# AberHu/TF-NAS

Measured on AMD Instinct MI355X. Metric: supernet search images/sec (w-step + alpha-step), higher is better.
Workload: dtype fp32

## Files before the change

### include/tfnas_hip.h

```cpp
#ifndef TFNAS_HIP_H
#define TFNAS_HIP_H

#include <stddef.h>
#include <stdint.h>

#ifdef __cplusplus
extern "C" {
#endif

#define TFNAS_ABI_VERSION 4
#define TFNAS_MAX_GROUPS 8
#define TFNAS_MAX_SINK 4
#define TFNAS_MAX_CELLS 32

#define TFNAS_MODE_CELL 0
#define TFNAS_MODE_STEM 1
#define TFNAS_MODE_HEAD 2

#define TFNAS_ACT_RELU 0
#define TFNAS_ACT_SWISH 1
#define TFNAS_ACT_RELU6 2
#define TFNAS_ACT_HSWISH 3

#define TFNAS_EINVAL (-1)
#define TFNAS_ENULL (-2)
#define TFNAS_ERANGE (-3)

typedef struct TfnasGroup {
    int32_t mc;
    int32_t k;
    int32_t se;
    int32_t mcp;
    int32_t off;
    int32_t se_off;
    int32_t pad0, pad1;
    const float *w_expand, *w_dw, *w_proj, *w_se_r, *b_se_r, *w_se_e, *b_se_e;
    float *g_expand, *g_dw, *g_proj, *g_se_r, *gb_se_r, *g_se_e, *gb_se_e;
} TfnasGroup;

typedef struct TfnasCellDesc {
    int32_t N, H, W;
    int32_t ic, oc;
    int32_t stride;
    int32_t act;
    int32_t has_res;
    int32_t G;
    int32_t need_wgrad;
    int32_t Ho, Wo;
    int32_t M;
    int32_t SE;
    float eps;
    int32_t mode;
    int32_t Hi, Wi;
    int32_t stor;
    int32_t gemm_mode;
    int32_t flags;
    TfnasGroup g[TFNAS_MAX_GROUPS];
    int (*sync_fn)(void *user, double *table, uint64_t ndoubles, void *stream);
    void *sync_user;
    int32_t sync_world;
    int32_t route;
    int32_t fwd_route;
    int32_t pad_route;
    void *wgrad_stream[3];
} TfnasCellDesc;
#define TFNAS_GEMM_EXPLICIT 0x1000
#define TFNAS_CELL_LAZY_JOIN 1
#define TFNAS_CELL_ACCUM_WGRAD 0x20
#define TFNAS_CELL_K7 0x80
#define TFNAS_CELL_ACTS 0x100
#define TFNAS_CELL_NOEXPAND 0x200
#define TFNAS_CELL_FUSED 0x400
#define TFNAS_ROUTE_FX_OFF 0x1
#define TFNAS_ROUTE_FOLD_OFF 0x2
#define TFNAS_ROUTE_DWWG_OFF 0x4
#define TFNAS_ROUTE_DWWG2_OFF 0x8
#define TFNAS_ROUTE_XG_OFF 0x10
#define TFNAS_ROUTE_XG_ALL 0x20
#define TFNAS_ROUTE_DW_SHIFT 6
#define TFNAS_ROUTE_DW_MASK 0xc0
#define TFNAS_ROUTE_SE_SHIFT 8
#define TFNAS_ROUTE_SE_MASK 0x300
#define TFNAS_ROUTE_WGRAD_INLINE 0x400
#define TFNAS_ROUTE_GRAM2 0x800
#define TFNAS_ROUTE_ALL 0xfff
#define TFNAS_ROUTE_TAKEN_VALID 0x1
#define TFNAS_ROUTE_TAKEN_FX 0x2

typedef struct TfnasCellWs {
    uint64_t E;
    uint64_t D;
    uint64_t Pr;
    uint64_t fsmall;
    uint64_t off_pooled, off_gate, off_hpre;
    uint64_t stats;
    uint64_t off_stats1, off_stats2, off_stats3;
    uint64_t out;
    uint64_t dZ;
    uint64_t dEh;
    uint64_t bsmall;
    uint64_t off_dgate, off_dpooled, off_dgl, off_dhpre, off_cb1;
    uint64_t red;
    uint64_t off_red3, off_red2, off_red1, off_resdot;
    uint64_t part;
    uint64_t dx;
    uint64_t dxp;
} TfnasCellWs;

int tfnas_abi_version(void);

typedef int (*tfnas_stats_sync_fn)(void *user, double *table, uint64_t ndoubles, void *stream);
int tfnas_set_stats_sync(tfnas_stats_sync_fn fn, void *user, int world);

int tfnas_shutdown(void);

uint64_t tfnas_sizeof(int which);

int tfnas_cell_plan(TfnasCellDesc *d);

int tfnas_cell_ws(const TfnasCellDesc *d, TfnasCellWs *ws);

int tfnas_efree_supported(const TfnasCellDesc *d);
int tfnas_cell_route(const TfnasCellDesc *d);
int tfnas_fx_supported(const TfnasCellDesc *d);

int tfnas_mixedop_fwd(const TfnasCellDesc *d, const float *x, const float *wmix,
                      float *E, float *D, float *Pr, float *fsmall, double *stats, float *part,
                      float *out, void *stream);

int tfnas_mixedop_bwd(const TfnasCellDesc *d, const float *x, const float *wmix,
                      const float *E, const float *D, const float *Pr, const float *fsmall,
                      const double *stats, const float *dout,
                      float *dZ, float *dEh, float *bsmall, double *red, float *part,
                      float *dx, float *dxp, float *dwmix, void *stream);

typedef struct TfnasBnAffine {
    const float *weight[3], *bias[3];
    float *g_weight[3], *g_bias[3];
    float *running_mean[3], *running_var[3];
    float momentum;
    int32_t eval;
} TfnasBnAffine;

int tfnas_mbconv_fwd(const TfnasCellDesc *d, const TfnasBnAffine *bn, const float *drop_scale, const float *x,
                     float *E, float *D, float *Pr, float *fsmall, double *stats, float *part, float *out, void *stream);

int tfnas_mbconv_bwd(const TfnasCellDesc *d, const TfnasBnAffine *bn, const float *drop_scale, const float *x,
                     const float *E, const float *D, const float *Pr, const float *fsmall, const double *stats,
                     const float *dout, float *dout_s, float *dZ, float *dEh, float *bsmall, double *red, float *part,
                     float *dx, float *dxp, void *stream);

int tfnas_head_affine_fwd(const TfnasCellDesc *d, const TfnasBnAffine *bn, const float *x, float *E, double *stats,
                          float *part, float *pooled, void *stream);
int tfnas_head_affine_bwd(const TfnasCellDesc *d, const TfnasBnAffine *bn, const float *x, const float *E,
                          const double *stats, const float *dpooled, float *dEh, float *cb1, double *red, float *part,
                          float *dx, float *dxp, void *stream);

int tfnas_head_fwd(const TfnasCellDesc *d, const float *x, float *E, double *stats, float *part, float *pooled,
                   void *stream);
int tfnas_head_bwd(const TfnasCellDesc *d, const float *x, const float *E, const double *stats, const float *dpooled,
                   float *dEh, float *cb1, double *red, float *part, float *dx, float *dxp, void *stream);

int tfnas_head_wgrad(const TfnasCellDesc *d, const float *x, const float *E, const float *dEh, const float *cb1, float *part,
                     void *stream);

int tfnas_cls_ce(int N, int C, int K, const float *pooled, const float *W, const float *bias, const int64_t *target, float scale,
                 float *logits, float *loss_n, float *dlogits, float *dpooled, void *stream);
int tfnas_cls_ce_ex(int N, int C, int K, const float *pooled, const float *W, const float *bias, const int64_t *target, float scale,
                    float eps, float *logits, float *loss_n, int32_t *rank, float *dlogits, float *dpooled, void *stream);
int tfnas_cls_wgrad(int npath, int N, int C, int K, const float *const *pooled, const float *const *dlogits,
                    const float *const *loss_n, float loss_scale, float *dW, float *db, float *loss, void *stream);
int tfnas_cls_wgrad_ex(int npath, int N, int C, int K, const float *const *pooled, const float *const *dlogits,
                       const float *const *loss_n, const int32_t *rank0, float loss_scale, float *dW, float *db, float *loss,
                       double *meter, void *stream);
int tfnas_cls_reduce(int N, int C, int K, const float *pooled, const float *dlogits, const float *loss_n, const int32_t *rank,
                     const float *gscale, int accumulate, float *dW, float *db, float *out, double *meter, void *stream);
int tfnas_add_into(float *dst, const float *src, uint64_t count, void *stream);

int tfnas_arch_fwd(int ncell, const float *const *log_alpha, const float *e, const float *lat, float T,
                   float *w, float *cell_lat, void *stream);

int tfnas_arch_bwd(int ncell, const float *w, const float *lat, const float *dw, const float *dcell_lat,
                   float T, float *const *dlog_alpha, void *stream);

int tfnas_arch_sample(int ncell, const float *const *log_alpha, const uint8_t *mask, const float *e, float T,
                      int mode, int32_t *pos_out, void *stream);

int tfnas_arch_project(int n, float *const *p, const int32_t *len, void *stream);

int tfnas_sink_fwd(int K, const float *betas, const float *const *res, const float *cell_lat,
                   uint64_t count, float *out, float *out_lat, float *bw_out, void *stream);

int tfnas_sink_bwd(int K, const float *bw, const float *const *res, const float *cell_lat, const float *dout,
                   const float *dlat, uint64_t count, float *const *dres, float *dbetas, float *dcell_lat,
                   double *dot_scratch, void *stream);

#define TFNAS_MAX_STAGES 8

typedef struct TfnasStage {
    int32_t ncell;
    int32_t start_res;
    int32_t first_cell;
    int32_t nres;
    const float *betas;
    float *dbetas;
} TfnasStage;

typedef struct TfnasPathDesc {
    int32_t ncell, nstage;
    int32_t soft;
    int32_t need_dx0;
    int32_t efree_mask_lo;
    int32_t reserved0;
    TfnasStage stage[TFNAS_MAX_STAGES];
    TfnasCellDesc cell[TFNAS_MAX_CELLS];
} TfnasPathDesc;

typedef struct TfnasPathWs {
    uint64_t saved;
    uint64_t scratch;
    uint64_t total;
    uint64_t out_count;
    int32_t out_h, out_w, out_c, pad;
} TfnasPathWs;

int tfnas_path_create(void **ctx);
int tfnas_path_destroy(void *ctx);
int tfnas_path_set_side_stream(void *ctx, void *stream);
int tfnas_path_plan(void *ctx, const TfnasPathDesc *pd, TfnasPathWs *ws);
int tfnas_path_set_wgrad_accum(void *ctx, uint32_t cell_mask);

int tfnas_paths_fwd(int npath, void *const *ctx, const float *const *x0, const float *const *wmix,
                    const float *const *cell_lat, float *const *arena, float *const *out, float *const *out_lat,
                    void *const *streams);

int tfnas_paths_bwd(int npath, void *const *ctx, const float *const *x0, const float *const *wmix,
                    const float *const *cell_lat, float *const *arena, const float *const *dout,
                    const float *const *dout_lat, float *const *dx0, float *const *dwmix, float *const *dcell_lat,
                    void *const *streams, int stage_begin, int stage_end);

int tfnas_sgd_clip_step(float *w, float *g, float *m, int nranges, const uint64_t *off, const uint64_t *goff, const uint64_t *len,
                        float max_norm, float lr, float momentum, float wd, float grad_scale, double *scratch,
                        uint64_t scratch_doubles, float *norm_out, void *stream);

int tfnas_pack_ranges(const float *src, float *dst, int nranges, const uint64_t *off, const uint64_t *doff,
                      const uint64_t *len, void *stream);

int tfnas_arch_adam_project(int n, float *const *p, const float *const *g, const int32_t *len, float *m, float *v,
                            float max_norm, float lr, float beta1, float beta2, float eps, float wd, int step,
                            float grad_scale, float *norm_out, void *stream);

int tfnas_set_lazy_join(int on);
int tfnas_side_stream(void *stream, void **side);
int tfnas_side_join(void *stream);

#define TFNAS_GEMM_F32 0
#define TFNAS_GEMM_BF16 1
#define TFNAS_GEMM_X2 3
#define TFNAS_GEMM_X3 6
#define TFNAS_GEMM_EVERYWHERE 0x100
int tfnas_set_gemm_mode(int mode);
int tfnas_gemm_mode(void);

int tfnas_prof_enable(unsigned mask);
int tfnas_prof_count(void);
const char *tfnas_prof_name(int id);
int tfnas_prof_collect(int id, uint64_t *launches, double *total_ms);
int tfnas_prof_last_split(int id, uint64_t *soft_launches, double *soft_ms);

#ifdef __cplusplus
}
#endif
#endif
```

### tf-nas_amd/csrc/capi.hip

```cpp
#include <string.h>
#include "tfnas_dev.h"
#include "kernels.h"
#include "cell_impl.h"

#include <stdlib.h>
#include <mutex>
#include <vector>

struct SideCtx {
    int device;
    hipStream_t main, side;
    hipEvent_t fork[4], join;
};
static std::mutex g_side_mu;
static std::vector<SideCtx*> g_side;

static SideCtx* side_for(hipStream_t s) {
    int dev = 0;
    if (hipGetDevice(&dev) != hipSuccess) return nullptr;
    std::lock_guard<std::mutex> lk(g_side_mu);
    for (SideCtx* c : g_side)
        if (c->main == s && c->device == dev) return c;
    SideCtx* c = new SideCtx();
    c->device = dev;
// ... 51 lines not shown
static int g_lazy_join = 0;
extern "C" int tfnas_set_lazy_join(int on) {
    g_lazy_join = on ? 1 : 0;
    return 0;
}
extern "C" int tfnas_side_stream(void* stream, void** side) {
    if (!side) return TFNAS_ENULL;
    *side = nullptr;
    SideCtx* c = side_for(S(stream));
    if (c) *side = (void*)c->side;
    return 0;
}
extern "C" int tfnas_side_join(void* stream) {
    return side_join(side_for(S(stream)), S(stream));
}

extern "C" int tfnas_shutdown(void) {
    std::lock_guard<std::mutex> lk(g_side_mu);
    for (SideCtx* c : g_side) {
        (void)hipStreamSynchronize(c->side);
        for (int i = 0; i < 4; ++i) (void)hipEventDestroy(c->fork[i]);
        (void)hipEventDestroy(c->join);
        (void)hipStreamDestroy(c->side);
        delete c;
    }
    g_side.clear();
    return 0;
}

StatsSync g_stats_sync = {nullptr, nullptr, 1};

extern "C" int tfnas_set_stats_sync(tfnas_stats_sync_fn fn, void* user, int world) {
    if (fn && world < 1) return TFNAS_ERANGE;
    g_stats_sync.fn = fn;
    g_stats_sync.user = user;
    g_stats_sync.world = fn ? world : 1;
    return 0;
}

extern "C" int tfnas_abi_version(void) { return TFNAS_ABI_VERSION; }
extern "C" int tfnas_set_gemm_mode(int mode) { return set_gemm_mode(mode); }
extern "C" int tfnas_gemm_mode(void) { return gemm_mode(); }

extern "C" uint64_t tfnas_sizeof(int which) {
    switch (which) {
        case 0: return sizeof(TfnasGroup);
        case 1: return sizeof(TfnasCellDesc);
        case 2: return sizeof(TfnasCellWs);
        case 3: return sizeof(TfnasStage);
        case 4: return sizeof(TfnasPathDesc);
        case 5: return sizeof(TfnasPathWs);
        case 6: return sizeof(TfnasBnAffine);
        case 7: return TFNAS_PART_ALLOC;
        case 8: return TFNAS_TAIL_SLOTS;
        default: return 0;
    }
}

static int check_act(const TfnasCellDesc* d) {
    if (d->act == TFNAS_ACT_RELU || d->act == TFNAS_ACT_SWISH) return 0;
    if (d->act != TFNAS_ACT_RELU6 && d->act != TFNAS_ACT_HSWISH) return TFNAS_EINVAL;
    if (!(d->flags & TFNAS_CELL_ACTS) || d->mode == TFNAS_MODE_STEM) return TFNAS_EINVAL;
    return 0;
}

static int check_kind(const TfnasCellDesc* d) {
    const CellKind kind = cell_kind(*d);
    if (kind == TFNAS_KIND_MBCONV) return 0;
    if (cell_noexpand(*d) && cell_fused(*d)) return TFNAS_EINVAL;
    if (d->mode != TFNAS_MODE_CELL || d->G != 1) return TFNAS_EINVAL;
    const TfnasGroup& g = d->g[0];
    if (kind == TFNAS_KIND_NOEXPAND && (g.mc != d->ic || g.w_expand || g.g_expand)) return TFNAS_EINVAL;
    if (kind == TFNAS_KIND_FUSED && (g.k != 3 || g.w_dw || g.g_dw)) return TFNAS_EINVAL;
    return 0;
}

static int check_modes(const TfnasCellDesc* d) {
    TRY(check_act(d));
    if (d->gemm_mode != 0) {
        const int gm = d->gemm_mode & ~(TFNAS_GEMM_EXPLICIT | TFNAS_GEMM_EVERYWHERE);
        if (!(d->gemm_mode & TFNAS_GEMM_EXPLICIT) || (gm != 0 && gm != 1 && gm != 3 && gm != 6)) return TFNAS_EINVAL;
    }
    if (d->flags & ~(TFNAS_CELL_LAZY_JOIN | TFNAS_CELL_ACCUM_WGRAD | TFNAS_CELL_K7 | TFNAS_CELL_ACTS | TFNAS_CELL_NOEXPAND |
                     TFNAS_CELL_FUSED))
        return TFNAS_EINVAL;
    TRY(check_kind(d));
    if (!(d->flags & TFNAS_CELL_K7)) {
        for (int g = 0; g < d->G && g < TFNAS_MAX_GROUPS; ++g)
            if (d->g[g].k == 7) return TFNAS_EINVAL;
    }
    if (d->route & ~TFNAS_ROUTE_ALL) return TFNAS_EINVAL;
    if ((d->route & TFNAS_ROUTE_XG_OFF) && (d->route & TFNAS_ROUTE_XG_ALL)) return TFNAS_EINVAL;
    if ((d->route & TFNAS_ROUTE_SE_MASK) == TFNAS_ROUTE_SE_MASK) return TFNAS_EINVAL;
    if (d->fwd_route & ~(TFNAS_ROUTE_TAKEN_VALID | TFNAS_ROUTE_TAKEN_FX)) return TFNAS_EINVAL;
    if (d->sync_fn && d->sync_world < 1) return TFNAS_ERANGE;
    return 0;
}

static bool wgrad_row_fits(const TfnasCellDesc& d) { return cell_fused(d) ? conv_wgrad_row_fits(d) : dw_wgrad_row_fits(d); }

extern "C" int tfnas_cell_plan(TfnasCellDesc* d) {
    if (!d) return TFNAS_ENULL;
    if (d->G < 1 || d->G > TFNAS_MAX_GROUPS) return TFNAS_ERANGE;
    if (d->mode < TFNAS_MODE_CELL || d->mode > TFNAS_MODE_HEAD) return TFNAS_EINVAL;
    if (d->mode == TFNAS_MODE_STEM) {
        if (d->ic != 27 || d->G != 1 || d->Hi < 1 || d->Wi < 1 || d->has_res) return TFNAS_EINVAL;
        d->H = (d->Hi - 1) / 2 + 1;
        d->W = (d->Wi - 1) / 2 + 1;
    } else if (d->ic < 4 || (d->ic & 3)) {
        return TFNAS_EINVAL;
    }
    if (d->mode == TFNAS_MODE_HEAD && d->G != 1) return TFNAS_EINVAL;
    if (d->stor != 0) return TFNAS_EINVAL;
    if (d->N < 1 || d->H < 1 || d->W < 1 || d->oc < 4 || (d->oc & 3)) return TFNAS_EINVAL;
    if (d->oc > 1024) return TFNAS_EINVAL;
    if (d->stride != 1 && d->stride != 2) return TFNAS_EINVAL;
    TRY(check_act(d));
    if (d->has_res && (d->ic != d->oc || d->stride != 1)) return TFNAS_EINVAL;
    TRY(check_modes(d));
    d->Ho = (d->H - 1) / d->stride + 1;
    d->Wo = (d->W - 1) / d->stride + 1;
    int off = 0, se_off = 0;
    for (int g = 0; g < d->G; ++g) {
        TfnasGroup& gr = d->g[g];
        if (gr.mc < 1 || (gr.k != 3 && gr.k != 5 && gr.k != 7) ||
            gr.se < 0) return TFNAS_EINVAL;
        if (gr.se & 3) return TFNAS_EINVAL;
        gr.mcp = (gr.mc + 3) & ~3;
        off = (off + 31) & ~31;
        gr.off = off;
        gr.se_off = se_off;
        off += gr.mcp;
        se_off += gr.se;
    }
    off = (off + 31) & ~31;
    if ((off & 511) == 0) off += 32;
    d->M = off;
    d->SE = se_off;
    if ((double)d->N * d->H * d->W >= 2147483647.0) return TFNAS_ERANGE;
    if (!wgrad_row_fits(*d)) return TFNAS_ERANGE;
    return 0;
}

extern "C" int tfnas_cell_ws(const TfnasCellDesc* d, TfnasCellWs* ws) {
    if (!d || !ws) return TFNAS_ENULL;
    memset(ws, 0, sizeof(*ws));
    if (!wgrad_row_fits(*d)) return TFNAS_ERANGE;
    const uint64_t P = (uint64_t)d->N * d->H * d->W, Po = (uint64_t)d->N * d->Ho * d->Wo;
    const uint64_t M = d->M, N = d->N, SE = d->SE, G = d->G, oc = d->oc;
    ws->E = cell_has_E(*d) ? P * M : 0;
    ws->D = Po * M;
    ws->Pr = G * Po * oc;
    ws->off_pooled = 0;
    ws->off_gate = N * M;
    ws->off_hpre = 2 * N * M;
    ws->fsmall = 2 * N * M + N * SE + 4;
    ws->off_stats1 = 0;
    ws->off_stats2 = 2 * M;
    ws->off_stats3 = 4 * M;
    ws->stats = 4 * M + 2 * G * oc;
    ws->out = Po * oc;
    ws->dZ = Po * M;
    ws->dEh = P * M;
    ws->off_dgate = 0;
    ws->off_dpooled = N * M;
    ws->off_dgl = 2 * N * M;
    ws->off_dhpre = 3 * N * M;
    ws->off_cb1 = 3 * N * M + ((N * SE + 3) & ~(uint64_t)3);
    ws->bsmall = ws->off_cb1 + 4 * M;
    ws->off_red3 = 0;
    ws->off_resdot = 2 * G * oc;
    ws->off_red2 = 2 * G * oc + oc;
    ws->off_red1 = ws->off_red2 + 2 * M;
    ws->red = ws->off_red1 + 2 * M;
    ws->part = (d->need_wgrad ? 2 : 1) * (uint64_t)TFNAS_PART_ALLOC;
    ws->dx = P * d->ic;
    {
        const int ns = (d->mode == TFNAS_MODE_STEM || !cell_has_E(*d)) ? 1 : gemm_plan_expand_dgrad(*d, true).splits;
        ws->dxp = ns > 1 ? (uint64_t)ns * P * d->ic : 4;
    }
    return 0;
}

extern "C" int tfnas_efree_supported(const TfnasCellDesc* dp) { return (dp && efree_supported(*dp)) ? 1 : 0; }
extern "C" int tfnas_fx_supported(const TfnasCellDesc* dp) { return (dp && fx_supported(*dp)) ? 1 : 0; }
static int route_taken(const TfnasCellDesc& d, bool affine) {
    return TFNAS_ROUTE_TAKEN_VALID | ((!affine && fx_supported(d)) ? TFNAS_ROUTE_TAKEN_FX : 0);
}
extern "C" int tfnas_cell_route(const TfnasCellDesc* dp) { return dp ? route_taken(*dp, false) : 0; }

static void bn_site(const TfnasCellDesc& d, int site, int& nch, uint64_t& cnt) {
    const uint64_t P = (uint64_t)d.N * d.H * d.W, Po = (uint64_t)d.N * d.Ho * d.Wo;
    nch = site == 2 ? d.oc : d.g[0].mc;
    cnt = site == 0 ? P : Po;
}
static int check_bn_sites(const TfnasCellDesc& d, const TfnasBnAffine* bn) {
    if (cell_has_bn0(d)) return 0;
    if (bn->weight[0] || bn->bias[0] || bn->g_weight[0] || bn->g_bias[0] || bn->running_mean[0] || bn->running_var[0])
        return TFNAS_EINVAL;
    return 0;
}
static int bn_fwd_fix(const TfnasCellDesc& d, const TfnasBnAffine* bn, int site, double* stats, hipStream_t s) {
    int nch;
    uint64_t cnt;
    bn_site(d, site, nch, cnt);
    return launch_bn_fwd_fix(stats, nch, cnt, d.eps, bn->weight[site], bn->bias[site], bn->running_mean[site],
                             bn->running_var[site], bn->momentum, bn->eval, s, stats_world(d));
}

static int fwd_front_mbconv(const TfnasCellDesc& d, const TfnasCellDesc& d0, const CellFwdBufs& b, bool fx, bool sync,
                            double* stats1, double* stats2, hipStream_t s) {
    const TfnasBnAffine* bn = b.bn;
    if (fx) TRY(launch_fx_stats(d, b.x, stats1, b.part, s));
    else if (b.E) TRY(launch_expand_fwd(d, b.x, b.E, stats1, b.part, s));
    else TRY(launch_expand_stats_gram(d, b.x, stats1, b.part, s));
    if (sync) TRY(stats_sync(d, stats1, 2 * (size_t)d.M, s));
    if (bn) TRY(bn_fwd_fix(d0, bn, 0, stats1, s));
    if (fx) TRY(launch_fx_fwd(d, b.x, stats1, b.E, b.D, stats2, b.part, s));
    else TRY(launch_dw_fwd(d, b.E, b.x, stats1, b.D, stats2, b.part, s));
    return 0;
}

int cell_fwd_impl(const TfnasCellDesc& d0, const TfnasCellWs& ws, const CellFwdBufs& b, hipStream_t s, int* route) {
    double* stats1 = b.stats + ws.off_stats1;
    double* stats2 = b.stats + ws.off_stats2;
    double* stats3 = b.stats + ws.off_stats3;
    float* pooled = b.fsmall + ws.off_pooled;
    float* gate = b.fsmall + ws.off_gate;
    float* hpre = b.fsmall + ws.off_hpre;
    const TfnasBnAffine* bn = b.bn;
    TfnasCellDesc dc = d0;
    if (bn) dc.eps = -1.f;
    const TfnasCellDesc& d = dc;
    const int taken = route_taken(d0, bn != nullptr);
    if (route) *route = taken;
    const bool fx = (taken & TFNAS_ROUTE_TAKEN_FX) != 0;
    const bool sync = !(bn && bn->eval);
    switch (cell_kind(d)) {
    case TFNAS_KIND_FUSED:
        TRY(launch_conv_fwd(d, b.x, b.D, stats2, b.part, s));
        break;
    case TFNAS_KIND_NOEXPAND:
        TRY(launch_dw_fwd(d, nullptr, b.x, nullptr, b.D, stats2, b.part, s));
        break;
    case TFNAS_KIND_MBCONV:
        TRY(fwd_front_mbconv(d, d0, b, fx, sync, stats1, stats2, s));
        break;
    }
    if (sync) TRY(stats_sync(d, stats2, 2 * (size_t)d.M, s));
    if (bn) TRY(bn_fwd_fix(d0, bn, 1, stats2, s));
    TRY(launch_se_pool(d, b.D, stats2, pooled, s));
    TRY(launch_se_fc_fwd(d, pooled, hpre, gate, b.part, TFNAS_PART_FLOATS, s));
    TRY(launch_project_fwd(d, b.D, gate, stats2, b.Pr, stats3, b.part, s));
    if (sync) TRY(stats_sync(d, stats3, 2 * (size_t)d.G * d.oc, s));
    if (bn) TRY(bn_fwd_fix(d0, bn, 2, stats3, s));
    if (b.drop_scale && d.has_res) {
        TfnasCellDesc dn = dc;
        dn.has_res = 0;
        TRY(launch_mix_fwd(dn, b.Pr, stats3, b.wmix, b.x, b.out, s));
        return launch_rowscale(b.out, b.out, b.x, b.drop_scale, d.N, (uint64_t)d.Ho * d.Wo * d.oc, s);
    }
    TRY(launch_mix_fwd(d, b.Pr, stats3, b.wmix, b.x, b.out, s));
    return 0;
}

static hipStream_t fork_to(const CellSide* so, int k, hipStream_t main) {
    if (!so || !so->side[k] || so->side[k] == main) return main;
    if (hipEventRecord(so->fork[k], main) != hipSuccess || hipStreamWaitEvent(so->side[k], so->fork[k], 0) != hipSuccess)
        return main;
    return so->side[k];
}

static int bn_bwd_fix(const TfnasCellDesc& d, const TfnasBnAffine* bn, int site, double* red, hipStream_t s) {
    int nch;
    uint64_t cnt;
    bn_site(d, site, nch, cnt);
    TRY(launch_bn_bwd_fix(red, nch, cnt, bn->weight[site], bn->bias[site], bn->g_weight[site], bn->g_bias[site], s,
                          wgrad_accum(d)));
    if (bn->eval) return (int)hipMemsetAsync(red, 0, sizeof(double) * 2 * (size_t)nch, s);
    return 0;
}

static int expand_dx(const TfnasCellDesc& d, const float* dEh, const float* x, const float* cb1, float* part, const float* dout,
                     const float* wmix, float* dx, float* dxp, hipStream_t s, const float* add_src = nullptr,
                     const float* add_scale = nullptr, int nsl = -1) {
    const size_t room = TFNAS_PART_FLOATS - expand_gram_floats(d);
    float* gram = part + room;
    TRY(launch_expand_gram(d, cb1, part, room, gram, s));
    return launch_expand_dgrad(d, dEh, x, cb1, gram, dout, wmix, dx, dxp, s, add_src, add_scale, nsl);
}


namespace {
struct CellBwd {
    const TfnasCellDesc& d0;
    TfnasCellDesc d;
    const TfnasCellWs& ws;
    CellBwdBufs b;
    hipStream_t s;
    const CellSide* so;
    const TfnasBnAffine* bn;
    int taken;
    const float* dout_res;
    const double *stats1, *stats2, *stats3;
    const float *pooled, *gate, *hpre;
    float *dgate, *dpooled, *dhpre, *cb1;
    double *red3, *red2, *red1;
    float *part, *part_w, *part_w1, *part_w2;

    int run();
    int tail_fused();
    int tail_noexpand();
    int tail_mbconv();
};

int CellBwd::run() {
    if (d.need_wgrad) {
        const CellKind kind = cell_kind(d);
        for (int g = 0; g < d.G; ++g) {
            const TfnasGroup& gr = d.g[g];
            if ((!gr.g_expand && kind != TFNAS_KIND_NOEXPAND) || (!gr.g_dw && kind != TFNAS_KIND_FUSED) || !gr.g_proj) return TFNAS_ENULL;
            if (gr.se > 0 && (!gr.g_se_r || !gr.gb_se_r || !gr.g_se_e || !gr.gb_se_e)) return TFNAS_ENULL;
        }
    }
    TRY(launch_mix_bwd_stats(d, b.dout, b.Pr, stats3, b.x, red3, part, s));
    TRY(stats_sync(d, red3, 2 * (size_t)d.G * d.oc, s));
    if (b.dwmix) TRY(launch_mix_dw(d, red3, b.red + ws.off_resdot, b.dwmix, s));
    if (bn) TRY(bn_bwd_fix(d0, bn, 2, red3, s));
    if (!b.dx && !d.need_wgrad) return 0;
    if (d.need_wgrad)
        TRY(launch_project_wgrad(d, b.dout, b.Pr, b.D, gate, stats2, stats3, red3, b.wmix, part_w, fork_to(so, 0, s)));
    const bool fused2 = bn2_fused_fits(d);
    const bool fold = fused2 && !(d.route & TFNAS_ROUTE_FOLD_OFF) && project_fold_ok(d, (size_t)ws.dEh) && (d.G == 1 || d.Ho * d.Wo <= 784);
    if (fold) {
        TRY(launch_project_dgrad(d, b.dout, b.Pr, stats3, red3, b.wmix, b.dZ, s, b.D, stats2, b.dEh));
        TRY(launch_bn2_gather(d, b.dEh, dgate, part, s));
    } else {
        TRY(launch_project_dgrad(d, b.dout, b.Pr, stats3, red3, b.wmix, b.dZ, s));
        if (fused2) TRY(launch_bn2_pool(d, b.dZ, b.D, stats2, dgate, part, s));
        else TRY(launch_se_bwd_reduce(d, b.dZ, b.D, stats2, dgate, s));
    }
    TRY(launch_se_fc_bwd(d, dgate, gate, hpre, dhpre, dpooled, b.dEh, (size_t)ws.dEh, s));
    if (fused2) TRY(launch_bn2_finish(d, part, gate, dpooled, red2, s));
    else TRY(launch_bn2_bwd(d, b.dZ, b.D, stats2, gate, dpooled, red2, part, s));
    TRY(stats_sync(d, red2, 2 * (size_t)d.M, s));
    if (bn) TRY(bn_bwd_fix(d0, bn, 1, red2, s));
    switch (cell_kind(d)) {
    case TFNAS_KIND_FUSED: return tail_fused();
    case TFNAS_KIND_NOEXPAND: return tail_noexpand();
    case TFNAS_KIND_MBCONV: break;
    }
    return tail_mbconv();
}

int CellBwd::tail_fused() {
    TRY(launch_conv_dd(d, b.dZ, b.D, gate, dpooled, stats2, red2, b.dEh, s));
    if (d.need_wgrad) {
        hipStream_t sw = fork_to(so, 1, s);
        if (d.SE > 0) TRY(launch_se_wgrad(d, dgate, gate, dhpre, hpre, pooled, sw));
        TRY(launch_conv_wgrad(d, b.dEh, b.x, part_w1, sw));
    }
    if (b.dx) TRY(launch_conv_dgrad(d, b.dEh, d.has_res ? dout_res : nullptr, b.dx, part, s));
    return 0;
}

int CellBwd::tail_noexpand() {
    if (d.need_wgrad) {
        hipStream_t sw = fork_to(so, 1, s);
        if (d.SE > 0) TRY(launch_se_wgrad(d, dgate, gate, dhpre, hpre, pooled, sw));
        TRY(launch_dw_wgrad(d, b.dZ, gate, dpooled, b.D, stats2, red2, b.x, nullptr, part_w1, sw));
    }
    if (b.dx)
        TRY(launch_dw_bwd_dx(d, b.dZ, gate, dpooled, b.D, stats2, red2, d.has_res ? dout_res : nullptr, b.dx, s));
    return 0;
}

int CellBwd::tail_mbconv() {
    if (taken & TFNAS_ROUTE_TAKEN_FX) {
        int nsl = 0;
        TRY(launch_fx_bwd(d, b.x, b.E, stats1, stats2, red2, b.dZ, b.D, gate, dpooled, b.dEh, (size_t)ws.dEh, red1, cb1, part, &nsl, s));
        if (b.dx) TRY(expand_dx(d, nullptr, b.x, cb1, part, dout_res, b.wmix, b.dx, b.dEh, s, b.add_src, b.add_scale, nsl));
        return 0;
    }
    const DwPlan dw_bwd = dw_plan_bwd_data(d, b.E == nullptr, b.x != nullptr);
    const bool dw_fused = dw_bwd.fuse_wgrad;
    if (d.need_wgrad) {
        if (d.SE > 0 || !dw_fused) {
            hipStream_t sw = fork_to(so, 1, s);
            if (d.SE > 0) TRY(launch_se_wgrad(d, dgate, gate, dhpre, hpre, pooled, sw));
            if (!dw_fused) TRY(launch_dw_wgrad(d, b.dZ, gate, dpooled, b.D, stats2, red2, b.E, stats1, part_w1, sw));
        }
    }
    if (bn || stats_sync_on(d)) {
        TRY(launch_dw_bwd_data(dw_bwd, d, b.dZ, gate, dpooled, b.D, stats2, red2, b.E, b.x, stats1, b.dEh, red1, part, s));
        TRY(stats_sync(d, red1, 2 * (size_t)d.M, s));
        if (bn) TRY(bn_bwd_fix(d0, bn, 0, red1, s));
        TRY(launch_bn1_consts(d, stats1, red1, cb1, s));
    } else {
        TRY(launch_dw_bwd_data(dw_bwd, d, b.dZ, gate, dpooled, b.D, stats2, red2, b.E, b.x, stats1, b.dEh, red1, part, s, cb1));
    }
    if (d.need_wgrad) TRY(launch_expand_wgrad(d, b.dEh, b.E, cb1, b.x, part_w2, fork_to(so, 2, s)));
    if (b.dx && d.mode != TFNAS_MODE_STEM)
        TRY(expand_dx(d, b.dEh, b.x, cb1, part, dout_res, b.wmix, b.dx, b.dxp, s, b.add_src, b.add_scale));
    return 0;
}
}

int cell_bwd_impl(const TfnasCellDesc& d0, const TfnasCellWs& ws, const CellBwdBufs& b0, hipStream_t s, const CellSide* so,
                  int fwd_route) {
    const TfnasBnAffine* bn = b0.bn;
    const int taken = route_taken(d0, bn != nullptr);
    if ((fwd_route & TFNAS_ROUTE_TAKEN_VALID) && taken != fwd_route) return TFNAS_EINVAL;
    const CellBwdBufs& b = b0;
    CellBwd c = {d0, d0, ws, b0, s, so, bn, taken, b0.dout,
                 b.stats + ws.off_stats1, b.stats + ws.off_stats2, b.stats + ws.off_stats3,
                 b.fsmall + ws.off_pooled, b.fsmall + ws.off_gate, b.fsmall + ws.off_hpre,
                 b.bsmall + ws.off_dgate, b.bsmall + ws.off_dpooled, b.bsmall + ws.off_dhpre, b.bsmall + ws.off_cb1,
                 b.red + ws.off_red3, b.red + ws.off_red2, b.red + ws.off_red1,
                 b.part, b.part_w,
                 b.part_w1 ? b.part_w1 : b.part_w,
                 b.part_w2 ? b.part_w2 : b.part_w};
    if (bn) c.d.eps = -1.f;
    if (b0.drop_scale && d0.has_res) {
        if (!b0.dout_s) return TFNAS_ENULL;
        TRY(launch_rowscale(b0.dout_s, b0.dout, nullptr, b0.drop_scale, d0.N, (uint64_t)d0.Ho * d0.Wo * d0.oc, s));
        c.b.dout = b0.dout_s;
    }
    return c.run();
}

static int check_E(const TfnasCellDesc& d, const float* E, bool efree_counts) {
    if (E || !cell_has_E(d) || (efree_counts && efree_supported(d))) return 0;
    return TFNAS_ENULL;
}

extern "C" int tfnas_mixedop_fwd(const TfnasCellDesc* dp, const float* x, const float* wmix, float* E, float* D,
                                 float* Pr, float* fsmall, double* stats, float* part, float* out, void* stream) {
    if (!dp || !x || !D || !Pr || !fsmall || !stats || !part || !out) return TFNAS_ENULL;
    const TfnasCellDesc& d = *dp;
    if (d.mode == TFNAS_MODE_HEAD) return TFNAS_EINVAL;
    TRY(check_modes(dp));
    TRY(check_E(d, E, true));
    TfnasCellWs ws;
    TRY(tfnas_cell_ws(dp, &ws));
    CellFwdBufs b = {x, wmix, E, D, Pr, fsmall, stats, part, out};
    return cell_fwd_impl(d, ws, b, S(stream));
}

static int cell_bwd_entry(const TfnasCellDesc& d, CellBwdBufs b, hipStream_t s, void* const* wgrad_stream, bool lazy) {
    TfnasCellWs ws;
    TRY(tfnas_cell_ws(&d, &ws));
    SideCtx* sc = (d.need_wgrad && route_side(d)) ? side_for(s) : nullptr;
    SideJoinGuard guard;
    guard.c = sc;
    guard.main = s;
    CellSide so = {};
    if (sc) {
        for (int i = 0; i < 3; ++i) {
            hipStream_t own = (wgrad_stream && wgrad_stream[i]) ? S(wgrad_stream[i]) : nullptr;
            so.side[i] = own ? own : sc->side;
            guard.extra[i] = own;
            so.fork[i] = sc->fork[i];
            if (own) {
// ... 210 lines not shown
```

### tf-nas_amd/csrc/cell_impl.h

```cpp
#pragma once
#include <hip/hip_runtime.h>
#include "tfnas_hip.h"

static inline hipStream_t S(void* s) { return reinterpret_cast<hipStream_t>(s); }

#define TRY(call)               \
    do {                        \
        int _r = (call);        \
        if (_r != 0) return _r; \
    } while (0)

struct CellFwdBufs {
    const float* x;
    const float* wmix;
    float *E, *D, *Pr, *fsmall;
    double* stats;
    float* part;
    float* out;
    const TfnasBnAffine* bn = nullptr;
    const float* drop_scale = nullptr;
};

struct CellBwdBufs {
    const float *x, *wmix, *E, *D, *Pr, *fsmall;
    const double* stats;
    const float* dout;
    float *dZ, *dEh, *bsmall;
    double* red;
    float *part, *part_w;
    float *dx, *dxp, *dwmix;
    const float* add_src;
    const float* add_scale;
    const TfnasBnAffine* bn = nullptr;
    const float* drop_scale = nullptr;
    float* dout_s = nullptr;
    float *part_w1 = nullptr, *part_w2 = nullptr;
};

struct CellSide {
    hipStream_t side[3];
    hipEvent_t fork[3];
};

int cell_fwd_impl(const TfnasCellDesc& d, const TfnasCellWs& ws, const CellFwdBufs& b, hipStream_t s, int* route = nullptr);
int cell_bwd_impl(const TfnasCellDesc& d, const TfnasCellWs& ws, const CellBwdBufs& b, hipStream_t s, const CellSide* so,
                  int fwd_route);
```

### tf-nas_amd/csrc/efree_kernels.hip

```cpp
#include "tfnas_dev.h"
#include "kernels.h"
#include "prof.h"
#include "efree.h"

__global__ __launch_bounds__(256) void k_x_colsum(const float* __restrict__ x, int P, int ic, int rps,
                                                  float* __restrict__ part) {
    __shared__ f32x4 red[256];
    const int tid = threadIdx.x, icq = ic >> 2, stride = (256 / icq) * icq;
    const int r0 = blockIdx.x * rps, r1 = min(P, r0 + rps);
    const f32x4* __restrict__ x4 = reinterpret_cast<const f32x4*>(x) + (size_t)r0 * icq;
    const int n4 = (r1 - r0) * icq;
    f32x4 s = zero4();
    if (tid < stride) {
        int i = tid;
        for (; i + 7 * stride < n4; i += 8 * stride) {
            f32x4 v[8];
#pragma unroll
            for (int u = 0; u < 8; ++u) v[u] = x4[i + u * stride];
            s += ((v[0] + v[1]) + (v[2] + v[3])) + ((v[4] + v[5]) + (v[6] + v[7]));
        }
        for (; i < n4; i += stride) s += x4[i];
    }
    red[tid] = s;
    __syncthreads();
    if (tid < ic) {
        const int cq = tid >> 2, comp = tid & 3;
        float t = 0.f;
        for (int k = cq; k < stride; k += icq) t += red[k][comp];
        part[(size_t)blockIdx.x * ic + tid] = t;
    }
}

template <int CT>
__global__ __launch_bounds__(256) void k_x_gram(const float* __restrict__ x, int P, int ic, int rps,
                                                const double* __restrict__ xsum, float* __restrict__ part) {
    __shared__ float red[4][CT * CT][4][64 + 1];
    const int tid = threadIdx.x, lane = tid & 63, wave = tid >> 6, n = lane & 15, q = lane >> 4;
    const int r0 = blockIdx.x * rps, r1 = min(P, r0 + rps);
    float mu[CT];
    bool chok[CT];
#pragma unroll
    for (int t = 0; t < CT; ++t) {
        chok[t] = 16 * t + n < ic;
        mu[t] = chok[t] ? (float)(xsum[16 * t + n] / (double)P) : 0.f;
    }
    f32x4 acc[CT][CT];
#pragma unroll
    for (int i = 0; i < CT; ++i)
#pragma unroll
        for (int j = 0; j < CT; ++j) acc[i][j] = zero4();
    for (int p = r0 + 4 * wave; p < r1; p += 64) {
        float a[4][CT];
#pragma unroll
        for (int u = 0; u < 4; ++u) {
            const int row = p + 16 * u + q;
#pragma unroll
            for (int t = 0; t < CT; ++t)
                a[u][t] = (row < r1 && chok[t]) ? x[(size_t)row * ic + 16 * t + n] - mu[t] : 0.f;
        }
#pragma unroll
        for (int u = 0; u < 4; ++u)
#pragma unroll
            for (int i = 0; i < CT; ++i)
#pragma unroll
                for (int j = 0; j < CT; ++j)
                    acc[i][j] = __builtin_amdgcn_mfma_f32_16x16x4f32(a[u][i], a[u][j], acc[i][j], 0, 0, 0);
    }
#pragma unroll
    for (int i = 0; i < CT; ++i)
#pragma unroll
        for (int j = 0; j < CT; ++j)
#pragma unroll
            for (int r = 0; r < 4; ++r) red[wave][i * CT + j][r][lane] = acc[i][j][r];
    __syncthreads();
    for (int e = tid; e < ic * ic; e += 256) {
        const int gi = e / ic, gj = e - gi * ic;
        const int i = gi >> 4, ri = gi & 15, j = gj >> 4, l = (ri >> 2) * 16 + (gj & 15), r = ri & 3;
        part[(size_t)blockIdx.x * ic * ic + e] =
            (red[0][i * CT + j][r][l] + red[1][i * CT + j][r][l]) + (red[2][i * CT + j][r][l] + red[3][i * CT + j][r][l]);
    }
}

__global__ __launch_bounds__(256) void k_stats1_gram(TfnasCellDesc d, const double* __restrict__ xsum,
                                                     const double* __restrict__ C, double* __restrict__ stats1) {
    __shared__ double Cs[40 * 40 + 40];
    const int ic = d.ic;
    for (int i = threadIdx.x; i < ic * ic + ic; i += 256) Cs[i] = i < ic * ic ? C[i] : xsum[i - ic * ic];
    __syncthreads();
    const int col = blockIdx.x * 256 + threadIdx.x;
    if (col >= d.M) return;
    int g = 0;
    for (; g < d.G - 1; ++g)
        if (col < d.g[g + 1].off) break;
    const int m = col - d.g[g].off;
    double s = 0.0, q = 0.0;
    if (m < d.g[g].mc) {
        const float* __restrict__ w = d.g[g].w_expand + (size_t)m * ic;
        const double P = (double)d.N * d.H * d.W;
        float wr[40];
#pragma unroll
        for (int c = 0; c < 40; ++c) wr[c] = c < ic ? w[c] : 0.f;
        for (int c = 0; c < ic; ++c) {
            double t0 = 0.0, t1 = 0.0;
            const double* row = Cs + c * ic;
#pragma unroll
            for (int c2 = 0; c2 < 40; c2 += 2) {
                if (c2 < ic) {
                    t0 += row[c2] * (double)wr[c2];
                    t1 += row[c2 + 1] * (double)wr[c2 + 1];
                }
            }
            q += (double)w[c] * (t0 + t1);
            s += (double)w[c] * Cs[ic * ic + c];
        }
        q += s * s / P;
    }
    stats1[2 * (size_t)col + 0] = s;
    stats1[2 * (size_t)col + 1] = q;
}

bool efree_supported(const TfnasCellDesc& d) {
    if (d.mode != TFNAS_MODE_CELL || d.need_wgrad) return false;
    if (act_tile_only(d.act)) return false;
    if (cell_noexpand(d) || cell_fused(d)) return false;
    if (!efree_ic_ok(d.ic)) return fx_supported(d);
    if (stats_sync_on(d)) return false;
    if ((size_t)d.N * d.H * d.W * d.ic >= ((size_t)1 << 31)) return false;
    for (int g = 0; g < d.G; ++g)
        if (d.g[g].k != 3 && d.g[g].k != 5) return false;
    return true;
}

int launch_x_colsum(const float* x, int P, int ic, int rps, int nb, float* part, hipStream_t s) {
    ProfScope _prof(TK_EXPAND_FWD, s);
    hipLaunchKernelGGL(k_x_colsum, dim3(nb), dim3(256), 0, s, x, P, ic, rps, part);
    return (int)hipGetLastError();
}

int launch_expand_stats_gram(const TfnasCellDesc& d, const float* x, double* stats1, float* part, hipStream_t s) {
    const int P = d.N * d.H * d.W, ic = d.ic, ne = ic * ic;
    int rps = cdiv(P, 1024);
    if (rps < 256) rps = 256;
    rps = (rps + 63) & ~63;
    const int nb = cdiv(P, rps);
    double* xsum = reinterpret_cast<double*>(part + TFNAS_PART_FLOATS) - (ne + ic + 2);
    xsum = reinterpret_cast<double*>((uintptr_t)xsum & ~(uintptr_t)15);
    double* C = xsum + ic;
    if ((size_t)nb * ne + 2 * (size_t)(ne + ic + 4) > TFNAS_PART_FLOATS) return TFNAS_ERANGE;
    {
        ProfScope _prof(TK_EXPAND_FWD, s);
        hipLaunchKernelGGL(k_x_colsum, dim3(nb), dim3(256), 0, s, x, P, ic, rps, part);
    }
    int rc = launch_reduce_rows(part, nb, ic, (size_t)ic, xsum, nullptr, s);
    if (rc) return rc;
    {
        ProfScope _prof(TK_EXPAND_FWD, s);
        if (ic <= 16) hipLaunchKernelGGL(k_x_gram<1>, dim3(nb), dim3(256), 0, s, x, P, ic, rps, xsum, part);
        else if (ic <= 32) hipLaunchKernelGGL(k_x_gram<2>, dim3(nb), dim3(256), 0, s, x, P, ic, rps, xsum, part);
        else hipLaunchKernelGGL(k_x_gram<3>, dim3(nb), dim3(256), 0, s, x, P, ic, rps, xsum, part);
    }
    rc = launch_reduce_rows(part, nb, ne, (size_t)ne, C, nullptr, s);
    if (rc) return rc;
    ProfScope _prof(TK_SMALL, s);
    hipLaunchKernelGGL(k_stats1_gram, dim3(cdiv(d.M, 256)), dim3(256), 0, s, d, xsum, C, stats1);
    return (int)hipGetLastError();
}
```

### tf-nas_amd/csrc/fx_kernels.hip

```cpp
#include "tfnas_dev.h"
#include "kernels.h"
#include "prof.h"
#include "fx.h"
#include "gemm_x3.h"
#include <type_traits>

static int fx_ks(int ic) { return (ic + 31) / 32; }

bool fx_plan(const TfnasCellDesc& d, FxPlan& pl, bool bwd) {
    if (d.mode != TFNAS_MODE_CELL || d.need_wgrad) return false;
    if (d.act != TFNAS_ACT_RELU && d.act != TFNAS_ACT_SWISH) return false;
    if (stats_sync_on(d)) return false;
    if (d.ic < 64 || d.ic > 192 || (d.ic & 15)) return false;
    if (d.stride != 1) return false;
    const int HW = d.H * d.W;
    if (HW > 196 || d.W < 4) return false;
    const int KS = fx_ks(d.ic);
    int NI = 128 / HW;
    if (NI < 1) NI = 1;
    if (NI > 4) NI = 4;
    if (NI > d.N) NI = d.N;
    const int ntiles = (NI * HW + 15) / 16, RT = (ntiles + 7) / 8;
    const int RTF = (ntiles + 6) / 7;
    if (RTF * KS > 8) return false;
// ... 23 lines not shown
    }
    if (want < 1) want = 1;
    int cps = (nch + want - 1) / want;
    if (cps < (bwd ? 6 : 3)) cps = bwd ? 6 : 3;
    int ns = 0, chunk0 = 0;
    for (int g = 0; g < d.G; ++g) {
        const int ng = (d.g[g].mcp + 31) / 32;
        const int parts = (ng + cps - 1) / cps;
        for (int p = 0; p < parts; ++p) {
            if (ns >= FX_MAX_SLICES) return false;
            const int a = (int)((long)ng * p / parts), b = (int)((long)ng * (p + 1) / parts);
            pl.sl[ns].g = (int16_t)g;
            pl.sl[ns].c0 = (int16_t)(32 * a);
            pl.sl[ns].nch = (int16_t)(b - a);
            pl.sl[ns].chunk0 = (int16_t)(chunk0 + a);
            ++ns;
        }
        chunk0 += ng;
    }
    pl.nslices = ns;
    return true;
}

static size_t fx_fwd_lds(const TfnasCellDesc& d, const FxPlan& pl) {
    const int PAD = pl.KMAX / 2, HP = d.H + 2 * PAD, WP = (d.W + 2 * PAD) | 1;
    const size_t tile = (size_t)(pl.NI * HP * WP + 8) * 128;
    return 2 * tile + 2 * (size_t)pl.PB + 2 * (size_t)pl.WB + 2 * 2048;
}

__device__ __host__ __forceinline__ int fx_swz(int row) { return (0x1230 >> (4 * ((row >> 2) & 3))) & 3; }

__device__ __forceinline__ void fx_split3(float v, unsigned short& h, unsigned short& m, unsigned short& l) {
    const unsigned hb = x3_bits(v);
    const float r1 = v - x3_float(hb & 0xffff0000u);
    const unsigned mb = x3_bits(r1);
    const float r2 = r1 - x3_float(mb & 0xffff0000u);
    h = (unsigned short)(hb >> 16);
    m = (unsigned short)(mb >> 16);
    l = (unsigned short)(x3_bits(r2) >> 16);
}

__global__ __launch_bounds__(256) void k_fx_pack(TfnasCellDesc d, FxPlan pl, const double* __restrict__ stats1,
                                                 const double* __restrict__ stats2, const double* __restrict__ red2,
                                                 unsigned char* __restrict__ blob) {
    const int chunk = blockIdx.x, cy = blockIdx.y * 8, tid = threadIdx.x;
    int si = 0;
    for (; si < pl.nslices - 1; ++si)
        if (chunk < pl.sl[si + 1].chunk0) break;
    const int g = pl.sl[si].g, c0 = pl.sl[si].c0 + 32 * (chunk - pl.sl[si].chunk0);
    const int mc = d.g[g].mc, off = d.g[g].off, ic = d.ic, K = d.g[g].k, KK = K * K;
    const int RS = pl.RS, KP = 32 * pl.KS;
    unsigned char* b = blob + (size_t)chunk * pl.BLOB;
    const float* __restrict__ w1 = d.g[g].w_expand;
    __shared__ float2 cst[8];
    __shared__ float w1s[8][200];
    if (tid < 8) {
        float2 c = make_float2(0.f, 0.f);
        if (c0 + cy + tid < mc) c = bn_consts(stats1 + 2 * (size_t)(off + c0 + cy + tid), 1.0 / ((double)d.N * d.H * d.W), d.eps);
        cst[tid] = c;
        reinterpret_cast<float2*>(b + 96 * RS)[cy + tid] = c;
    }
    for (int e = tid; e < 8 * ic; e += 256) {
        const int chl = e / ic, c = e - chl * ic;
        w1s[chl][c] = (c0 + cy + chl < mc) ? w1[(size_t)(c0 + cy + chl) * ic + c] : 0.f;
    }
    __syncthreads();
    for (int e = tid; e < 8 * (KP / 8); e += 256) {
        const int chl = e / (KP / 8), k0 = 8 * (e - chl * (KP / 8));
        unsigned short h[8], m[8], l[8];
#pragma unroll
        for (int j = 0; j < 8; ++j) fx_split3(k0 + j < ic ? w1s[chl][k0 + j] : 0.f, h[j], m[j], l[j]);
        unsigned char* row = b + (cy + chl) * RS + 2 * k0;
        *reinterpret_cast<u32x4*>(row) = u32x4{h[0] | (unsigned)h[1] << 16, h[2] | (unsigned)h[3] << 16, h[4] | (unsigned)h[5] << 16, h[6] | (unsigned)h[7] << 16};
        *reinterpret_cast<u32x4*>(row + 32 * RS) = u32x4{m[0] | (unsigned)m[1] << 16, m[2] | (unsigned)m[3] << 16, m[4] | (unsigned)m[5] << 16, m[6] | (unsigned)m[7] << 16};
        *reinterpret_cast<u32x4*>(row + 64 * RS) = u32x4{l[0] | (unsigned)l[1] << 16, l[2] | (unsigned)l[3] << 16, l[4] | (unsigned)l[5] << 16, l[6] | (unsigned)l[7] << 16};
    }
    float* taps = reinterpret_cast<float*>(b + pl.PB);
    for (int e = tid; e < KK * 8; e += 256) {
        const int t = e >> 3, ch = cy + (e & 7);
        taps[t * 32 + ch] = (c0 + ch < mc) ? d.g[g].w_dw[(size_t)(c0 + ch) * KK + t] : 0.f;
    }
    if (pl.XB) {
        f32x4* c2 = reinterpret_cast<f32x4*>(b + pl.PB + pl.WB);
        if (tid < 8) {
            f32x4 t = zero4();
            const int ch = cy + tid;
            if (c0 + ch < mc) {
                const double inv = 1.0 / ((double)d.N * d.Ho * d.Wo);
                const float2 c = bn_consts(stats2 + 2 * (size_t)(off + c0 + ch), inv, d.eps);
                t.x = c.x;
                t.y = c.y;
                t.z = (float)(red2[2 * (size_t)(off + c0 + ch) + 0] * inv);
                t.w = (float)(red2[2 * (size_t)(off + c0 + ch) + 1] * inv);
            }
            c2[ch] = t;
        }
        unsigned char* wr = b + pl.PB + pl.WB + 512;
        for (int c = tid; c < ic; c += 256) {
            unsigned short h[8], m[8], l[8];
#pragma unroll
            for (int j = 0; j < 8; ++j) fx_split3(cst[j].y * w1s[j][c], h[j], m[j], l[j]);
            unsigned char* p = wr + c * 64 + (((cy >> 3) ^ fx_swz(c)) * 16);
            *reinterpret_cast<u32x4*>(p) = u32x4{h[0] | (unsigned)h[1] << 16, h[2] | (unsigned)h[3] << 16, h[4] | (unsigned)h[5] << 16, h[6] | (unsigned)h[7] << 16};
            *reinterpret_cast<u32x4*>(p + ic * 64) = u32x4{m[0] | (unsigned)m[1] << 16, m[2] | (unsigned)m[3] << 16, m[4] | (unsigned)m[5] << 16, m[6] | (unsigned)m[7] << 16};
            *reinterpret_cast<u32x4*>(p + 2 * ic * 64) = u32x4{l[0] | (unsigned)l[1] << 16, l[2] | (unsigned)l[3] << 16, l[4] | (unsigned)l[5] << 16, l[6] | (unsigned)l[7] << 16};
        }
    }
}

typedef unsigned char u8;

template <int KS, int RT>
struct FxX {
    bf16x8 h[RT][KS], m[RT][KS], l[RT][KS];
};

__device__ __forceinline__ void fx_split8(f32x4 a, f32x4 b, bf16x8& h, bf16x8& m, bf16x8& l) {
    const X3Planes pa = x3_split4<6>(a), pb = x3_split4<6>(b);
    h = __builtin_bit_cast(bf16x8, u32x4{pa.h.x, pa.h.y, pb.h.x, pb.h.y});
    m = __builtin_bit_cast(bf16x8, u32x4{pa.m.x, pa.m.y, pb.m.x, pb.m.y});
    l = __builtin_bit_cast(bf16x8, u32x4{pa.l.x, pa.l.y, pb.l.x, pb.l.y});
}

#define FX_MFMA6(acc, ah, am, al, bh, bm, bl)                                   \
    acc = __builtin_amdgcn_mfma_f32_16x16x32_bf16(al, bh, acc, 0, 0, 0);        \
    acc = __builtin_amdgcn_mfma_f32_16x16x32_bf16(am, bm, acc, 0, 0, 0);        \
    acc = __builtin_amdgcn_mfma_f32_16x16x32_bf16(ah, bl, acc, 0, 0, 0);        \
    acc = __builtin_amdgcn_mfma_f32_16x16x32_bf16(am, bh, acc, 0, 0, 0);        \
    acc = __builtin_amdgcn_mfma_f32_16x16x32_bf16(ah, bm, acc, 0, 0, 0);        \
    acc = __builtin_amdgcn_mfma_f32_16x16x32_bf16(ah, bh, acc, 0, 0, 0);

template <int NV>
struct FxCopy {
    u32x4 v[NV];
    __device__ __forceinline__ void load(const u8* __restrict__ src, int bytes) {
#pragma unroll
        for (int i = 0; i < NV; ++i) {
            const int o = (threadIdx.x + i * FX_THREADS) * 16;
            v[i] = *reinterpret_cast<const u32x4*>(src + (o < bytes ? o : bytes - 16));
        }
    }
    __device__ __forceinline__ void store(u8* dst, int bytes) const {
#pragma unroll
        for (int i = 0; i < NV; ++i) {
            const int o = (threadIdx.x + i * FX_THREADS) * 16;
            if (o < bytes) *reinterpret_cast<u32x4*>(dst + o) = v[i];
        }
    }
};

#define FX_TERM(A_, B_)                                                                                                  \
    _Pragma("unroll") for (int ct = 0; ct < 2; ++ct) _Pragma("unroll") for (int pt = 0; pt < RT; ++pt)                   \
        acc[ct][pt] = __builtin_amdgcn_mfma_f32_16x16x32_bf16(A_[ct], X.B_[pt][ks], acc[ct][pt], 0, 0, 0);

template <int KS, int RT, int OUT>
__device__ __forceinline__ void fx_expand(const u8* P, const FxX<KS, RT>& X, float* tile, const int (&slot)[RT],
                                          const bool (&pv)[RT], int ntiles, float* __restrict__ eg = nullptr,
                                          const size_t* egoff = nullptr, int chlim = 0) {
    constexpr int RS = 64 * KS + FX_RS_PAD;
    const int lane = threadIdx.x & 63, wave = threadIdx.x >> 6, n = lane & 15, q = lane >> 4;
    f32x4 acc[2][RT];
#pragma unroll
    for (int ct = 0; ct < 2; ++ct)
#pragma unroll
        for (int pt = 0; pt < RT; ++pt) acc[ct][pt] = zero4();
#pragma unroll
    for (int ks = 0; ks < KS; ++ks) {
// ... 792 lines not shown
            for (int r = 0; r < NR; ++r) {
                const size_t a = (pixbase + lpix[r]) * M + goff + cn + 4 * cq;
                dz[r] = ld4_nt(dZ + a);
                dv[r] = ld4_nt(Dt + a);
            }
        }
        {
            const float* taps = reinterpret_cast<const float*>(Wb(i & 1));
            f32x4 t1 = zero4(), t2 = zero4();
            const float* base = DD + it.toff;
            f32x4 acc[4] = {zero4(), zero4(), zero4(), zero4()};
#pragma unroll 1
            for (int ky = 0; ky < K; ++ky) {
                const float* rowp = base + ky * WP * 32;
                const float* wp = taps + (K * K - 1 - ky * K) * 32 + 4 * cq;
                f32x4 win[K + 3];
#pragma unroll
                for (int u = 0; u < K + 3; ++u) win[u] = ld4(rowp + u * 32);
#pragma unroll
                for (int kx = 0; kx < K; ++kx) {
                    const f32x4 wv = ld4(wp - kx * 32);
#pragma unroll
                    for (int jj = 0; jj < 4; ++jj) acc[jj] += win[jj + kx] * wv;
                }
            }
#pragma unroll
            for (int jj = 0; jj < 4; ++jj) {
                const bool ok = chok && jj < it.npx;
                f32x4 de;
#pragma unroll
                for (int r = 0; r < 4; ++r) de[r] = ok ? acc[jj][r] * act_d<ACT>(ev[jj][r]) : 0.f;
                t1 += de;
#pragma unroll
                for (int r = 0; r < 4; ++r) t2[r] += ok ? de[r] * ev[jj][r] : 0.f;
                if (jj < it.npx) st4(DE + it.eoff + jj * 32, de);
            }
            fx_stat_park(t1, t2, St);
        }
        __syncthreads();
    }
    float* __restrict__ dst = dxp + (size_t)si * d.N * HW * ic;
#pragma unroll
    for (int pt = 0; pt < RT; ++pt) {
        if (pv[pt]) {
            float* __restrict__ o = dst + (pixbase + prow_[pt]) * ic + 4 * q;
#pragma unroll
            for (int ct = 0; ct < CT; ++ct) st4(o + 16 * ct, dx[ct][pt]);
        }
    }
}

template <int ACT, int CT, int RT>
__global__ __launch_bounds__(FX_THREADS) void k_fx_bwde(TfnasCellDesc d, FxPlan pl, const u8* __restrict__ blob,
                                                        const float* __restrict__ Eh, const float* __restrict__ dZ,
                                                        const float* __restrict__ Dt, const float* __restrict__ gate,
                                                        const float* __restrict__ dpooled, float* __restrict__ dxp,
                                                        float* __restrict__ part) {
    extern __shared__ __attribute__((aligned(16))) u8 fx_lds[];
    const int si = blockIdx.x / pl.nig, ig = blockIdx.x - si * pl.nig;
    const FxSlice sl = pl.sl[si];
    if (d.g[sl.g].k == 3) fx_bwde_body<3, ACT, CT, RT>(d, pl, blob, Eh, dZ, Dt, gate, dpooled, dxp, part, fx_lds, ig, sl, si);
    else fx_bwde_body<5, ACT, CT, RT>(d, pl, blob, Eh, dZ, Dt, gate, dpooled, dxp, part, fx_lds, ig, sl, si);
}

template <int ACT, int CT, int RT>
__global__ __launch_bounds__(FX_THREADS) void k_fx_bwd(TfnasCellDesc d, FxPlan pl, const float* __restrict__ x,
                                                       const u8* __restrict__ blob, const float* __restrict__ dZ,
                                                       const float* __restrict__ Dt, const float* __restrict__ gate,
                                                       const float* __restrict__ dpooled, float* __restrict__ dxp,
                                                       float* __restrict__ part) {
    extern __shared__ __attribute__((aligned(16))) u8 fx_lds[];
    const int si = blockIdx.x / pl.nig, ig = blockIdx.x - si * pl.nig;
    const FxSlice sl = pl.sl[si];
    if (d.g[sl.g].k == 3) fx_bwd_body<3, ACT, CT, RT>(d, pl, x, blob, dZ, Dt, gate, dpooled, dxp, part, fx_lds, ig, sl, si);
    else fx_bwd_body<5, ACT, CT, RT>(d, pl, x, blob, dZ, Dt, gate, dpooled, dxp, part, fx_lds, ig, sl, si);
}

template <int CT>
__global__ __launch_bounds__(256) void k_fx_gram(const float* __restrict__ x, int P, int ic, int rps,
                                                 const double* __restrict__ xsum, float* __restrict__ part) {
    constexpr int NT = (CT + 3) / 4;
    const int tid = threadIdx.x, lane = tid & 63, wave = tid >> 6, n = lane & 15, q = lane >> 4, jy = blockIdx.y;
    const int r0 = blockIdx.x * rps, r1 = min(P, r0 + rps);
    float mui[NT], muj[NT];
#pragma unroll
    for (int t = 0; t < NT; ++t) {
        const int it = wave + 4 * t, jt = jy + 4 * t;
        mui[t] = it < CT ? (float)(xsum[16 * it + n] / (double)P) : 0.f;
        muj[t] = jt < CT ? (float)(xsum[16 * jt + n] / (double)P) : 0.f;
    }
    f32x4 acc[NT][NT];
#pragma unroll
    for (int i = 0; i < NT; ++i)
#pragma unroll
        for (int j = 0; j < NT; ++j) acc[i][j] = zero4();
    constexpr int RU = 8;
    for (int p = r0; p < r1; p += 4 * RU) {
        float a[RU][NT], b[RU][NT];
#pragma unroll
        for (int u = 0; u < RU; ++u) {
            const int row = p + 4 * u + q;
            const float* __restrict__ xr = x + (size_t)(row < r1 ? row : r1 - 1) * ic + n;
#pragma unroll
            for (int t = 0; t < NT; ++t) {
                const int it = wave + 4 * t, jt = jy + 4 * t;
                const float va = xr[16 * (it < CT ? it : 0)], vb = xr[16 * (jt < CT ? jt : 0)];
                a[u][t] = (row < r1 && it < CT) ? va - mui[t] : 0.f;
                b[u][t] = (row < r1 && jt < CT) ? vb - muj[t] : 0.f;
            }
        }
#pragma unroll
        for (int u = 0; u < RU; ++u)
#pragma unroll
            for (int i = 0; i < NT; ++i)
#pragma unroll
                for (int j = 0; j < NT; ++j) acc[i][j] = __builtin_amdgcn_mfma_f32_16x16x4f32(a[u][i], b[u][j], acc[i][j], 0, 0, 0);
    }
    float* __restrict__ out = part + (size_t)blockIdx.x * ic * ic;
#pragma unroll
    for (int i = 0; i < NT; ++i) {
        const int it = wave + 4 * i;
#pragma unroll
        for (int j = 0; j < NT; ++j) {
            const int jt = jy + 4 * j;
            if (it < CT && jt < CT) {
#pragma unroll
                for (int r = 0; r < 4; ++r) out[(size_t)(16 * it + 4 * q + r) * ic + 16 * jt + n] = acc[i][j][r];
            }
        }
    }
}

typedef double f64x4 __attribute__((ext_vector_type(4)));
__device__ __forceinline__ const float* fx_wrow(const TfnasCellDesc& d, int col) {
    if (col >= d.M) return nullptr;
    int g = 0;
    for (; g < d.G - 1; ++g)
        if (col < d.g[g + 1].off) break;
    const int m = col - d.g[g].off;
    return (m >= 0 && m < d.g[g].mc) ? d.g[g].w_expand + (size_t)m * d.ic : nullptr;
}
template <int CT>
__global__ __launch_bounds__(256) void k_fx_stats1(TfnasCellDesc d, const double* __restrict__ xsum, const double* __restrict__ C,
                                                   double* __restrict__ stats1) {
    constexpr int NT = (CT + 3) / 4;
    __shared__ double red[2][4][16];
    const int tid = threadIdx.x, lane = tid & 63, wave = tid >> 6, n = lane & 15, q = lane >> 4, ic = d.ic, col0 = blockIdx.x * 16;
    const float* __restrict__ wa = fx_wrow(d, col0 + n);
    f64x4 acc[NT];
#pragma unroll
    for (int t = 0; t < NT; ++t) acc[t] = f64x4{0.0, 0.0, 0.0, 0.0};
    const float* __restrict__ wac = wa ? wa : d.g[0].w_expand;
    int ctile[NT];
#pragma unroll
    for (int t = 0; t < NT; ++t) ctile[t] = wave + 4 * t < CT ? 16 * (wave + 4 * t) : 0;
    constexpr int PD = 4;
    float an[PD];
    double bn[PD][NT];
    const int nks = ic >> 2;
#pragma unroll
    for (int u = 0; u < PD; ++u) {
        const int k = 4 * (u < nks ? u : nks - 1) + q;
        an[u] = wac[k];
#pragma unroll
        for (int t = 0; t < NT; ++t) bn[u][t] = C[(size_t)k * ic + n + ctile[t]];
    }
    for (int ks = 0; ks < nks; ks += PD) {
#pragma unroll
        for (int u = 0; u < PD; ++u) {
            const bool live = ks + u < nks;
            const double a = (wa && live) ? (double)an[u] : 0.0;
            double b[NT];
#pragma unroll
            for (int t = 0; t < NT; ++t) b[t] = bn[u][t];
            const int kn = ks + u + PD;
            const int k = 4 * (kn < nks ? kn : nks - 1) + q;
            an[u] = wac[k];
#pragma unroll
            for (int t = 0; t < NT; ++t) bn[u][t] = C[(size_t)k * ic + n + ctile[t]];
#pragma unroll
            for (int t = 0; t < NT; ++t) acc[t] = __builtin_amdgcn_mfma_f64_16x16x4f64(a, b[t], acc[t], 0, 0, 0);
        }
    }
#pragma unroll
    for (int i = 0; i < 4; ++i) {
        const int col = col0 + q + 4 * i;
        const float* __restrict__ wr = fx_wrow(d, col);
        double qf = 0.0, sm = 0.0;
        if (wr) {
#pragma unroll
            for (int t = 0; t < NT; ++t) {
                if (wave + 4 * t < CT) {
                    const double wv = (double)wr[ctile[t] + n];
                    qf += acc[t][i] * wv;
                    sm += wv * xsum[ctile[t] + n];
                }
            }
        }
#pragma unroll
        for (int o = 1; o < 16; o <<= 1) {
            qf += __shfl_xor(qf, o, 64);
            sm += __shfl_xor(sm, o, 64);
        }
        if (n == 0) {
            red[0][wave][q + 4 * i] = sm;
            red[1][wave][q + 4 * i] = qf;
        }
    }
    __syncthreads();
    if (tid < 16 && col0 + tid < d.M) {
        const double sm = (red[0][0][tid] + red[0][1][tid]) + (red[0][2][tid] + red[0][3][tid]);
        const double qf = (red[1][0][tid] + red[1][1][tid]) + (red[1][2][tid] + red[1][3][tid]);
        const double P = (double)d.N * d.H * d.W;
        stats1[2 * (size_t)(col0 + tid) + 0] = sm;
        stats1[2 * (size_t)(col0 + tid) + 1] = qf + sm * sm / P;
    }
}

int launch_fx_stats(const TfnasCellDesc& d, const float* x, double* stats1, float* part, hipStream_t s) {
    const int P = d.N * d.H * d.W, ic = d.ic, ne = ic * ic;
    int nb = 256;
    while (nb > 1 && (size_t)nb * ne + 2 * (size_t)(ne + ic + 4) + 64 > TFNAS_PART_FLOATS) nb >>= 1;
    int rps = cdiv(P, nb);
    rps = (rps + 3) & ~3;
    if (rps < 16) rps = 16;
    nb = cdiv(P, rps);
    double* xsum = reinterpret_cast<double*>(part + TFNAS_PART_FLOATS) - (ne + ic + 2);
    xsum = reinterpret_cast<double*>((uintptr_t)xsum & ~(uintptr_t)15);
    double* Cm = xsum + ic;
    int rc = launch_x_colsum(x, P, ic, rps, nb, part, s);
    if (rc) return rc;
    rc = launch_reduce_rows(part, nb, ic, (size_t)ic, xsum, nullptr, s);
    if (rc) return rc;
    {
        ProfScope _prof(TK_EXPAND_FWD, s);
        const int CT = ic / 16;
        switch (CT) {
#define FX_GRAM(N_) case N_: hipLaunchKernelGGL(k_fx_gram<N_>, dim3(nb, 4), dim3(256), 0, s, x, P, ic, rps, xsum, part); break;
            FX_GRAM(4) FX_GRAM(5) FX_GRAM(6) FX_GRAM(7) FX_GRAM(8) FX_GRAM(9) FX_GRAM(10) FX_GRAM(11) FX_GRAM(12)
#undef FX_GRAM
            default: return TFNAS_EINVAL;
        }
    }
    rc = launch_reduce_rows(part, nb, ne, (size_t)ne, Cm, nullptr, s);
    if (rc) return rc;
    ProfScope _prof(TK_SMALL, s);
    switch (ic / 16) {
#define FX_ST1(N_) case N_: hipLaunchKernelGGL(k_fx_stats1<N_>, dim3(cdiv(d.M, 16)), dim3(256), 0, s, d, xsum, Cm, stats1); break;
        FX_ST1(4) FX_ST1(5) FX_ST1(6) FX_ST1(7) FX_ST1(8) FX_ST1(9) FX_ST1(10) FX_ST1(11) FX_ST1(12)
#undef FX_ST1
        default: return TFNAS_EINVAL;
    }
    return (int)hipGetLastError();
}

static bool fx_attr_done(const void* fn, size_t shm) {
    return hipFuncSetAttribute(fn, hipFuncAttributeMaxDynamicSharedMemorySize, (int)shm) == hipSuccess;
}

int launch_fx_fwd(const TfnasCellDesc& d, const float* x, const double* stats1, float* E, float* D, double* stats2,
                  float* part, hipStream_t s) {
    FxPlan pl;
    if (!fx_plan(d, pl, false)) return TFNAS_EINVAL;
    const size_t rows = ((size_t)pl.nig * 2 * d.M + 63) & ~(size_t)63;
    u8* blob = reinterpret_cast<u8*>(part + rows);
    {
        ProfScope _prof(TK_SMALL, s);
        hipLaunchKernelGGL(k_fx_pack, dim3(pl.nchunks, 4), dim3(256), 0, s, d, pl, stats1, (const double*)nullptr,
                           (const double*)nullptr, blob);
    }
    const size_t shm = fx_fwd_lds(d, pl);
    const dim3 grid(pl.nig * pl.nslices);
    {
        ProfScope _prof(TK_DW_FWD, s, d.G > 2);
#define FX_FWD(A_, KS_, RT_)                                                                                        \
    {                                                                                                               \
        static bool attr = fx_attr_done((const void*)k_fx_fwd<A_, KS_, RT_>, 160 * 1024);                           \
        if (!attr) return TFNAS_EINVAL;                                                                             \
        hipLaunchKernelGGL((k_fx_fwd<A_, KS_, RT_>), grid, dim3(FX_THREADS), shm, s, d, pl, x, blob, D, part, E);   \
    }
#define FX_FWD_A(KS_, RT_)                                                       \
    {                                                                            \
        if (d.act == TFNAS_ACT_RELU) FX_FWD(TFNAS_ACT_RELU, KS_, RT_)            \
        else if (d.act == TFNAS_ACT_SWISH) FX_FWD(TFNAS_ACT_SWISH, KS_, RT_)     \
        else return TFNAS_EINVAL;                                                \
    }
        const int key = pl.KS * 10 + pl.RTF;
        switch (key) {
            case 21: FX_FWD_A(2, 1) break;
            case 22: FX_FWD_A(2, 2) break;
            case 31: FX_FWD_A(3, 1) break;
            case 32: FX_FWD_A(3, 2) break;
            case 41: FX_FWD_A(4, 1) break;
            case 42: FX_FWD_A(4, 2) break;
            case 51: FX_FWD_A(5, 1) break;
            case 61: FX_FWD_A(6, 1) break;
            default: return TFNAS_EINVAL;
        }
#undef FX_FWD_A
#undef FX_FWD
    }
    int rc = (int)hipGetLastError();
    if (rc) return rc;
    return launch_reduce_rows(part, pl.nig, 2 * d.M, 2 * (size_t)d.M, stats2, nullptr, s);
}

static bool fx_enabled(const TfnasCellDesc& d) { return !(d.route & TFNAS_ROUTE_FX_OFF); }

static bool fx_bwd_layout(const TfnasCellDesc& d, const FxPlan& pl, size_t scratch_floats, size_t& blob_off_scratch,
                          size_t& blob_off_part) {
    const size_t P = (size_t)d.N * d.H * d.W;
    const size_t dxp = (((size_t)(pl.nslices + 1) * P * d.ic) + 63) & ~(size_t)63;
    const size_t blobs = ((size_t)pl.nchunks * pl.BLOB + 3) / 4;
    if (dxp > scratch_floats) return false;
    blob_off_scratch = blob_off_part = ~(size_t)0;
    if (dxp + blobs <= scratch_floats) {
        blob_off_scratch = dxp;
        return true;
    }
    const size_t rows = ((size_t)pl.nig * 2 * d.M + 63) & ~(size_t)63;
    if (rows + blobs + 256 > TFNAS_PART_FLOATS) return false;
    blob_off_part = rows;
    return true;
}

bool fx_supported(const TfnasCellDesc& d) {
    FxPlan pl;
    if (cell_noexpand(d) || cell_fused(d)) return false;
    if (!fx_enabled(d) || !fx_plan(d, pl, false)) return false;
    if (gemm_mode_of(d) != TFNAS_GEMM_X3) return false;
    if (fx_fwd_lds(d, pl) > 160 * 1024) return false;
    const size_t rows = (((size_t)pl.nig * 2 * d.M) + 63) & ~(size_t)63, blobs = ((size_t)pl.nchunks * pl.BLOB + 3) / 4;
    const size_t top = 2 * (size_t)(d.ic * d.ic + d.ic + 4) + 64;
    if (rows + blobs + top + 256 > TFNAS_PART_FLOATS) return false;
    FxPlan pb;
    if (!fx_plan(d, pb, true)) return false;
    if (fx_bwd_lds(d, pb) > 160 * 1024 || fx_bwde_lds(d, pb) > 160 * 1024) return false;
    size_t a, b;
    return fx_bwd_layout(d, pb, (size_t)d.N * d.H * d.W * d.M, a, b);
}

int launch_fx_bwd(const TfnasCellDesc& d, const float* x, const float* Eh, const double* stats1, const double* stats2,
                  const double* red2, const float* dZ, const float* D, const float* gate, const float* dpooled, float* scratch,
                  size_t scratch_floats, double* red1, float* cb1, float* part, int* nsl, hipStream_t s) {
    FxPlan pl;
    if (!fx_plan(d, pl, true)) return TFNAS_EINVAL;
    size_t bo_s, bo_p;
    if (!fx_bwd_layout(d, pl, scratch_floats, bo_s, bo_p)) return TFNAS_ERANGE;
    u8* blob = reinterpret_cast<u8*>(bo_s != ~(size_t)0 ? scratch + bo_s : part + bo_p);
    {
        ProfScope _prof(TK_SMALL, s);
        hipLaunchKernelGGL(k_fx_pack, dim3(pl.nchunks, 4), dim3(256), 0, s, d, pl, stats1, stats2, red2, blob);
    }
    const size_t shm = Eh ? fx_bwde_lds(d, pl) : fx_bwd_lds(d, pl);
    const dim3 grid(pl.nig * pl.nslices);
    {
        ProfScope _prof(TK_DW_BWD_DATA, s, d.G > 2);
#define FX_BWD(A_, CT_, RT_)                                                                                         \
    {                                                                                                                \
        static bool attr = fx_attr_done((const void*)k_fx_bwd<A_, CT_, RT_>, 160 * 1024) &&                          \
                           fx_attr_done((const void*)k_fx_bwde<A_, CT_, RT_>, 160 * 1024);                           \
        if (!attr) return TFNAS_EINVAL;                                                                              \
        if (Eh)                                                                                                      \
            hipLaunchKernelGGL((k_fx_bwde<A_, CT_, RT_>), grid, dim3(FX_THREADS), shm, s, d, pl, blob, Eh, dZ, D,    \
                               gate, dpooled, scratch, part);                                                        \
        else                                                                                                         \
            hipLaunchKernelGGL((k_fx_bwd<A_, CT_, RT_>), grid, dim3(FX_THREADS), shm, s, d, pl, x, blob, dZ, D,      \
                               gate, dpooled, scratch, part);                                                        \
    }
#define FX_BWD_A(CT_, RT_)                                                       \
    {                                                                            \
        if (d.act == TFNAS_ACT_RELU) FX_BWD(TFNAS_ACT_RELU, CT_, RT_)            \
        else if (d.act == TFNAS_ACT_SWISH) FX_BWD(TFNAS_ACT_SWISH, CT_, RT_)     \
        else return TFNAS_EINVAL;                                                \
    }
        const int key = (d.ic / 16) * 10 + (Eh ? pl.RTF : pl.RT);
        switch (key) {
            case 41: FX_BWD_A(4, 1) break;
            case 42: FX_BWD_A(4, 2) break;
            case 51: FX_BWD_A(5, 1) break;
            case 52: FX_BWD_A(5, 2) break;
            case 61: FX_BWD_A(6, 1) break;
            case 62: FX_BWD_A(6, 2) break;
            case 71: FX_BWD_A(7, 1) break;
            case 72: FX_BWD_A(7, 2) break;
            case 81: FX_BWD_A(8, 1) break;
            case 82: FX_BWD_A(8, 2) break;
            case 91: FX_BWD_A(9, 1) break;
            case 101: FX_BWD_A(10, 1) break;
            case 111: FX_BWD_A(11, 1) break;
            case 121: FX_BWD_A(12, 1) break;
            default: return TFNAS_EINVAL;
        }
#undef FX_BWD_A
#undef FX_BWD
    }
    int rc = (int)hipGetLastError();
    if (rc) return rc;
    *nsl = pl.nslices;
    return launch_reduce_bn1(d, part, pl.nig, stats1, red1, cb1, s);
}
```

### tf-nas_amd/csrc/kernels.h

```cpp
#pragma once
#include <stdlib.h>
#include <hip/hip_runtime.h>
#include "tfnas_hip.h"

struct StatsSync {
    tfnas_stats_sync_fn fn;
    void* user;
    int world;
};
extern StatsSync g_stats_sync;
static inline StatsSync sync_of(const TfnasCellDesc& d) {
    if (d.sync_fn) return StatsSync{d.sync_fn, d.sync_user, d.sync_world > 0 ? d.sync_world : 1};
    return g_stats_sync;
}
static inline bool stats_sync_on(const TfnasCellDesc& d) { return sync_of(d).fn != nullptr; }
static inline int stats_sync(const TfnasCellDesc& d, double* table, size_t ndoubles, hipStream_t s) {
    const StatsSync y = sync_of(d);
    return y.fn ? y.fn(y.user, table, (uint64_t)ndoubles, (void*)s) : 0;
}
static inline uint64_t stats_world(const TfnasCellDesc& d) {
    const StatsSync y = sync_of(d);
    return (y.fn && y.world > 1) ? (uint64_t)y.world : 1;
}

static inline int route_dw(const TfnasCellDesc& d) { return (d.route & TFNAS_ROUTE_DW_MASK) >> TFNAS_ROUTE_DW_SHIFT; }
static inline int route_se(const TfnasCellDesc& d) { return (d.route & TFNAS_ROUTE_SE_MASK) >> TFNAS_ROUTE_SE_SHIFT; }
static inline bool route_side(const TfnasCellDesc& d) { return !(d.route & TFNAS_ROUTE_WGRAD_INLINE); }
static inline int wgrad_accum(const TfnasCellDesc& d) { return (d.flags & TFNAS_CELL_ACCUM_WGRAD) ? 1 : 0; }
static constexpr bool act_tile_only(int act) { return act == TFNAS_ACT_RELU6 || act == TFNAS_ACT_HSWISH; }
static inline bool cell_noexpand(const TfnasCellDesc& d) { return (d.flags & TFNAS_CELL_NOEXPAND) != 0; }
static inline bool cell_fused(const TfnasCellDesc& d) { return (d.flags & TFNAS_CELL_FUSED) != 0; }
enum CellKind { TFNAS_KIND_MBCONV, TFNAS_KIND_NOEXPAND, TFNAS_KIND_FUSED };
static inline CellKind cell_kind(const TfnasCellDesc& d) {
    return cell_fused(d) ? TFNAS_KIND_FUSED : cell_noexpand(d) ? TFNAS_KIND_NOEXPAND : TFNAS_KIND_MBCONV;
}
static inline bool cell_has_E(const TfnasCellDesc& d) { return cell_kind(d) == TFNAS_KIND_MBCONV; }
static inline bool cell_has_bn0(const TfnasCellDesc& d) { return cell_kind(d) == TFNAS_KIND_MBCONV; }
#define ACT_DISPATCH(act, ...)                                                                        \
    if ((act) == TFNAS_ACT_RELU) { constexpr int ACT = TFNAS_ACT_RELU; __VA_ARGS__; }                 \
    else if ((act) == TFNAS_ACT_SWISH) { constexpr int ACT = TFNAS_ACT_SWISH; __VA_ARGS__; }          \
    else if ((act) == TFNAS_ACT_RELU6) { constexpr int ACT = TFNAS_ACT_RELU6; __VA_ARGS__; }          \
    else if ((act) == TFNAS_ACT_HSWISH) { constexpr int ACT = TFNAS_ACT_HSWISH; __VA_ARGS__; }        \
    else return TFNAS_EINVAL;

int gemm_mode();
int set_gemm_mode(int m);
int gemm_mode_of(const TfnasCellDesc& d);
enum GemmVariant { GEMM_PLAIN, GEMM_STEM, GEMM_XG, GEMM_FOLD, GEMM_GRAM1 };
struct GemmPlan {
    GemmVariant var;
    int mm;
    int nt, tiles;
    int splits;
    int rps;
    int parts;
    dim3 grid, grid2;
    size_t shm;
    size_t out, out_main;
};
GemmPlan gemm_plan_expand_fwd(const TfnasCellDesc& d);
GemmPlan gemm_plan_project_fwd(const TfnasCellDesc& d);
GemmPlan gemm_plan_project_dgrad(const TfnasCellDesc& d, bool fold);
GemmPlan gemm_plan_project_wgrad(const TfnasCellDesc& d);
GemmPlan gemm_plan_expand_gram(const TfnasCellDesc& d, size_t scratch_floats);
GemmPlan gemm_plan_expand_dgrad(const TfnasCellDesc& d, bool split, int nsl = -1);
GemmPlan gemm_plan_expand_wgrad(const TfnasCellDesc& d);
int launch_expand_fwd(const TfnasCellDesc& d, const float* x, float* E, double* stats1, float* part,
                      hipStream_t s);
int launch_project_fwd(const TfnasCellDesc& d, const float* D, const float* gate, const double* stats2,
                       float* Pr, double* stats3, float* part, hipStream_t s);
int launch_project_dgrad(const TfnasCellDesc& d, const float* dout, const float* Pr, const double* stats3,
                         const double* red3, const float* wmix, float* dZ, hipStream_t s, const float* D = nullptr,
                         const double* stats2 = nullptr, float* rec = nullptr);
constexpr int FOLD_SLOTS = 4, FOLD_Q = 5;
static inline bool project_fold_ok(const TfnasCellDesc& d, size_t scratch_floats) {
    const int HW = d.Ho * d.Wo;
    const size_t nrt = ((size_t)d.N * HW + 127) / 128;
    if (act_tile_only(d.act)) return false;
    return HW >= 43 && nrt * FOLD_SLOTS * FOLD_Q * (size_t)d.M <= scratch_floats;
}
int launch_project_wgrad(const TfnasCellDesc& d, const float* dout, const float* Pr, const float* D,
                         const float* gate, const double* stats2, const double* stats3, const double* red3,
                         const float* wmix, float* part, hipStream_t s);
size_t expand_gram_floats(const TfnasCellDesc& d);
int launch_expand_gram(const TfnasCellDesc& d, const float* cb1, float* scratch, size_t scratch_floats, float* gram,
                       hipStream_t s);
int launch_expand_dgrad(const TfnasCellDesc& d, const float* dEh, const float* x, const float* cb1, const float* gram,
                        const float* dout, const float* wmix, float* dx, float* dxp, hipStream_t s,
                        const float* add_src = nullptr, const float* add_scale = nullptr, int nsl = -1);
int launch_expand_wgrad(const TfnasCellDesc& d, const float* dEh, const float* E, const float* cb1,
                        const float* x, float* part, hipStream_t s);

struct DwDirect {
    int chunks;
    int ncg;
    int nseg;
    int per;
    int steps;
    int nwg;
};
struct DwSlide {
    int TH, TW;
    int CC, CCP, cq_shift;
    int RB, L1;
    int chunks, gx;
};
struct DwGeom {
    int T0, T1;
    int CC;
    int cq_shift;
    int tilesH, tilesW, ntiles;
    int L0, L1;
};
enum DwFamily { DW_DIRECT, DW_RING, DW_TILE };
constexpr int DW_NK = 3;
struct DwPlan {
    DwFamily fam;
    int rows;
    int chunks[DW_NK];
    DwDirect direct[2];
    DwSlide ring[2];
    DwGeom tile[DW_NK];
    int jw;
    bool pipe;
    int kq;
    bool fuse_wgrad;
};
int launch_dw_fwd(const TfnasCellDesc& d, const float* E, const float* x, const double* stats1, float* D,
                  double* stats2, float* part, hipStream_t s);
bool efree_supported(const TfnasCellDesc& d);
static inline bool efree_ic_ok(int ic) { return ic == 16 || ic == 24 || ic == 40; }
int launch_expand_stats_gram(const TfnasCellDesc& d, const float* x, double* stats1, float* part, hipStream_t s);
int launch_x_colsum(const float* x, int P, int ic, int rps, int nb, float* part, hipStream_t s);
bool fx_supported(const TfnasCellDesc& d);
int launch_fx_stats(const TfnasCellDesc& d, const float* x, double* stats1, float* part, hipStream_t s);
int launch_fx_fwd(const TfnasCellDesc& d, const float* x, const double* stats1, float* E, float* D, double* stats2,
                  float* part, hipStream_t s);
int launch_fx_bwd(const TfnasCellDesc& d, const float* x, const float* Eh, const double* stats1, const double* stats2,
                  const double* red2, const float* dZ, const float* D, const float* gate, const float* dpooled, float* scratch,
                  size_t scratch_floats, double* red1, float* cb1, float* part, int* nsl, hipStream_t s);
bool dw_wgrad_row_fits(const TfnasCellDesc& d);
DwPlan dw_plan_bwd_data(const TfnasCellDesc& d, bool efree, bool has_x);
int launch_dw_bwd_data(const DwPlan& p, const TfnasCellDesc& d, const float* dZ, const float* gate, const float* dpooled,
                       const float* D, const double* stats2, const double* red2, const float* E, const float* x,
                       const double* stats1, float* dEh, double* red1, float* part, hipStream_t s, float* cb1 = nullptr);
int launch_dw_bwd_dx(const TfnasCellDesc& d, const float* dZ, const float* gate, const float* dpooled, const float* D,
                     const double* stats2, const double* red2, const float* dres, float* dx, hipStream_t s);
int launch_reduce_bn1(const TfnasCellDesc& d, const float* part, int nb, const double* stats1, double* red1, float* cb1,
                      hipStream_t s);
int launch_dw_wgrad(const TfnasCellDesc& d, const float* dZ, const float* gate, const float* dpooled, const float* D,
                    const double* stats2,
                    const double* red2, const float* E, const double* stats1, float* part, hipStream_t s);

int launch_conv_fwd(const TfnasCellDesc& d, const float* x, float* D, double* stats2, float* part, hipStream_t s);
int launch_conv_dd(const TfnasCellDesc& d, const float* dZ, const float* D, const float* gate, const float* dpooled,
                   const double* stats2, const double* red2, float* dd, hipStream_t s);
int launch_conv_wgrad(const TfnasCellDesc& d, const float* dd, const float* x, float* part, hipStream_t s);
bool conv_wgrad_row_fits(const TfnasCellDesc& d);
int launch_conv_dgrad(const TfnasCellDesc& d, const float* dd, const float* dres, float* dx, float* part, hipStream_t s);

int launch_se_pool(const TfnasCellDesc& d, const float* D, const double* stats2, float* pooled, hipStream_t s);
int launch_se_fc_fwd(const TfnasCellDesc& d, const float* pooled, float* hpre, float* gate, float* scratch,
                     size_t scratch_floats, hipStream_t s);
int launch_mix_fwd(const TfnasCellDesc& d, const float* Pr, const double* stats3, const float* wmix,
                   const float* x, float* out, hipStream_t s);
int launch_mix_bwd_stats(const TfnasCellDesc& d, const float* dout, const float* Pr, const double* stats3,
                         const float* x, double* red3, float* part, hipStream_t s);
int launch_mix_dw(const TfnasCellDesc& d, const double* red3, const double* resdot, float* dwmix, hipStream_t s);
int launch_se_bwd_reduce(const TfnasCellDesc& d, const float* dZ, const float* D, const double* stats2,
                         float* dgate, hipStream_t s);
int launch_se_fc_bwd(const TfnasCellDesc& d, const float* dgate, const float* gate, const float* hpre, float* dhpre,
                     float* dpooled, float* scratch, size_t scratch_floats, hipStream_t s);
int launch_se_wgrad(const TfnasCellDesc& d, const float* dgate, const float* gate, const float* dhpre,
                    const float* hpre, const float* pooled, hipStream_t s);
bool bn2_fused_fits(const TfnasCellDesc& d);
int launch_bn2_pool(const TfnasCellDesc& d, const float* dZ, const float* D, const double* stats2, float* dgate,
                    float* pp, hipStream_t s);
int launch_bn2_gather(const TfnasCellDesc& d, const float* rec, float* dgate, float* pp, hipStream_t s);
int launch_bn2_finish(const TfnasCellDesc& d, const float* pp, const float* gate, const float* dpooled, double* red2,
                      hipStream_t s);
int launch_bn2_bwd(const TfnasCellDesc& d, const float* dZ, const float* D, const double* stats2, const float* gate,
                   const float* dpooled, double* red2, float* part, hipStream_t s);
int launch_head_pool(const TfnasCellDesc& d, const float* E, const double* stats1, float* pooled, hipStream_t s);
int launch_head_bwd(const TfnasCellDesc& d, const float* E, const double* stats1, const float* dpooled, float* dEh,
                    double* red1, float* part, hipStream_t s);
int launch_reduce_rows(const float* part, int nb, int ncols, size_t stride, double* out_d, float* out_f,
                       hipStream_t s, int accum = 0);
#define TFNAS_PART_ALLOC ((size_t)4 << 20)
#define TFNAS_TAIL_SLOTS ((size_t)1024)
#define TFNAS_PART_FLOATS (TFNAS_PART_ALLOC - TFNAS_TAIL_SLOTS)
int launch_bn1_consts(const TfnasCellDesc& d, const double* stats1, const double* red1, float* cb1,
                      hipStream_t s);

int launch_arch_fwd(int ncell, const float* const* la, const float* e, const float* lat, float T, float* w,
                    float* cell_lat, hipStream_t s);
int launch_arch_bwd(int ncell, const float* w, const float* lat, const float* dw, const float* dcl, float T,
                    float* const* dla, hipStream_t s);
int launch_arch_project(int n, float* const* p, const int32_t* len, hipStream_t s);
int launch_arch_sample(int ncell, const float* const* la, const uint8_t* mask, const float* e, float T, int mode,
                       int32_t* pos, hipStream_t s);
int launch_sink_fwd(int K, const float* betas, const float* const* res, const float* cell_lat, uint64_t count,
                    float* out, float* out_lat, float* bw, hipStream_t s);
int launch_scale_copy(float* dst, const float* src, const float* scale, uint64_t count, hipStream_t s);
int launch_sink_bwd(int K, const float* bw, const float* const* res, const float* cell_lat, const float* dout,
                    const float* dlat, uint64_t count, float* const* dres, float* dbetas, float* dcell_lat,
                    double* dots, hipStream_t s);

int launch_pack_ranges(const float* src, float* dst, int nranges, const uint64_t* off, const uint64_t* doff,
                       const uint64_t* len, hipStream_t s);
int launch_sgd_clip_step(float* w, float* g, float* m, int nranges, const uint64_t* off, const uint64_t* goff,
                         const uint64_t* len, float max_norm,
                         float lr, float momentum, float wd, float grad_scale, double* scratch, uint64_t scratch_doubles,
                         float* norm_out, hipStream_t s);
int launch_arch_adam_project(int n, float* const* p, const float* const* g, const int32_t* len, float* m, float* v,
                             float max_norm, float lr, float b1, float b2, float eps, float wd, int step, float grad_scale,
                             float* norm_out, hipStream_t s);

int launch_bn_fwd_fix(double* stats, int nch, uint64_t cnt, float eps, const float* gamma, const float* beta, float* rmean,
                      float* rvar, float momentum, int eval, hipStream_t s, uint64_t world = 1);
int launch_bn_bwd_fix(double* red, int nch, uint64_t cnt, const float* gamma, const float* beta, float* dgamma, float* dbeta,
                      hipStream_t s, int accum = 0);
int launch_rowscale(float* out, const float* y, const float* res, const float* scale, int N, uint64_t per_image,
                    hipStream_t s);
```

### tf-nas_amd/csrc/path.hip

```cpp
#include <string.h>
#include <new>
#include "tfnas_dev.h"
#include "kernels.h"
#include "cell_impl.h"

namespace {

constexpr uint64_t ALIGN = 64;
inline uint64_t up(uint64_t v) { return (v + ALIGN - 1) / ALIGN * ALIGN; }

struct CellOff {
    uint64_t E, D, Pr, fsmall, stats, out;
};
struct StageOff {
    uint64_t sink_out, bw, dots, bound;
    uint64_t count;
};
struct ScratchSet {
    uint64_t dZ, dEh, bsmall, red, part, part_w;
};

#ifndef TFNAS_LAG
#define TFNAS_LAG 2
#endif
constexpr int LAG = TFNAS_LAG;
constexpr int NSET = LAG + 1, NRING = LAG + 2;

struct PathCtx {
    int device = 0;
    bool planned = false;
    TfnasPathDesc pd;
    TfnasCellWs cws[TFNAS_MAX_CELLS];
    CellOff co[TFNAS_MAX_CELLS];
    StageOff so[TFNAS_MAX_STAGES];
    int stage_of[TFNAS_MAX_CELLS];
    ScratchSet set[NSET];
    uint64_t ring[NRING], dxp;
    TfnasPathWs ws;
    hipStream_t side = nullptr;
    bool own_side = true;
    hipEvent_t fork[TFNAS_MAX_CELLS][3];
    hipEvent_t wdone[TFNAS_MAX_CELLS];
    hipEvent_t join = nullptr;
    bool events_ok = false;
    int fwd_route[TFNAS_MAX_CELLS] = {};
};

int plan_path(PathCtx& c, const TfnasPathDesc& in, TfnasPathWs* out) {
    if (in.ncell < 1 || in.ncell > TFNAS_MAX_CELLS || in.nstage < 1 || in.nstage > TFNAS_MAX_STAGES) return TFNAS_ERANGE;
    c.planned = false;
    c.pd = in;
    memset(c.fwd_route, 0, sizeof(c.fwd_route));
    TfnasPathDesc& pd = c.pd;
    int nc = 0;
    for (int st = 0; st < pd.nstage; ++st) {
        TfnasStage& sg = pd.stage[st];
        if (sg.ncell < 1 || sg.ncell + 1 > TFNAS_MAX_SINK + 1 || (sg.start_res != 0 && sg.start_res != 1)) return TFNAS_EINVAL;
        sg.first_cell = nc;
        sg.nres = sg.ncell + 1 - sg.start_res;
        if (sg.nres < 1 || sg.nres > TFNAS_MAX_SINK) return TFNAS_ERANGE;
        if (!sg.betas) return TFNAS_ENULL;
        for (int j = 0; j < sg.ncell; ++j) c.stage_of[nc + j] = st;
        nc += sg.ncell;
    }
    if (nc != pd.ncell) return TFNAS_EINVAL;
    if (pd.reserved0 != 0) return TFNAS_EINVAL;
    for (int i = 0; i < pd.ncell; ++i) {
        TfnasCellDesc& d = pd.cell[i];
        if (d.mode != TFNAS_MODE_CELL) return TFNAS_EINVAL;
        if (cell_kind(d) != TFNAS_KIND_MBCONV) return TFNAS_EINVAL;
        if (!pd.soft && d.G != 1) return TFNAS_EINVAL;
        if (i > 0) {
            const TfnasCellDesc& p = pd.cell[i - 1];
            if (d.ic != p.oc) return TFNAS_EINVAL;
            d.N = p.N;
            d.H = p.Ho;
            d.W = p.Wo;
        }
        TRY(tfnas_cell_plan(&d));
        TRY(tfnas_cell_ws(&d, &c.cws[i]));
        const bool efree = (pd.efree_mask_lo >> i) & 1;
        if (efree && (d.need_wgrad || !efree_supported(d))) return TFNAS_EINVAL;
    }
    for (int st = 0; st < pd.nstage; ++st) {
        const TfnasStage& sg = pd.stage[st];
        const TfnasCellDesc& f = pd.cell[sg.first_cell];
        if (sg.start_res == 0 && (f.ic != f.oc || f.stride != 1)) return TFNAS_EINVAL;
        for (int j = 1; j < sg.ncell; ++j) {
            const TfnasCellDesc& d = pd.cell[sg.first_cell + j];
            if (d.ic != d.oc || d.stride != 1) return TFNAS_EINVAL;
        }
    }
    uint64_t off = 0;
    for (int k = 0; k < NSET; ++k) {
        ScratchSet& s = c.set[k];
        s.part = off; off += up(TFNAS_PART_ALLOC);
        s.part_w = off; off += up(TFNAS_PART_ALLOC);
    }
    for (int i = 0; i < pd.ncell; ++i) {
        const TfnasCellWs& w = c.cws[i];
        const bool efree = (pd.efree_mask_lo >> i) & 1;
        CellOff& o = c.co[i];
        o.E = ~(uint64_t)0;
        if (!efree) { o.E = off; off += up(w.E); }
        o.D = off; off += up(w.D);
        o.Pr = off; off += up(w.Pr);
        o.fsmall = off; off += up(w.fsmall);
        o.stats = off; off += up(2 * w.stats);
        o.out = off; off += up(w.out);
    }
    for (int st = 0; st < pd.nstage; ++st) {
        const TfnasStage& sg = pd.stage[st];
        const TfnasCellDesc& l = pd.cell[sg.first_cell + sg.ncell - 1];
        StageOff& o = c.so[st];
        o.count = (uint64_t)l.N * l.Ho * l.Wo * l.oc;
        o.sink_out = ~(uint64_t)0;
        if (st + 1 < pd.nstage) { o.sink_out = off; off += up(o.count); }
        o.bw = off; off += ALIGN;
        o.dots = off; off += ALIGN;
    }
    const uint64_t saved = off;
    uint64_t mdZ = 4, mdEh = 4, mbs = 4, mred = 4, mring = 4, mdxp = 4;
    for (int i = 0; i < pd.ncell; ++i) {
        const TfnasCellWs& w = c.cws[i];
        const TfnasCellDesc& d = pd.cell[i];
        const bool light = pd.soft && i == 0 && !pd.need_dx0 && !d.need_wgrad;
        if (!light) {
            mdZ = w.dZ > mdZ ? w.dZ : mdZ;
            mdEh = w.dEh > mdEh ? w.dEh : mdEh;
        }
        mbs = w.bsmall > mbs ? w.bsmall : mbs;
        mred = w.red > mred ? w.red : mred;
        mring = w.dx > mring ? w.dx : mring;
        mring = w.out > mring ? w.out : mring;
        mdxp = w.dxp > mdxp ? w.dxp : mdxp;
    }
    for (int k = 0; k < NSET; ++k) {
        ScratchSet& s = c.set[k];
        s.dZ = off; off += up(mdZ);
        s.dEh = off; off += up(mdEh);
        s.bsmall = off; off += up(mbs);
        s.red = off; off += up(2 * mred);
    }
    for (int k = 0; k < NRING; ++k) { c.ring[k] = off; off += up(mring); }
    c.dxp = off; off += up(mdxp);
    for (int st = 0; st + 1 < pd.nstage; ++st) { c.so[st].bound = off; off += up(c.so[st].count); }
    c.so[pd.nstage - 1].bound = ~(uint64_t)0;
    const TfnasCellDesc& last = pd.cell[pd.ncell - 1];
    c.ws.saved = saved;
    c.ws.scratch = off - saved;
    c.ws.total = off;
    c.ws.out_count = c.so[pd.nstage - 1].count;
    c.ws.out_h = last.Ho;
    c.ws.out_w = last.Wo;
    c.ws.out_c = last.oc;
    c.ws.pad = 0;
    if (out) *out = c.ws;
    c.planned = true;
    return 0;
}

inline const float* stage_input(const PathCtx& c, int st, const float* x0, const float* arena) {
    return st == 0 ? x0 : arena + c.so[st - 1].sink_out;
}

int fwd_cell(PathCtx& c, int i, const float* x0, const float* wmix, float* arena, hipStream_t s) {
    const TfnasPathDesc& pd = c.pd;
    const int st = c.stage_of[i];
    const TfnasStage& sg = pd.stage[st];
    const CellOff& o = c.co[i];
    CellFwdBufs b;
    b.x = (i == sg.first_cell) ? stage_input(c, st, x0, arena) : arena + c.co[i - 1].out;
    b.wmix = wmix ? wmix + (size_t)i * TFNAS_MAX_GROUPS : nullptr;
    b.E = o.E == ~(uint64_t)0 ? nullptr : arena + o.E;
    b.D = arena + o.D;
    b.Pr = arena + o.Pr;
    b.fsmall = arena + o.fsmall;
    b.stats = reinterpret_cast<double*>(arena + o.stats);
    b.part = arena + c.set[0].part;
    b.out = arena + o.out;
    return cell_fwd_impl(pd.cell[i], c.cws[i], b, s, &c.fwd_route[i]);
}

void sink_res(const PathCtx& c, int st, const float* x0, const float* arena, const float* res[TFNAS_MAX_SINK]) {
    const TfnasStage& sg = c.pd.stage[st];
    for (int k = 0; k < sg.nres; ++k) {
        const int r = sg.start_res + k;
        res[k] = r == 0 ? stage_input(c, st, x0, arena) : arena + c.co[sg.first_cell + r - 1].out;
    }
}

int fwd_sink(PathCtx& c, int st, const float* x0, const float* cell_lat_x, int lat_off, float* arena, float* out,
             float* out_lat, hipStream_t s) {
    const TfnasStage& sg = c.pd.stage[st];
    const float* res[TFNAS_MAX_SINK];
    sink_res(c, st, x0, arena, res);
    float* dst = (st + 1 < c.pd.nstage) ? arena + c.so[st].sink_out : out;
    return launch_sink_fwd(sg.nres, sg.betas, res, cell_lat_x ? cell_lat_x + lat_off : nullptr, c.so[st].count, dst,
                           out_lat ? out_lat + st : nullptr, arena + c.so[st].bw, s);
}

}

extern "C" int tfnas_path_create(void** ctx) {
    if (!ctx) return TFNAS_ENULL;
    PathCtx* c = new (std::nothrow) PathCtx();
    if (!c) return TFNAS_ERANGE;
    if (hipGetDevice(&c->device) != hipSuccess) { delete c; return (int)hipGetLastError(); }
    *ctx = c;
    return 0;
}

static int ensure_side(PathCtx* c) {
    if (c->events_ok) return 0;
    hipError_t e = hipSuccess;
    if (!c->side) {
        e = hipStreamCreateWithFlags(&c->side, hipStreamNonBlocking);
        c->own_side = true;
    }
    for (int i = 0; i < TFNAS_MAX_CELLS && e == hipSuccess; ++i) {
        for (int k = 0; k < 3 && e == hipSuccess; ++k) e = hipEventCreateWithFlags(&c->fork[i][k], hipEventDisableTiming);
        if (e == hipSuccess) e = hipEventCreateWithFlags(&c->wdone[i], hipEventDisableTiming);
    }
    if (e == hipSuccess) e = hipEventCreateWithFlags(&c->join, hipEventDisableTiming);
    if (e != hipSuccess) return (int)e;
    c->events_ok = true;
    return 0;
}

extern "C" int tfnas_path_destroy(void* ctx) {
    PathCtx* c = static_cast<PathCtx*>(ctx);
    if (!c) return 0;
    if (c->events_ok) {
        (void)hipStreamSynchronize(c->side);
        for (int i = 0; i < TFNAS_MAX_CELLS; ++i) {
            for (int k = 0; k < 3; ++k) (void)hipEventDestroy(c->fork[i][k]);
            (void)hipEventDestroy(c->wdone[i]);
        }
        (void)hipEventDestroy(c->join);
        if (c->own_side) (void)hipStreamDestroy(c->side);
    }
    delete c;
    return 0;
}

extern "C" int tfnas_path_set_side_stream(void* ctx, void* stream) {
    PathCtx* c = static_cast<PathCtx*>(ctx);
    if (!c || !stream) return TFNAS_ENULL;
    if (c->side && c->own_side) {
        (void)hipStreamSynchronize(c->side);
        (void)hipStreamDestroy(c->side);
    }
    c->side = S(stream);
    c->own_side = false;
    return 0;
}

static int join_sides(PathCtx* c, hipStream_t s) {
    hipError_t e = hipEventRecord(c->join, c->side);
    if (e == hipSuccess) e = hipStreamWaitEvent(s, c->join, 0);
    if (e != hipSuccess) (void)hipStreamSynchronize(c->side);
    return (int)e;
}

extern "C" int tfnas_path_plan(void* ctx, const TfnasPathDesc* pd, TfnasPathWs* ws) {
    if (!ctx || !pd) return TFNAS_ENULL;
    return plan_path(*static_cast<PathCtx*>(ctx), *pd, ws);
}

extern "C" int tfnas_path_set_wgrad_accum(void* ctx, uint32_t cell_mask) {
    PathCtx* c = static_cast<PathCtx*>(ctx);
    if (!c) return TFNAS_ENULL;
    if (!c->planned) return TFNAS_EINVAL;
    if (c->pd.ncell < 32 && (cell_mask >> c->pd.ncell) != 0) return TFNAS_ERANGE;
    for (int i = 0; i < c->pd.ncell; ++i) {
        if ((cell_mask >> i) & 1) c->pd.cell[i].flags |= TFNAS_CELL_ACCUM_WGRAD;
        else c->pd.cell[i].flags &= ~TFNAS_CELL_ACCUM_WGRAD;
    }
    return 0;
}

static int check_paths(int npath, void* const* ctx) {
    if (npath < 1 || npath > 4) return TFNAS_ERANGE;
    if (!ctx) return TFNAS_ENULL;
    for (int p = 0; p < npath; ++p) {
        const PathCtx* c = static_cast<const PathCtx*>(ctx[p]);
        if (!c) return TFNAS_ENULL;
        if (!c->planned) return TFNAS_EINVAL;
        const PathCtx* c0 = static_cast<const PathCtx*>(ctx[0]);
        if (c->pd.ncell != c0->pd.ncell || c->pd.nstage != c0->pd.nstage) return TFNAS_EINVAL;
        for (int st = 0; st < c->pd.nstage; ++st)
            if (c->pd.stage[st].ncell != c0->pd.stage[st].ncell) return TFNAS_EINVAL;
    }
    return 0;
}

extern "C" int tfnas_paths_fwd(int npath, void* const* ctx, const float* const* x0, const float* const* wmix,
                               const float* const* cell_lat, float* const* arena, float* const* out,
                               float* const* out_lat, void* const* streams) {
    TRY(check_paths(npath, ctx));
    if (!x0 || !arena || !out || !streams) return TFNAS_ENULL;
    for (int p = 0; p < npath; ++p) {
        const PathCtx* c = static_cast<const PathCtx*>(ctx[p]);
        if (!x0[p] || !arena[p] || !out[p]) return TFNAS_ENULL;
        if (c->pd.soft && (!wmix || !wmix[p])) return TFNAS_ENULL;
    }
    PathCtx* c0 = static_cast<PathCtx*>(ctx[0]);
    int lat_off = 0;
    for (int st = 0; st < c0->pd.nstage; ++st) {
        const TfnasStage& sg = c0->pd.stage[st];
        for (int j = 0; j < sg.ncell; ++j)
            for (int p = 0; p < npath; ++p) {
                PathCtx* c = static_cast<PathCtx*>(ctx[p]);
                TRY(fwd_cell(*c, sg.first_cell + j, x0[p], (wmix && c->pd.soft) ? wmix[p] : nullptr, arena[p], S(streams[p])));
            }
        for (int p = 0; p < npath; ++p) {
            PathCtx* c = static_cast<PathCtx*>(ctx[p]);
            TRY(fwd_sink(*c, st, x0[p], (cell_lat && c->pd.soft) ? cell_lat[p] : nullptr, lat_off, arena[p], out[p],
                         (out_lat && c->pd.soft) ? out_lat[p] : nullptr, S(streams[p])));
        }
        lat_off += sg.nres;
    }
    return 0;
}

namespace {

struct BwdRun {
    PathCtx* c;
    const float *x0, *wmix, *cell_lat;
    float* arena;
    const float *dout, *dout_lat;
    float *dx0, *dwmix, *dcell_lat;
    hipStream_t s;
    bool side_on;
};

int wait_wgrads(BwdRun& r, int i) {
    const int j = i + NSET;
    if (!r.side_on || j >= r.c->pd.ncell || !r.c->pd.cell[j].need_wgrad) return 0;
    return (int)hipStreamWaitEvent(r.s, r.c->wdone[j], 0);
}

int bwd_sink(BwdRun& r, int st, int lat_off) {
    PathCtx& c = *r.c;
    const TfnasStage& sg = c.pd.stage[st];
    const int last = sg.first_cell + sg.ncell - 1;
    TRY(wait_wgrads(r, last));
    const float* dsink = (st + 1 < c.pd.nstage) ? r.arena + c.so[st].bound : r.dout;
    float* dlast = r.arena + c.ring[(last + 1) % NRING];
    const float* bw = r.arena + c.so[st].bw;
    const bool want_lat = c.pd.soft && r.dcell_lat && r.cell_lat;
    if (!sg.dbetas && !want_lat) return launch_scale_copy(dlast, dsink, bw + (sg.nres - 1), c.so[st].count, r.s);
    const float* res[TFNAS_MAX_SINK];
    float* dres[TFNAS_MAX_SINK];
    sink_res(c, st, r.x0, r.arena, res);
    for (int k = 0; k < sg.nres; ++k) dres[k] = (k == sg.nres - 1) ? dlast : nullptr;
    return launch_sink_bwd(sg.nres, bw, res, want_lat ? r.cell_lat + lat_off : nullptr, dsink,
                           r.dout_lat ? r.dout_lat + st : nullptr, c.so[st].count, dres, sg.dbetas,
                           want_lat ? r.dcell_lat + lat_off : nullptr, reinterpret_cast<double*>(r.arena + c.so[st].dots),
                           r.s);
}

int bwd_cell(BwdRun& r, int i) {
    PathCtx& c = *r.c;
    const TfnasPathDesc& pd = c.pd;
    const int st = c.stage_of[i];
    const TfnasStage& sg = pd.stage[st];
    const int j = i - sg.first_cell;
    const CellOff& o = c.co[i];
    const ScratchSet& ss = c.set[i % NSET];
    if (j != sg.ncell - 1) TRY(wait_wgrads(r, i));
    CellBwdBufs b;
    b.x = (j == 0) ? stage_input(c, st, r.x0, r.arena) : r.arena + c.co[i - 1].out;
    b.wmix = (r.wmix && pd.soft) ? r.wmix + (size_t)i * TFNAS_MAX_GROUPS : nullptr;
    b.E = o.E == ~(uint64_t)0 ? nullptr : r.arena + o.E;
    b.D = r.arena + o.D;
    b.Pr = r.arena + o.Pr;
    b.fsmall = r.arena + o.fsmall;
    b.stats = reinterpret_cast<const double*>(r.arena + o.stats);
    b.dout = r.arena + c.ring[(i + 1) % NRING];
    b.dZ = r.arena + ss.dZ;
    b.dEh = r.arena + ss.dEh;
    b.bsmall = r.arena + ss.bsmall;
    b.red = reinterpret_cast<double*>(r.arena + ss.red);
    b.part = r.arena + ss.part;
    b.part_w = r.arena + ss.part_w;
    b.dxp = r.arena + c.dxp;
    b.dwmix = (r.dwmix && pd.soft) ? r.dwmix + (size_t)i * TFNAS_MAX_GROUPS : nullptr;
    if (j > 0) b.dx = r.arena + c.ring[i % NRING];
    else if (st > 0) b.dx = r.arena + c.so[st - 1].bound;
    else b.dx = pd.need_dx0 ? r.dx0 : nullptr;
    b.add_src = nullptr;
    b.add_scale = nullptr;
    if (j >= sg.start_res && b.dx) {
        b.add_src = (st + 1 < pd.nstage) ? r.arena + c.so[st].bound : r.dout;
        b.add_scale = r.arena + c.so[st].bw + (j - sg.start_res);
    }
    CellSide so = {};
    const bool side = r.side_on && pd.cell[i].need_wgrad;
    if (side) {
        for (int k = 0; k < 3; ++k) {
            so.side[k] = c.side;
            so.fork[k] = c.fork[i][k];
        }
    }
    TRY(cell_bwd_impl(pd.cell[i], c.cws[i], b, r.s, side ? &so : nullptr, c.fwd_route[i]));
    if (side) HIP_TRY(hipEventRecord(c.wdone[i], c.side));
    return 0;
}

}

extern "C" int tfnas_paths_bwd(int npath, void* const* ctx, const float* const* x0, const float* const* wmix,
                               const float* const* cell_lat, float* const* arena, const float* const* dout,
                               const float* const* dout_lat, float* const* dx0, float* const* dwmix,
                               float* const* dcell_lat, void* const* streams, int stage_begin, int stage_end) {
    TRY(check_paths(npath, ctx));
    {
        const int ns = static_cast<const PathCtx*>(ctx[0])->pd.nstage;
        if (stage_end < 0) stage_end = ns;
        if (stage_begin < 0 || stage_begin >= stage_end || stage_end > ns) return TFNAS_ERANGE;
    }
    if (!x0 || !arena || !dout || !streams) return TFNAS_ENULL;
    BwdRun run[4];
    for (int p = 0; p < npath; ++p) {
        PathCtx* c = static_cast<PathCtx*>(ctx[p]);
        if (!x0[p] || !arena[p] || !dout[p]) return TFNAS_ENULL;
        if (c->pd.need_dx0 && (!dx0 || !dx0[p])) return TFNAS_ENULL;
        if (c->pd.soft && (!wmix || !wmix[p] || !dwmix || !dwmix[p])) return TFNAS_ENULL;
        BwdRun& r = run[p];
        r.c = c;
        r.x0 = x0[p];
        r.wmix = wmix ? wmix[p] : nullptr;
        r.cell_lat = cell_lat ? cell_lat[p] : nullptr;
        r.arena = arena[p];
        r.dout = dout[p];
        r.dout_lat = dout_lat ? dout_lat[p] : nullptr;
        r.dx0 = dx0 ? dx0[p] : nullptr;
        r.dwmix = dwmix ? dwmix[p] : nullptr;
        r.dcell_lat = dcell_lat ? dcell_lat[p] : nullptr;
        r.s = S(streams[p]);
        bool any_w = false, inl = false;
        for (int i = 0; i < c->pd.ncell; ++i) {
            any_w = any_w || c->pd.cell[i].need_wgrad;
            inl = inl || !route_side(c->pd.cell[i]);
        }
        r.side_on = !inl && any_w;
        if (r.side_on) TRY(ensure_side(c));
    }
    const PathCtx* c0 = run[0].c;
    int lat_off_end = 0;
    for (int st = 0; st < c0->pd.nstage; ++st) lat_off_end += c0->pd.stage[st].nres;
    int rc = 0;
    int lat_off = lat_off_end;
    for (int st = c0->pd.nstage - 1; st >= stage_begin && rc == 0; --st) {
        const TfnasStage& sg = c0->pd.stage[st];
        lat_off -= sg.nres;
        if (st >= stage_end) continue;
        for (int p = 0; p < npath && rc == 0; ++p) rc = bwd_sink(run[p], st, lat_off);
        for (int j = sg.ncell - 1; j >= 0 && rc == 0; --j)
            for (int p = 0; p < npath && rc == 0; ++p) rc = bwd_cell(run[p], sg.first_cell + j);
    }
    for (int p = 0; p < npath; ++p) {
        BwdRun& r = run[p];
        if (!r.side_on) continue;
        const int e = join_sides(r.c, r.s);
        if (e != 0 && rc == 0) rc = e;
    }
    return rc;
}
```

### tf-nas_amd/csrc/pointwise_kernels.hip

```cpp
#include "tfnas_dev.h"
#include "kernels.h"
#include "prof.h"

__device__ __forceinline__ f32x4 reduce_rows(f32x4 v, f32x4* buf, int pr, int col, int RP, int TQ, bool active) {
    __syncthreads();
    if (active) buf[pr * TQ + col] = v;
    __syncthreads();
    int s = 1;
    while (s * 2 < RP) s *= 2;
    for (; s > 0; s >>= 1) {
        if (active && pr < s && pr + s < RP) buf[pr * TQ + col] += buf[(pr + s) * TQ + col];
        __syncthreads();
    }
    return (active && pr == 0) ? buf[col] : zero4();
}

__device__ __forceinline__ bool chunk_locate(const TfnasCellDesc& d, int cy, int CH, bool se_only, int& g, int& c0) {
    for (g = 0; g < d.G; ++g) {
        if (se_only && d.g[g].se == 0) continue;
        const int t = (d.g[g].mcp + CH - 1) / CH;
        if (cy < t) {
            c0 = cy * CH;
            return true;
        }
// ... 196 lines not shown
                        const float dh = (v[u][j] - c2[j].x) * c2[j].y;
                        const float ad = act_d<ACT>(dh), zd = z[u][j] * ad;
                        a1[j] += zd;
                        b1[j] += zd * dh;
                        if (has_se) {
                            g0[j] += z[u][j] * act_f<ACT>(dh);
                            a2[j] += ad;
                            b2[j] += ad * dh;
                        }
                    }
                }
            }
        }
    }
    const size_t NM = (size_t)d.N * M, o = (size_t)n * M + off + ch;
    a1 = reduce_rows(a1, buf, rl, cq, RLN, CQN, active);
    if (active && rl == 0) st4(pp + o, a1);
    b1 = reduce_rows(b1, buf, rl, cq, RLN, CQN, active);
    if (active && rl == 0) st4(pp + NM + o, b1);
    if (has_se) {
        a2 = reduce_rows(a2, buf, rl, cq, RLN, CQN, active);
        if (active && rl == 0) st4(pp + 2 * NM + o, a2);
        b2 = reduce_rows(b2, buf, rl, cq, RLN, CQN, active);
        if (active && rl == 0) st4(pp + 3 * NM + o, b2);
        g0 = reduce_rows(g0, buf, rl, cq, RLN, CQN, active);
        if (active && rl == 0) st4(dgate + o, g0);
    }
}

__global__ __launch_bounds__(256) void k_bn2_gather(TfnasCellDesc d, const float* __restrict__ rec, float* __restrict__ dgate,
                                                    float* __restrict__ pp) {
    __shared__ double sh[4][FOLD_Q][64];
    int g, c0;
    if (!chunk_locate(d, blockIdx.y, 64, false, g, c0)) return;
    const int mcp = d.g[g].mcp, off = d.g[g].off;
    const bool has_se = d.g[g].se > 0;
    const int HW = d.Ho * d.Wo, M = d.M, n = blockIdx.x, Po = d.N * HW;
    const int tid = threadIdx.x, cl = tid & 63, part = tid >> 6;
    const bool active = c0 + cl < mcp;
    const int t0 = (n * HW) >> 7, t1 = ((n + 1) * HW - 1) >> 7;
    const int nq = has_se ? FOLD_Q : 2;
    double acc[FOLD_Q] = {0, 0, 0, 0, 0};
    if (active) {
        constexpr int U = 8;
        for (int t = t0 + part; t <= t1; t += 4 * U) {
            float v[U][FOLD_Q];
#pragma unroll
            for (int u = 0; u < U; ++u) {
                const int tt = min(t + 4 * u, t1);
                const int slot = n - min(tt * 128, Po - 1) / HW;
                const float* r = rec + (((size_t)tt * FOLD_SLOTS + slot) * FOLD_Q) * M + off + c0 + cl;
#pragma unroll
                for (int q = 0; q < FOLD_Q; ++q) v[u][q] = q < nq ? r[(size_t)q * M] : 0.f;
            }
#pragma unroll
            for (int u = 0; u < U; ++u) {
                const bool ok = t + 4 * u <= t1;
#pragma unroll
                for (int q = 0; q < FOLD_Q; ++q)
                    if (q < nq) acc[q] += ok ? (double)v[u][q] : 0.0;
            }
        }
    }
#pragma unroll
    for (int q = 0; q < FOLD_Q; ++q) sh[part][q][cl] = acc[q];
    __syncthreads();
    if (part == 0 && active) {
        const size_t NM = (size_t)d.N * M, o = (size_t)n * M + off + c0 + cl;
        double v[FOLD_Q];
#pragma unroll
        for (int q = 0; q < FOLD_Q; ++q) v[q] = ((sh[0][q][cl] + sh[1][q][cl]) + sh[2][q][cl]) + sh[3][q][cl];
        pp[o] = (float)v[0];
        pp[NM + o] = (float)v[1];
        if (has_se) {
            dgate[o] = (float)v[2];
            pp[2 * NM + o] = (float)v[3];
            pp[3 * NM + o] = (float)v[4];
        }
    }
}

__global__ __launch_bounds__(256) void k_bn2_finish(TfnasCellDesc d, const float* __restrict__ pp,
                                                    const float* __restrict__ gate, const float* __restrict__ dpooled,
                                                    double* __restrict__ red2) {
    __shared__ double sh[2][16][65];
    int g, c0;
    if (!chunk_locate(d, blockIdx.x, 64, false, g, c0)) return;
    const int mc = d.g[g].mc, mcp = d.g[g].mcp, off = d.g[g].off;
    const bool has_se = d.g[g].se > 0;
    const int M = d.M, N = d.N;
    const int tid = threadIdx.x, cq = tid & 15, rl = tid >> 4;
    const int ch = c0 + 4 * cq;
    const bool active = ch < mcp;
    const size_t NM = (size_t)N * M;
    const float inv_hw = 1.f / (float)(d.Ho * d.Wo);
    double r1[4] = {0, 0, 0, 0}, r2[4] = {0, 0, 0, 0};
    if (active) {
        for (int n = rl; n < N; n += 16) {
            const size_t o = (size_t)n * M + off + ch;
            f32x4 x1 = ld4(pp + o), y1 = ld4(pp + NM + o);
            if (has_se) {
                const f32x4 gt = ld4(gate + o), dp = ld4(dpooled + o) * splat4(inv_hw);
                x1 = gt * x1 + dp * ld4(pp + 2 * NM + o);
                y1 = gt * y1 + dp * ld4(pp + 3 * NM + o);
            }
#pragma unroll
            for (int j = 0; j < 4; ++j) {
                r1[j] += (double)x1[j];
                r2[j] += (double)y1[j];
            }
        }
    }
#pragma unroll
    for (int j = 0; j < 4; ++j) {
        sh[0][rl][4 * cq + j] = r1[j];
        sh[1][rl][4 * cq + j] = r2[j];
    }
    __syncthreads();
    if (tid < 128) {
        const int which = tid >> 6, cl = tid & 63;
        if (c0 + cl < mc) {
            double t = 0.0;
#pragma unroll
            for (int r = 0; r < 16; ++r) t += sh[which][r][cl];
            red2[2 * (size_t)(off + c0 + cl) + which] = t;
        } else if (c0 + cl < mcp) {
            red2[2 * (size_t)(off + c0 + cl) + which] = 0.0;
        }
    }
}

template <int ACT>
__global__ __launch_bounds__(256) void k_bn2_bwd(TfnasCellDesc d, const float* __restrict__ dZ, const float* __restrict__ D,
                                                 const double* __restrict__ stats2, const float* __restrict__ gate,
                                                 const float* __restrict__ dpooled, float* __restrict__ part,
                                                 int rows_per_block) {
    __shared__ f32x4 buf[256];
    int g, c0;
    if (!chunk_locate(d, blockIdx.y, 64, false, g, c0)) return;
    const int mc = d.g[g].mc, mcp = d.g[g].mcp, off = d.g[g].off;
    const bool has_se = d.g[g].se > 0;
    const int HW = d.Ho * d.Wo, Po = d.N * HW, M = d.M;
    const int tid = threadIdx.x, cq = tid & 15, rl = tid >> 4;
    const int ch = c0 + 4 * cq;
    const bool active = ch < mcp;
    float2 c2[4];
#pragma unroll
    for (int j = 0; j < 4; ++j)
        c2[j] = (active && ch + j < mc) ? bn_consts(stats2 + 2 * (size_t)(off + ch + j), 1.0 / (double)Po, d.eps)
                                        : make_float2(0.f, 0.f);
    const float inv_hw = 1.f / (float)HW;
    const int p0 = blockIdx.x * rows_per_block, p1 = min(Po, p0 + rows_per_block);
    f32x4 r1 = zero4(), r2 = zero4();
    if (active) {
        for (int pb = p0 + rl; pb < p1; pb += 64) {
            f32x4 da[4], dv[4], gt[4], dp[4];
#pragma unroll
            for (int u = 0; u < 4; ++u) {
                const int p = pb + 16 * u < p1 ? pb + 16 * u : pb;
                const size_t a = (size_t)p * M + off + ch;
                da[u] = ld4_nt(dZ + a);
                dv[u] = ld4_nt(D + a);
                if (has_se) {
                    const size_t b = (size_t)(p / HW) * M + off + ch;
                    gt[u] = ld4(gate + b);
                    dp[u] = ld4(dpooled + b);
                }
            }
#pragma unroll
            for (int u = 0; u < 4; ++u) {
                const int p = pb + 16 * u;
                if (p < p1) {
                    if (has_se) da[u] = da[u] * gt[u] + dp[u] * splat4(inv_hw);
                    f32x4 ddh;
#pragma unroll
                    for (int j = 0; j < 4; ++j) {
                        const float dh = (dv[u][j] - c2[j].x) * c2[j].y;
                        ddh[j] = da[u][j] * act_d<ACT>(dh);
                        r1[j] += ddh[j];
                        r2[j] += ddh[j] * dh;
                    }
                }
            }
        }
    }
    r1 = reduce_rows(r1, buf, rl, cq, 16, 16, active);
    r2 = reduce_rows(r2, buf, rl, cq, 16, 16, active);
    if (active && rl == 0) {
        float* prow = part + (size_t)blockIdx.x * 2 * M + 2 * (size_t)(off + ch);
#pragma unroll
        for (int j = 0; j < 4; ++j) {
            prow[2 * j + 0] = r1[j];
            prow[2 * j + 1] = r2[j];
        }
    }
}

__global__ void k_bn1_consts(TfnasCellDesc d, const double* __restrict__ stats1, const double* __restrict__ red1,
                             float* __restrict__ cb1) {
    const int c = blockIdx.x * blockDim.x + threadIdx.x;
    if (c >= d.M) return;
    const double inv = 1.0 / ((double)d.N * d.H * d.W);
    const float2 m = bn_consts(stats1 + 2 * (size_t)c, inv, d.eps);
    f32x4 t;
    t.x = m.x;
    t.y = m.y;
    t.z = (float)(red1[2 * (size_t)c + 0] * inv);
    t.w = (float)(red1[2 * (size_t)c + 1] * inv);
    bool is_pad = true;
    for (int g = 0; g < d.G; ++g)
        if (c >= d.g[g].off && c < d.g[g].off + d.g[g].mc) is_pad = false;
// ... 268 lines not shown
                         float* dgate, hipStream_t s) {
    ProfScope _prof(TK_SE_BWD_REDUCE, s);
    const int chunks = chunk_count(d, 64, true);
    if (!chunks) return 0;
    dim3 grid(d.N, chunks);
    ACT_DISPATCH(d.act, {
        hipLaunchKernelGGL((k_se_pool<ACT, 1>), grid, dim3(256), 0, s, d, D, stats2, dZ, dgate);
    })
    return (int)hipGetLastError();
}

int launch_mix_fwd(const TfnasCellDesc& d, const float* Pr, const double* stats3, const float* wmix,
                   const float* x, float* out, hipStream_t s) {
    ProfScope _prof(TK_MIX_FWD, s);
    const size_t total = (size_t)d.N * d.Ho * d.Wo * (d.oc / 4);
    size_t blocks = cdiv64(total, 256 * 4);
    if (blocks > 4096) blocks = 4096;
    if (blocks < 1) blocks = 1;
    const size_t shm = (size_t)2 * d.G * d.oc * sizeof(float);
    hipLaunchKernelGGL(k_mix_fwd, dim3((unsigned)blocks), dim3(256), shm, s, d, Pr, stats3, wmix, x, out);
    return (int)hipGetLastError();
}

int launch_mix_bwd_stats(const TfnasCellDesc& d, const float* dout, const float* Pr, const double* stats3,
                         const float* x, double* red3, float* part, hipStream_t s) {
    ProfScope _prof(TK_MIX_BWD_STATS, s);
    const int Po = d.N * d.Ho * d.Wo;
    const int ncols = 2 * d.G * d.oc + d.oc;
    size_t nblk = 1024;
    if (nblk > TFNAS_PART_FLOATS / (size_t)ncols) nblk = TFNAS_PART_FLOATS / (size_t)ncols;
    int rpb = cdiv(Po, (int)nblk);
    const int RP = 256 / (d.oc / 4);
    if (rpb < 8 * RP) rpb = 8 * RP;
    const size_t shm = (size_t)(2 * d.G * d.oc + 4 * 256) * sizeof(float);
    const int gx = cdiv(Po, rpb);
    hipLaunchKernelGGL(k_mix_bwd_stats, dim3(gx), dim3(256), shm, s, d, dout, Pr, stats3, x, part, rpb);
    _prof.stop();
    return launch_reduce_rows(part, gx, ncols, (size_t)ncols, red3, nullptr, s);
}

int launch_mix_dw(const TfnasCellDesc& d, const double* red3, const double* resdot, float* dwmix, hipStream_t s) {
    ProfScope _prof(TK_SMALL, s);
    hipLaunchKernelGGL(k_mix_dw, dim3(d.G), dim3(64), 0, s, d, red3, resdot, dwmix);
    return (int)hipGetLastError();
}

int launch_bn2_bwd(const TfnasCellDesc& d, const float* dZ, const float* D, const double* stats2, const float* gate,
                   const float* dpooled, double* red2, float* part, hipStream_t s) {
    ProfScope _prof(TK_BN2_BWD, s);
    const int Po = d.N * d.Ho * d.Wo;
    const int chunks = chunk_count(d, 64, false);
    int want = cdiv(4096, chunks);
    if (want > 1024) want = 1024;
    const size_t cap = TFNAS_PART_FLOATS / (2 * (size_t)d.M);
    if ((size_t)want > cap) want = (int)cap;
    int rpb = cdiv(Po, want < 1 ? 1 : want);
    if (rpb < 64) rpb = 64;
    dim3 grid(cdiv(Po, rpb), chunks);
    ACT_DISPATCH(d.act, {
        hipLaunchKernelGGL((k_bn2_bwd<ACT>), grid, dim3(256), 0, s, d, dZ, D, stats2, gate, dpooled, part, rpb);
    })
    _prof.stop();
    return launch_reduce_rows(part, grid.x, 2 * d.M, 2 * (size_t)d.M, red2, nullptr, s);
}

bool bn2_fused_fits(const TfnasCellDesc& d) { return 4 * (size_t)d.N * d.M <= TFNAS_PART_FLOATS; }

int launch_bn2_pool(const TfnasCellDesc& d, const float* dZ, const float* D, const double* stats2, float* dgate,
                    float* pp, hipStream_t s) {
    ProfScope _prof(TK_SE_BWD_REDUCE, s);
    const int CH = (d.N * chunk_count(d, 64, false) < 1024 && d.Ho * d.Wo >= 196) ? 32 : 64;
    dim3 grid(d.N, chunk_count(d, CH, false));
    ACT_DISPATCH(d.act, { hipLaunchKernelGGL((k_bn2_pool<ACT>), grid, dim3(256), 0, s, d, dZ, D, stats2, dgate, pp, CH); })
    return (int)hipGetLastError();
}

int launch_bn2_gather(const TfnasCellDesc& d, const float* rec, float* dgate, float* pp, hipStream_t s) {
    ProfScope _prof(TK_SE_BWD_REDUCE, s);
    hipLaunchKernelGGL(k_bn2_gather, dim3(d.N, chunk_count(d, 64, false)), dim3(256), 0, s, d, rec, dgate, pp);
    return (int)hipGetLastError();
}

int launch_bn2_finish(const TfnasCellDesc& d, const float* pp, const float* gate, const float* dpooled, double* red2,
                      hipStream_t s) {
    ProfScope _prof(TK_BN2_BWD, s);
    hipLaunchKernelGGL(k_bn2_finish, dim3(chunk_count(d, 64, false)), dim3(256), 0, s, d, pp, gate, dpooled, red2);
    return (int)hipGetLastError();
}

int launch_head_pool(const TfnasCellDesc& d, const float* E, const double* stats1, float* pooled, hipStream_t s) {
    ProfScope _prof(TK_SMALL, s);
    dim3 grid(d.N, cdiv(d.g[0].mcp, 64));
    ACT_DISPATCH(d.act, { hipLaunchKernelGGL((k_head_pool<ACT>), grid, dim3(256), 0, s, d, E, stats1, pooled); })
    return (int)hipGetLastError();
}

int launch_head_bwd(const TfnasCellDesc& d, const float* E, const double* stats1, const float* dpooled, float* dEh,
                    double* red1, float* part, hipStream_t s) {
    ProfScope _prof(TK_SMALL, s);
    if ((size_t)d.N * 2 * d.M > TFNAS_PART_FLOATS) return TFNAS_ERANGE;
    dim3 grid(d.N, cdiv(d.g[0].mcp, 64));
    ACT_DISPATCH(d.act, { hipLaunchKernelGGL((k_head_bwd<ACT>), grid, dim3(256), 0, s, d, E, stats1, dpooled, dEh, part); })
    _prof.stop();
    return launch_reduce_rows(part, d.N, 2 * d.M, 2 * (size_t)d.M, red1, nullptr, s);
}

int launch_bn1_consts(const TfnasCellDesc& d, const double* stats1, const double* red1, float* cb1,
                      hipStream_t s) {
    ProfScope _prof(TK_SMALL, s);
    hipLaunchKernelGGL(k_bn1_consts, dim3(cdiv(d.M, 256)), dim3(256), 0, s, d, stats1, red1, cb1);
    return (int)hipGetLastError();
}
```

### tf-nas_amd/tfnas_amd/_lib.py

```python
import collections
import ctypes as C
import os

import torch

_HERE = os.path.dirname(os.path.abspath(__file__))
LIB_PATH = os.environ.get('TFNAS_LIB') or os.path.join(_HERE, 'libtfnas_hip.so')

MAX_GROUPS, MAX_SINK, MAX_CELLS = 8, 4, 32
ACT = {'relu': 0, 'swish': 1, 'relu6': 2, 'h-swish': 3}
MODE_CELL, MODE_STEM, MODE_HEAD = 0, 1, 2
BN_EPS = 1e-5

_W_FIELDS = ('w_expand', 'w_dw', 'w_proj', 'w_se_r', 'b_se_r', 'w_se_e', 'b_se_e')
_G_FIELDS = ('g_expand', 'g_dw', 'g_proj', 'g_se_r', 'gb_se_r', 'g_se_e', 'gb_se_e')


GEMM_EXPLICIT, GEMM_EVERYWHERE, CELL_LAZY_JOIN = 0x1000, 0x100, 1
CELL_ACCUM_WGRAD = 0x20
CELL_K7 = 0x80
CELL_ACTS = 0x100
CELL_NOEXPAND = 0x200
CELL_FUSED = 0x400
ROUTE_FX_OFF, ROUTE_FOLD_OFF, ROUTE_DWWG_OFF, ROUTE_DWWG2_OFF, ROUTE_XG_OFF, ROUTE_XG_ALL = 0x1, 0x2, 0x4, 0x8, 0x10, 0x20
ROUTE_DW = {'auto': 0, 'direct': 1 << 6, 'lds': 2 << 6, 'tiled': 3 << 6}
ROUTE_SE = {'wave': 0, 'fused': 1 << 8, 'gemm': 2 << 8}
ROUTE_WGRAD_INLINE, ROUTE_GRAM2 = 0x400, 0x800
ROUTE_TAKEN_VALID, ROUTE_TAKEN_FX = 1, 2
GEMM_MODES = {'f32': 0, 'bf16': 1, 'x2': 3, 'x3': 6}


def act_id(name):
    try:
        return ACT[name]
    except (KeyError, TypeError):
        raise ValueError('tfnas_amd: unknown activation %r (one of %s)' % (name, ', '.join(repr(a) for a in ACT))) from None


def act_flags(act):
    return CELL_ACTS if act in (ACT['relu6'], ACT['h-swish']) else 0


class BlockKind(collections.namedtuple('BlockKind', 'name flag fields bn_sites has_E')):
    __slots__ = ()

    def bound(self, se):
        return self.fields if se else tuple(k for k in self.fields if k < 3)


MBCONV = BlockKind('MBCONV', 0, (0, 1, 2, 3, 4, 5, 6), (0, 1, 2), True)
NOEXPAND = BlockKind('NOEXPAND', CELL_NOEXPAND, (1, 2, 3, 4, 5, 6), (1, 2), False)
FUSED = BlockKind('FUSED', CELL_FUSED, (0, 2, 3, 4, 5, 6), (1, 2), False)
KINDS = (MBCONV, NOEXPAND, FUSED)


def describe_block(kind, N, H, W, ic, mc, se, oc, k, stride, act):
    d = TfnasCellDesc()
    d.N, d.H, d.W, d.ic, d.oc, d.stride, d.act, d.G, d.mode = N, H, W, ic, oc, stride, act, 1, MODE_CELL
    d.has_res, d.eps = int(ic == oc and stride == 1), BN_EPS
    d.g[0].mc, d.g[0].k, d.g[0].se = mc, k, se
    d.flags = (CELL_K7 if k == 7 else 0) | act_flags(act) | kind.flag
    return d


class TfnasGroup(C.Structure):
    _fields_ = ([(n, C.c_int32) for n in ('mc', 'k', 'se', 'mcp', 'off', 'se_off', 'pad0', 'pad1')]
                + [(n, C.c_void_p) for n in _W_FIELDS] + [(n, C.c_void_p) for n in _G_FIELDS])


class TfnasCellDesc(C.Structure):
    _fields_ = ([(n, C.c_int32) for n in ('N', 'H', 'W', 'ic', 'oc', 'stride', 'act', 'has_res', 'G', 'need_wgrad',
                                          'Ho', 'Wo', 'M', 'SE')]
                + [('eps', C.c_float), ('mode', C.c_int32), ('Hi', C.c_int32), ('Wi', C.c_int32),
                   ('stor', C.c_int32), ('gemm_mode', C.c_int32), ('flags', C.c_int32), ('g', TfnasGroup * MAX_GROUPS),
                   ('sync_fn', C.c_void_p), ('sync_user', C.c_void_p), ('sync_world', C.c_int32), ('route', C.c_int32),
                   ('fwd_route', C.c_int32), ('pad_route', C.c_int32), ('wgrad_stream', C.c_void_p * 3)])


class TfnasCellWs(C.Structure):
    _fields_ = [(n, C.c_uint64) for n in (
        'E', 'D', 'Pr', 'fsmall', 'off_pooled', 'off_gate', 'off_hpre', 'stats', 'off_stats1', 'off_stats2',
        'off_stats3', 'out', 'dZ', 'dEh', 'bsmall', 'off_dgate', 'off_dpooled', 'off_dgl', 'off_dhpre', 'off_cb1',
        'red', 'off_red3', 'off_red2', 'off_red1', 'off_resdot', 'part', 'dx', 'dxp')]


MAX_STAGES = 8


class TfnasStage(C.Structure):
    _fields_ = ([(n, C.c_int32) for n in ('ncell', 'start_res', 'first_cell', 'nres')]
                + [('betas', C.c_void_p), ('dbetas', C.c_void_p)])


class TfnasPathDesc(C.Structure):
    _fields_ = ([(n, C.c_int32) for n in ('ncell', 'nstage', 'soft', 'need_dx0', 'efree_mask_lo', 'reserved0')]
                + [('stage', TfnasStage * MAX_STAGES), ('cell', TfnasCellDesc * MAX_CELLS)])


class TfnasPathWs(C.Structure):
    _fields_ = ([(n, C.c_uint64) for n in ('saved', 'scratch', 'total', 'out_count')]
                + [(n, C.c_int32) for n in ('out_h', 'out_w', 'out_c', 'pad')])


class TfnasBnAffine(C.Structure):
    _fields_ = ([(n, C.c_void_p * 3) for n in ('weight', 'bias', 'g_weight', 'g_bias', 'running_mean', 'running_var')]
                + [('momentum', C.c_float), ('eval', C.c_int32)])


_P = C.c_void_p
_PP = C.POINTER(C.c_void_p)
_PROTOS = {
    'tfnas_abi_version': (C.c_int, []),
    'tfnas_shutdown': (C.c_int, []),
    'tfnas_sizeof': (C.c_uint64, [C.c_int]),
    'tfnas_cell_plan': (C.c_int, [C.POINTER(TfnasCellDesc)]),
    'tfnas_cell_ws': (C.c_int, [C.POINTER(TfnasCellDesc), C.POINTER(TfnasCellWs)]),
    'tfnas_mixedop_fwd': (C.c_int, [C.POINTER(TfnasCellDesc)] + [_P] * 10),
    'tfnas_mixedop_bwd': (C.c_int, [C.POINTER(TfnasCellDesc)] + [_P] * 17),
    'tfnas_mbconv_fwd': (C.c_int, [C.POINTER(TfnasCellDesc), C.POINTER(TfnasBnAffine)] + [_P] * 10),
    'tfnas_mbconv_bwd': (C.c_int, [C.POINTER(TfnasCellDesc), C.POINTER(TfnasBnAffine)] + [_P] * 17),
    'tfnas_head_affine_fwd': (C.c_int, [C.POINTER(TfnasCellDesc), C.POINTER(TfnasBnAffine)] + [_P] * 6),
    'tfnas_head_affine_bwd': (C.c_int, [C.POINTER(TfnasCellDesc), C.POINTER(TfnasBnAffine)] + [_P] * 11),
    'tfnas_head_fwd': (C.c_int, [C.POINTER(TfnasCellDesc)] + [_P] * 6),
    'tfnas_head_bwd': (C.c_int, [C.POINTER(TfnasCellDesc)] + [_P] * 11),
    'tfnas_head_wgrad': (C.c_int, [C.POINTER(TfnasCellDesc)] + [_P] * 6),
    'tfnas_cls_ce': (C.c_int, [C.c_int, C.c_int, C.c_int, _P, _P, _P, _P, C.c_float, _P, _P, _P, _P, _P]),
    'tfnas_cls_wgrad': (C.c_int, [C.c_int, C.c_int, C.c_int, C.c_int, _PP, _PP, _PP, C.c_float, _P, _P, _P, _P]),
    'tfnas_cls_wgrad_ex': (C.c_int, [C.c_int, C.c_int, C.c_int, C.c_int, _PP, _PP, _PP, _P, C.c_float, _P, _P, _P, _P, _P]),
    'tfnas_cls_ce_ex': (C.c_int, [C.c_int, C.c_int, C.c_int, _P, _P, _P, _P, C.c_float, C.c_float, _P, _P, _P, _P, _P, _P]),
    'tfnas_cls_reduce': (C.c_int, [C.c_int, C.c_int, C.c_int, _P, _P, _P, _P, _P, C.c_int, _P, _P, _P, _P, _P]),
    'tfnas_add_into': (C.c_int, [_P, _P, C.c_uint64, _P]),
    'tfnas_path_create': (C.c_int, [C.POINTER(C.c_void_p)]),
    'tfnas_path_destroy': (C.c_int, [C.c_void_p]),
    'tfnas_path_set_side_stream': (C.c_int, [C.c_void_p, C.c_void_p]),
    'tfnas_path_set_wgrad_accum': (C.c_int, [C.c_void_p, C.c_uint32]),
    'tfnas_set_stats_sync': (C.c_int, [C.c_void_p, C.c_void_p, C.c_int]),
    'tfnas_path_plan': (C.c_int, [C.c_void_p, C.POINTER(TfnasPathDesc), C.POINTER(TfnasPathWs)]),
    'tfnas_paths_fwd': (C.c_int, [C.c_int] + [_PP] * 8),
    'tfnas_paths_bwd': (C.c_int, [C.c_int] + [_PP] * 11 + [C.c_int, C.c_int]),
    'tfnas_pack_ranges': (C.c_int, [_P, _P, C.c_int, C.POINTER(C.c_uint64), C.POINTER(C.c_uint64), C.POINTER(C.c_uint64), _P]),
    'tfnas_sgd_clip_step': (C.c_int, [_P, _P, _P, C.c_int, C.POINTER(C.c_uint64), C.POINTER(C.c_uint64),
                                      C.POINTER(C.c_uint64), C.c_float, C.c_float,
                                      C.c_float, C.c_float, C.c_float, _P, C.c_uint64, _P, _P]),
    'tfnas_arch_adam_project': (C.c_int, [C.c_int, _PP, _PP, C.POINTER(C.c_int32), _P, _P, C.c_float, C.c_float, C.c_float,
                                          C.c_float, C.c_float, C.c_float, C.c_int, C.c_float, _P, _P]),
    'tfnas_arch_fwd': (C.c_int, [C.c_int, C.POINTER(_P), _P, _P, C.c_float, _P, _P, _P]),
    'tfnas_arch_bwd': (C.c_int, [C.c_int, _P, _P, _P, _P, C.c_float, C.POINTER(_P), _P]),
    'tfnas_efree_supported': (C.c_int, [C.POINTER(TfnasCellDesc)]),
    'tfnas_fx_supported': (C.c_int, [C.POINTER(TfnasCellDesc)]),
    'tfnas_cell_route': (C.c_int, [C.POINTER(TfnasCellDesc)]),
    'tfnas_arch_project': (C.c_int, [C.c_int, C.POINTER(_P), C.POINTER(C.c_int32), _P]),
    'tfnas_arch_sample': (C.c_int, [C.c_int, C.POINTER(_P), _P, _P, C.c_float, C.c_int, _P, _P]),
    'tfnas_sink_fwd': (C.c_int, [C.c_int, _P, C.POINTER(_P), _P, C.c_uint64, _P, _P, _P, _P]),
    'tfnas_prof_enable': (C.c_int, [C.c_uint]),
    'tfnas_set_lazy_join': (C.c_int, [C.c_int]),
    'tfnas_set_gemm_mode': (C.c_int, [C.c_int]),
    'tfnas_gemm_mode': (C.c_int, []),
    'tfnas_side_stream': (C.c_int, [_P, C.POINTER(C.c_void_p)]),
    'tfnas_side_join': (C.c_int, [_P]),
    'tfnas_prof_count': (C.c_int, []),
    'tfnas_prof_name': (C.c_char_p, [C.c_int]),
    'tfnas_prof_collect': (C.c_int, [C.c_int, C.POINTER(C.c_uint64), C.POINTER(C.c_double)]),
    'tfnas_prof_last_split': (C.c_int, [C.c_int, C.POINTER(C.c_uint64), C.POINTER(C.c_double)]),
    'tfnas_sink_bwd': (C.c_int, [C.c_int, _P, C.POINTER(_P), _P, _P, _P, C.c_uint64, C.POINTER(_P), _P, _P, _P, _P]),
}

_lib_handle = None


def lib():
    global _lib_handle
    l = _lib_handle
    if l is None:
        path = LIB_PATH
        if not os.path.exists(path):
            raise RuntimeError(
                'tfnas_amd: HIP extension %s is missing -- run `python -c "import __graft_entry__ as g; g.build()"` '
                '(or `make -C tf-nas_amd/csrc`). There is no CPU/PyTorch fallback for the MixedOP hot path.' % path)
        l = C.CDLL(path)
        for name, (res, args) in _PROTOS.items():
            fn = getattr(l, name)
            fn.restype, fn.argtypes = res, args
        if l.tfnas_abi_version() != 4:
            raise RuntimeError('tfnas_amd: ABI version mismatch')
        for which, st in enumerate((TfnasGroup, TfnasCellDesc, TfnasCellWs, TfnasStage, TfnasPathDesc, TfnasPathWs, TfnasBnAffine)):
            if l.tfnas_sizeof(which) != C.sizeof(st):
                raise RuntimeError('tfnas_amd: struct layout mismatch for %s' % st.__name__)
        g = os.environ.get('TFNAS_GEMM')
        if g is not None:
            if g not in GEMM_MODES:
                raise RuntimeError('tfnas_amd: TFNAS_GEMM must be one of %s' % sorted(GEMM_MODES))
            if l.tfnas_set_gemm_mode(GEMM_MODES[g]) != 0:
                raise RuntimeError('tfnas_amd: tfnas_set_gemm_mode failed')
        _lib_handle = l
    return l


def check(rc, what):
    if rc != 0:
        raise RuntimeError('tfnas_hip: %s failed with code %d (%s)' % (
            what, rc, 'invalid argument' if rc < 0 else 'hipError_t'))


def ptr(t):
    return None if t is None else C.c_void_p(t.data_ptr())


def ptr_array(tensors):
    arr = (C.c_void_p * len(tensors))()
    for i, t in enumerate(tensors):
        arr[i] = None if t is None else t.data_ptr()
    return arr


def raw_array(values):
    arr = (C.c_void_p * len(values))()
    for i, v in enumerate(values):
        arr[i] = v
    return arr


def exported_names():
    return list(_PROTOS)
```

### tf-nas_amd/tfnas_amd/functions.py

```python
import ctypes as C
import os

import torch

from . import _lib
from ._lib import TfnasCellDesc, TfnasCellWs, ptr, ptr_array, check

BN_EPS = _lib.BN_EPS
_EFREE_ENV = os.environ.get('TFNAS_EFREE', '1')
EFREE = _EFREE_ENV != '0'
EFREE_STRIDE1 = _EFREE_ENV == 'all'


def route_from_env(env=None):
    env = os.environ if env is None else env
    r = 0
    for var, bit in (('TFNAS_FX', _lib.ROUTE_FX_OFF), ('TFNAS_FOLD', _lib.ROUTE_FOLD_OFF), ('TFNAS_DWWG', _lib.ROUTE_DWWG_OFF),
                     ('TFNAS_DWWG2', _lib.ROUTE_DWWG2_OFF), ('TFNAS_WGRAD_STREAM', _lib.ROUTE_WGRAD_INLINE)):
        if env.get(var, '1')[:1] == '0':
            r |= bit
    xg = env.get('TFNAS_XG', 'auto')
    r |= _lib.ROUTE_XG_OFF if xg[:1] == '0' else (_lib.ROUTE_XG_ALL if xg == 'all' else 0)
    r |= _lib.ROUTE_DW.get(env.get('TFNAS_DW', 'auto'), 0) | _lib.ROUTE_SE.get(env.get('TFNAS_SE', 'wave'), 0)
    if env.get('TFNAS_GRAM', '1') == '2':
        r |= _lib.ROUTE_GRAM2
    return r


def route_bits(fx=True, fold=True, dwwg=True, dwwg2=True, xg='auto', dw='auto', se='wave', wgrad_stream=True, gram=1):
    return route_from_env({'TFNAS_FX': '1' if fx else '0', 'TFNAS_FOLD': '1' if fold else '0', 'TFNAS_DWWG': '1' if dwwg else '0',
                           'TFNAS_DWWG2': '1' if dwwg2 else '0', 'TFNAS_XG': xg, 'TFNAS_DW': dw, 'TFNAS_SE': se,
                           'TFNAS_WGRAD_STREAM': '1' if wgrad_stream else '0', 'TFNAS_GRAM': str(gram)})


ENV_ROUTE = route_from_env()


def _stream(dev):
    return C.c_void_p(torch.cuda.current_stream(dev).cuda_stream)


class _Null:
    def __enter__(self):
        return None

    def __exit__(self, *a):
        return False


_NULL = _Null()


def _on(dev):
    return _NULL if torch.cuda.current_device() == dev.index else torch.cuda.device(dev)


def _same_device(dev, tensors, what):
    for t in tensors:
        if t is not None and t.device != dev:
            raise RuntimeError('tfnas_amd: %s lives on %s but the input is on %s -- all operands of a launch must share '
                               'one device (one process per GPU; nn.DataParallel replicas must own their parameters)'
                               % (what, t.device, dev))


def _nhwc(x):
    v = x.permute(0, 2, 3, 1)
    return v if v.is_contiguous() else v.contiguous()


def _require_cuda(t, what):
    if not t.is_cuda:
        raise RuntimeError('tfnas_amd: %s must live on the GPU -- the MixedOP hot path has no CPU implementation '
                           '(the CPU restatement is oracle/tfnas_oracle.py, test infrastructure only)' % what)
    if t.dtype != torch.float32:
        raise RuntimeError('tfnas_amd: %s must be float32' % what)


def _no_plan():
    return None


class HipModes:

    def __init__(self, gemm=None, everywhere=False, lazy_join=False, direct_grads=False, sync=None, route=None):
        self.gemm, self.everywhere, self.lazy_join, self.direct_grads, self.sync = gemm, everywhere, lazy_join, direct_grads, sync
        self.route = route

    def __deepcopy__(self, memo):
        return HipModes(self.gemm, self.everywhere, self.lazy_join, self.direct_grads, None, self.route)

    def __getstate__(self):
        st = dict(self.__dict__)
        st['sync'] = None
        return st

    def apply(self, d, kind=None):
        d.gemm_mode = 0 if self.gemm is None else (_lib.GEMM_EXPLICIT | _lib.GEMM_MODES[self.gemm]
                                                   | (_lib.GEMM_EVERYWHERE if self.everywhere else 0))
        d.flags = _lib.CELL_LAZY_JOIN if self.lazy_join else 0
        if any(d.g[g].k == 7 for g in range(min(d.G, _lib.MAX_GROUPS))):
            d.flags |= _lib.CELL_K7
        d.flags |= _lib.act_flags(d.act)
        if kind is None:
            kind = _lib.NOEXPAND if (d.mode == _lib.MODE_CELL and d.G == 1 and d.g[0].mc == d.ic) else _lib.MBCONV
        d.flags |= kind.flag
        d.route = ENV_ROUTE if self.route is None else int(self.route)
        if self.sync is None:
            d.sync_fn, d.sync_user, d.sync_world = None, None, 0
        else:
            d.sync_fn, d.sync_user, d.sync_world = self.sync[0], self.sync[1], int(self.sync[2])


DEFAULT_MODES = HipModes()


def adopt_modes(root, modes=None):
    modes = modes if modes is not None else HipModes()
    for m in root.modules():
        object.__setattr__(m, 'hip_modes', modes)
    return modes


class CellPlan:

    def __reduce__(self):
        return (_no_plan, ())

    def __deepcopy__(self, memo):
        return None

    def __init__(self, ic, oc, stride, act, blocks, mode=_lib.MODE_CELL, modes=None):
        self.ic, self.oc, self.stride, self.act = ic, oc, stride, act
        self.blocks = list(blocks)
        kinds = [getattr(b, 'kind', _lib.MBCONV) for b in self.blocks]
        if _lib.FUSED in kinds and (len(self.blocks) != 1 or mode != _lib.MODE_CELL):
            raise NotImplementedError('tfnas_amd: a FusedMBConvBlock runs as a one-block cell only (not as a candidate of a '
                                      'multi-candidate MixedOP launch, a stem or a head)')
        self.kind = kinds[0] if (mode == _lib.MODE_CELL and len(self.blocks) == 1) else _lib.MBCONV
        self._kind_arg = () if self.kind is _lib.MBCONV else (self.kind,)
        slots = []
        for g, (b, kind) in enumerate(zip(self.blocks, kinds)):
            fields = (0,) if mode == _lib.MODE_HEAD else (kind if mode == _lib.MODE_CELL else _lib.MBCONV).bound(b.se_channels > 0)
            slots += [(g, k) for k in fields]
        self._w_slots = [(g, _lib._W_FIELDS[k]) for g, k in slots]
        self._g_slots = [(g, _lib._G_FIELDS[k]) for g, k in slots]
        self._modes = modes
        self.mode = mode
        self.has_res = int(mode == _lib.MODE_CELL and ic == oc and stride == 1)
        self._desc_cache = {}
        self.grad_targets = None
        self.wgrad_streams = None

    def params(self):
        ps = []
        for b in self.blocks:
            ps.extend(b.hip_params())
        return ps

    @property
    def modes(self):
        m = self._modes if self._modes is not None else getattr(self.blocks[0], 'hip_modes', None)
        return m if m is not None else DEFAULT_MODES

    def desc(self, N, H, W):
        key = (N, H, W)
        hit = self._desc_cache.get(key)
        if hit is None:
            d = TfnasCellDesc()
            d.N, d.H, d.W, d.ic, d.oc, d.stride = N, H, W, self.ic, self.oc, self.stride
            d.mode = self.mode
            if self.mode == _lib.MODE_STEM:
                d.Hi, d.Wi = H, W
            d.act, d.has_res, d.G, d.need_wgrad, d.eps = _lib.act_id(self.act), self.has_res, len(self.blocks), 0, BN_EPS
            for g, b in enumerate(self.blocks):
                d.g[g].mc, d.g[g].k, d.g[g].se = b.mid_channels, b.kernel_size, b.se_channels
            self.modes.apply(d, *self._kind_arg)
            check(_lib.lib().tfnas_cell_plan(C.byref(d)), 'tfnas_cell_plan')
            ws = TfnasCellWs()
            check(_lib.lib().tfnas_cell_ws(C.byref(d), C.byref(ws)), 'tfnas_cell_ws')
            hit = (d, ws)
            self._desc_cache[key] = hit
        self.modes.apply(hit[0], *self._kind_arg)
        return hit

    def bind(self, d, params, grads=None):
        for (g, f), p in zip(self._w_slots, params):
            setattr(d.g[g], f, p.data_ptr())
        if grads is not None:
            for (g, f), t in zip(self._g_slots, grads):
                setattr(d.g[g], f, t.data_ptr())
        d.need_wgrad = int(grads is not None)


def _cell_forward(ctx, plan, xh, N, H, W, wmix, params):
    d, ws = plan.desc(N, H, W)
    for p in params:
        _require_cuda(p, 'MBConv weight')
        if not p.is_contiguous():
            raise RuntimeError('tfnas_amd: MBConv weights must be contiguous')
    plan.bind(d, params)
    d.need_wgrad = int(any(ctx.needs_input_grad[3:]))
    ctx.fwd_route = int(_lib.lib().tfnas_cell_route(C.byref(d)))
    dev = xh.device
    _same_device(dev, list(params) + [wmix], 'a MixedOP weight / mix weight')
    efree = (EFREE and ((plan.stride == 2 and plan.ic <= 24) or EFREE_STRIDE1) and not any(ctx.needs_input_grad[3:])
             and bool(_lib.lib().tfnas_efree_supported(C.byref(d))))
    E = None if (efree or ws.E == 0) else torch.empty(ws.E, device=dev, dtype=torch.float32)
    D = torch.empty(ws.D, device=dev, dtype=torch.float32)
    Pr = torch.empty(ws.Pr, device=dev, dtype=torch.float32)
    fsmall = torch.empty(ws.fsmall, device=dev, dtype=torch.float32)
    stats = torch.empty(ws.stats, device=dev, dtype=torch.float64)
    part = _part(ws.part, dev)
    out = torch.empty((N, d.Ho, d.Wo, plan.oc), device=dev, dtype=torch.float32)
    if wmix is not None:
        wmix = wmix.contiguous()
    with _on(dev):
        check(_lib.lib().tfnas_mixedop_fwd(C.byref(d), ptr(xh), ptr(wmix), ptr(E), ptr(D), ptr(Pr), ptr(fsmall),
                                           ptr(stats), ptr(part), ptr(out), _stream(dev)), 'tfnas_mixedop_fwd')
    d.need_wgrad = 0
    ctx.plan, ctx.shape, ctx.has_w = plan, (N, H, W), wmix is not None
    if MixedOpFn.fwd_sink is not None:
        MixedOpFn.fwd_sink.append(dict(plan=plan, d=d, ws=ws, E=E, D=D, stats=stats, fsmall=fsmall, shape=(N, d.H, d.W)))
    ctx.save_for_backward(xh, wmix, E, D, Pr, fsmall, stats, *params)
    return out.permute(0, 3, 1, 2)


def _cell_backward(ctx, dout, want_dx):
    xh, wmix, E, D, Pr, fsmall, stats, *params = ctx.saved_tensors
    plan = ctx.plan
    N, H, W = ctx.shape
    d, ws = plan.desc(N, H, W)
    dev = xh.device
    need_w = any(ctx.needs_input_grad[3:])
    direct = plan.grad_targets if need_w else None
    if direct is not None and (len(direct) != len(params) or any(g.shape != p.shape or g.device != p.device or not g.is_contiguous()
                                                                 for g, p in zip(direct, params))):
        raise RuntimeError('tfnas_amd: grad_targets do not match the parameters of this launch')
    grads = (list(direct) if direct is not None else [torch.empty_like(p) for p in params]) if need_w else None
    plan.bind(d, params, grads)
    douth = _nhwc(dout)
    light = not want_dx and not need_w
    dZ = torch.empty(4 if light else ws.dZ, device=dev, dtype=torch.float32)
    dEh = torch.empty(4 if light else ws.dEh, device=dev, dtype=torch.float32)
    bsmall = torch.empty(ws.bsmall, device=dev, dtype=torch.float32)
    red = torch.empty(ws.red, device=dev, dtype=torch.float64)
    ws_streams = plan.wgrad_streams if need_w else None
    part = _part(ws.part * (4 if ws_streams else (2 if need_w else 1)), dev)
    dx = torch.empty((N, d.H, d.W, plan.ic), device=dev, dtype=torch.float32) if want_dx else None
    dxp = torch.empty(ws.dxp, device=dev, dtype=torch.float32) if want_dx else None
    dwmix = torch.empty(d.G, device=dev, dtype=torch.float32) if ctx.has_w else None
    _same_device(dev, [douth], 'the output gradient')
    d.fwd_route = getattr(ctx, 'fwd_route', 0)
    for k in range(3):
        d.wgrad_stream[k] = ws_streams[k].cuda_stream if (ws_streams and ws_streams[k] is not None) else None
    try:
        with _on(dev):
            check(_lib.lib().tfnas_mixedop_bwd(C.byref(d), ptr(xh), ptr(wmix), ptr(E), ptr(D), ptr(Pr), ptr(fsmall),
                                               ptr(stats), ptr(douth), ptr(dZ), ptr(dEh), ptr(bsmall), ptr(red),
                                               ptr(part), ptr(dx), ptr(dxp), ptr(dwmix), _stream(dev)), 'tfnas_mixedop_bwd')
    finally:
        d.need_wgrad = 0
        d.fwd_route = 0
        for k in range(3):
            d.wgrad_stream[k] = None
    if MixedOpFn.debug_sink is not None:
        MixedOpFn.debug_sink.append(dict(dZ=dZ, dEh=dEh, bsmall=bsmall, red=red, ws=ws, d=d))
# ... 379 lines not shown
```

### tf-nas_amd/tfnas_amd/model_search.py

```python
import os
import weakref
import random

import torch
import torch.nn as nn
import torch.nn.functional as F

from . import _lib
from .functions import ArchFn, CellPlan, HeadFn, MixedOpFn, SinkFn, StemFn, arch_sample
from .layers import ConvLayer, LinearLayer, MBInvertedResBlock

PRIMITIVES = [
    'MBI_k3_e3', 'MBI_k3_e6', 'MBI_k5_e3', 'MBI_k5_e6',
    'MBI_k3_e3_se', 'MBI_k3_e6_se', 'MBI_k5_e3_se', 'MBI_k5_e6_se',
]

_OP_SPEC = {
    'MBI_k3_e3': (3, 0), 'MBI_k3_e6': (3, 0), 'MBI_k5_e3': (5, 0), 'MBI_k5_e6': (5, 0),
    'MBI_k3_e3_se': (3, 1), 'MBI_k3_e6_se': (3, 2), 'MBI_k5_e3_se': (5, 1), 'MBI_k5_e6_se': (5, 2),
}

OPS = {
    name: (lambda ic, mc, oc, s, aff, act, _k=k, _se=se:
           MBInvertedResBlock(ic, mc, ic * _se, oc, _k, s, affine=aff, act_func=act))
    for name, (k, se) in _OP_SPEC.items()
}

_SAMPLE_MODES = {'gumbel': 0, 'gumbel_2': 0, 'min_alphas': 1, 'max_alphas': 2}


class MixedOP(nn.Module):
    def __init__(self, in_channels, out_channels, stride, affine, act_func, num_ops, mc_num_dict, lat_lookup):
        super().__init__()
        self.num_ops = num_ops
        self.lat_lookup = lat_lookup
        self.mc_num_dict = mc_num_dict
        self.in_channels, self.out_channels, self.stride, self.act_func = in_channels, out_channels, stride, act_func
        self.m_ops = nn.ModuleList()
        for i in range(num_ops):
            self.m_ops.append(OPS[PRIMITIVES[i]](in_channels, self.mc_num_dict[i], out_channels, stride, affine,
                                                 act_func))
        self._initialize_log_alphas()
        self.reset_switches()
        self.T = 1.0
        self._plans = {}
        self._lat_cache = {}
        self._pre = None

    def fink_ori_idx(self, idx):
        count = 0
        for ori_idx in range(len(self.switches)):
            if self.switches[ori_idx]:
                count += 1
                if count == (idx + 1):
                    break
        return ori_idx

    def get_lookup_latency(self, size):
        lats = []
        for op in self.m_ops:
            key = '{}_{}_{}_{}_{}_k{}_s{}_{}'.format(op.name, size, op.in_channels, op.se_channels, op.out_channels,
                                                     op.kernel_size, op.stride, op.act_func)
            lats.append(self.lat_lookup[key][op.mid_channels])
        return lats

    def _initialize_log_alphas(self):
        self.register_parameter('log_alphas', nn.Parameter(F.log_softmax(torch.zeros((self.num_ops,)), dim=-1)))

    def reset_switches(self):
        self.switches = [True] * self.num_ops

    def set_temperature(self, T):
        self.T = T

    def _plan(self, idxs):
        key = tuple(idxs)
        p = self._plans.get(key)
        if p is not None and p.blocks[0] is not self.m_ops[key[0]]:
            self._plans, p = {}, None
        if p is None:
            p = CellPlan(self.in_channels, self.out_channels, self.stride, self.act_func,
                         [self.m_ops[i] for i in idxs])
            self._plans[key] = p
        return p

    def lat_tensor(self, size, device):
        key = (size, str(device), tuple(op.mid_channels for op in self.m_ops))
        t = self._lat_cache.get(key)
        if t is None:
            t = torch.tensor(self.get_lookup_latency(size), dtype=torch.float32, device=device)
            self._lat_cache = {key: t}
        return t

    def sample_index(self, mode, exp_noise=None, rand_pos=None, pos=None):
        nactive = sum(self.switches)
        if mode in _SAMPLE_MODES:
            if pos is None:
                if mode.startswith('gumbel') and exp_noise is None:
                    exp_noise = torch.empty(8, device=self.log_alphas.device).exponential_()
                pos = arch_sample([self.log_alphas], [[int(s) for s in self.switches]],
                                  None if exp_noise is None else exp_noise.reshape(1, -1)[:, :8], self.T,
                                  _SAMPLE_MODES[mode])[0]
            if not 0 <= pos < nactive:
                raise ValueError('sampled position %d outside the %d switched-on candidates' % (pos, nactive))
            if mode == 'gumbel':
                idx = pos
                self.switches[idx] = False
            else:
                idx = self.fink_ori_idx(pos)
                self.reset_switches()
        elif mode == 'random':
            p = random.choice(range(nactive)) if rand_pos is None else int(rand_pos)
            if not 0 <= p < nactive:
                raise ValueError('random position %d outside the %d switched-on candidates' % (p, nactive))
            idx = self.fink_ori_idx(p)
            self.reset_switches()
        else:
            raise ValueError('invalid sampling mode...')
        return idx

    def forward(self, x, sampling, mode, exp_noise=None, rand_pos=None):
        pre, self._pre = self._pre, None
        if sampling:
            idx = pre if pre is not None else self.sample_index(mode, exp_noise, rand_pos)
            self.last_idx = idx
            op = self.m_ops[idx]
            return MixedOpFn.apply(self._plan((idx,)), x, None, *op.hip_params()), 0
        if pre is not None:
            w, out_lat = pre
        else:
            if exp_noise is None:
                exp_noise = torch.empty(8, device=x.device).exponential_()
            lat = self.lat_tensor(x.size(-1), x.device)
            W, CL = ArchFn.apply(exp_noise.reshape(1, 8).to(x.device), lat.reshape(1, 8), self.T, self.log_alphas)
            w, out_lat = W[0], CL[0]
        plan = self._plan(tuple(range(self.num_ops)))
        out = MixedOpFn.apply(plan, x, w, *plan.params())
        self.last_w = w
        return out, out_lat


class MixedStage(nn.Module):
    def __init__(self, ics, ocs, ss, affs, acts, mc_num_ddict, lat_lookup, stage_type):
        super().__init__()
        self.lat_lookup = lat_lookup
        self.mc_num_ddict = mc_num_ddict
        self.stage_type = stage_type
        self.start_res = 0 if ((ics[0] == ocs[0]) and (ss[0] == 1)) else 1
        self.num_res = len(ics) - self.start_res + 1
        nblocks = {0: 1, 1: 2, 2: 3, 3: 4}.get(stage_type)
        if nblocks is None:
            raise ValueError('invalid stage_type...')
        self.nblocks = nblocks
        for b in range(nblocks):
            setattr(self, 'block%d' % (b + 1),
                    MixedOP(ics[b], ocs[b], ss[b], affs[b], acts[b], len(PRIMITIVES), mc_num_ddict['block%d' % (b + 1)],
                            lat_lookup))
        self._initialize_betas()

    def blocks(self):
        return [getattr(self, 'block%d' % (b + 1)) for b in range(self.nblocks)]

    def forward(self, x, sampling, mode, exp_noise=None, rand_pos=None):
        res_list, lat_list = [x], []
        for b, blk in enumerate(self.blocks()):
# ... 26 lines not shown
    def __init__(self, num_classes, mc_num_dddict, lat_lookup):
        super().__init__()
        self.lat_lookup = lat_lookup
        self.mc_num_dddict = mc_num_dddict

        self.first_stem = ConvLayer(3, 32, kernel_size=3, stride=2, affine=False, act_func='relu')
        self.second_stem = MBInvertedResBlock(32, 32, 8, 16, kernel_size=3, stride=1, affine=False, act_func='relu')
        cfg = [
            ('stage1', [16, 24], [24, 24], [2, 1], 'relu', 1),
            ('stage2', [24, 40, 40], [40, 40, 40], [2, 1, 1], 'swish', 2),
            ('stage3', [40, 80, 80, 80], [80, 80, 80, 80], [2, 1, 1, 1], 'swish', 3),
            ('stage4', [80, 112, 112, 112], [112, 112, 112, 112], [1, 1, 1, 1], 'swish', 3),
            ('stage5', [112, 192, 192, 192], [192, 192, 192, 192], [2, 1, 1, 1], 'swish', 3),
            ('stage6', [192], [320], [1], 'swish', 0),
        ]
        self._stage_names = [c[0] for c in cfg]
        for name, ics, ocs, ss, act, st in cfg:
            setattr(self, name, MixedStage(ics=ics, ocs=ocs, ss=ss, affs=[False] * len(ics), acts=[act] * len(ics),
                                           mc_num_ddict=mc_num_dddict[name], lat_lookup=lat_lookup, stage_type=st))
        self.feature_mix_layer = ConvLayer(320, 1280, kernel_size=1, stride=1, affine=False, act_func='swish')
        self.global_avg_pooling = nn.AdaptiveAvgPool2d(1)
        self.classifier = LinearLayer(1280, num_classes)
        self._initialization()
        self._cells = None
        self._lat_stack = None
        self._stem_plan = None
        self._head_plan = None
        from .functions import adopt_modes
        adopt_modes(self)

    def set_hip_modes(self, **kw):
        for k, v in kw.items():
            if not hasattr(self.hip_modes, k):
                raise AttributeError(k)
            setattr(self.hip_modes, k, v)

    class _StemBlock:

        def __init__(self, first, second):
            self.first, self.second = first, second
            self.mid_channels, self.kernel_size, self.se_channels = second.mid_channels, second.kernel_size, second.se_channels

        def hip_params(self):
            se = self.second.squeeze_excite
            return [self.first.conv.weight, self.second.depth_conv.conv.weight, self.second.point_linear.conv.weight,
                    se.conv_reduce.weight, se.conv_reduce.bias, se.conv_expand.weight, se.conv_expand.bias]

    class _HeadBlock:
        def __init__(self, conv_layer):
            self.layer = conv_layer
            self.mid_channels, self.kernel_size, self.se_channels = conv_layer.out_channels, 3, 0

        def hip_params(self):
            return [self.layer.conv.weight]

    def stem_plan(self):
        fs, ss = self.first_stem, self.second_stem
        if (fs.kernel_size, fs.stride, fs.in_channels, fs.act_func, ss.act_func, ss.stride) != (3, 2, 3, 'relu', 'relu', 1) \
                or ss.inverted_bottleneck is not None or ss.squeeze_excite is None:
            raise NotImplementedError('stem geometry differs from models/model_search.py:219-220')
        if self._stem_plan is None:
            self._stem_plan = CellPlan(27, ss.out_channels, 1, 'relu', [Network._StemBlock(fs, ss)], mode=_lib.MODE_STEM, modes=self.hip_modes)
        return self._stem_plan

    def _stem(self, x):
        plan = self.stem_plan()
        return StemFn.apply(plan, x, None, *plan.params())

    def head_plan(self):
        fm = self.feature_mix_layer
        if self._head_plan is None:
            self._head_plan = CellPlan(fm.in_channels, 4, 1, fm.act_func, [Network._HeadBlock(fm)], mode=_lib.MODE_HEAD, modes=self.hip_modes)
        return self._head_plan

    def _head(self, x):
        return HeadFn.apply(self.head_plan(), x, self.feature_mix_layer.conv.weight)

    def stages(self):
        return [getattr(self, n) for n in self._stage_names]

    def cells(self):
        if self._cells is None:
            self._cells = [blk for st in self.stages() for blk in st.blocks()]
        return self._cells

    def arch_weights(self, size, dev, exp_noise=None):
        cells = self.cells()
        if exp_noise is None:
            exp_noise = torch.empty(len(cells), 8, device=dev).exponential_()
        key = (size, str(dev), tuple(op.mid_channels for c in cells for op in c.m_ops))
        if self._lat_stack is None or self._lat_stack[0] != key:
            lats = []
            for st in self.stages():
                for blk in st.blocks():
                    lats.append(blk.lat_tensor(size, dev))
                    size = (size - 1) // blk.stride + 1
            self._lat_stack = (key, torch.stack(lats))
        T = cells[0].T
        if any(c.T != T for c in cells):
            raise ValueError('all MixedOPs must share one temperature (Network.set_temperature)')
        return ArchFn.apply(exp_noise.to(dev), self._lat_stack[1], T, *[c.log_alphas for c in cells])

    def _prepare(self, x, sampling, mode, exp_noise, rand_pos, pos=None):
        cells = self.cells()
        n = len(cells)
        dev = x.device
        if not sampling:
            W, CL = self.arch_weights(x.size(-1), dev, exp_noise)
            for c, w_c, cl_c in zip(cells, W.unbind(0), CL.unbind(0)):
                c._pre = (w_c, cl_c)
            return
        if mode in _SAMPLE_MODES:
            if pos is not None:
                if len(pos) != n:
                    raise ValueError('pos must hold one position per MixedOP')
                self._require_all_switches_on()
                for i, c in enumerate(cells):
                    c._pre = c.sample_index(mode, pos=int(pos[i]))
                return
            if mode.startswith('gumbel') and exp_noise is None:
                exp_noise = torch.empty(n, 8, device=dev).exponential_()
            pos = arch_sample([c.log_alphas for c in cells], [[int(s) for s in c.switches] for c in cells],
                              None if exp_noise is None else exp_noise.to(dev), cells[0].T, _SAMPLE_MODES[mode])
            for i, c in enumerate(cells):
                c._pre = c.sample_index(mode, pos=pos[i])
        elif mode == 'random':
            for i, c in enumerate(cells):
                c._pre = c.sample_index(mode, rand_pos=None if rand_pos is None else rand_pos[i])
        else:
            raise ValueError('invalid sampling mode...')

    def _require_all_switches_on(self):
        if not all(all(c.switches) for c in self.cells()):
            raise RuntimeError('host-sampled positions need every switch on: call reset_switches() first')

    def stem_features(self, x):
        return self._stem(x)

    def forward_bisample(self, x, pos_g, rand_pos, side_stream):
        cells = self.cells()
        if len(pos_g) != len(cells) or len(rand_pos) != len(cells):
            raise ValueError('pos_g / rand_pos must hold one entry per MixedOP')
        self._require_all_switches_on()
        cur = torch.cuda.current_stream(x.device)
        feat = self._stem(x)
        side_stream.wait_stream(cur)
        feat.record_stream(side_stream)
        xa = xb = feat
        ci = 0
        for st in self.stages():
            ra, rb = [xa], [xb]
            for blk in st.blocks():
                ia = blk.sample_index('gumbel', pos=int(pos_g[ci]))
                ib = blk.sample_index('random', rand_pos=rand_pos[ci])
                blk.last_idx = ib
                ra.append(MixedOpFn.apply(blk._plan((ia,)), ra[-1], None, *blk.m_ops[ia].hip_params()))
                with torch.cuda.stream(side_stream):
                    rb.append(MixedOpFn.apply(blk._plan((ib,)), rb[-1], None, *blk.m_ops[ib].hip_params()))
                ci += 1
            xa, _ = SinkFn.apply(st.betas, None, *ra[st.start_res:])
            with torch.cuda.stream(side_stream):
                xb, _ = SinkFn.apply(st.betas, None, *rb[st.start_res:])
        la = self.classifier(self._head(xa))
        with torch.cuda.stream(side_stream):
            lb = self.classifier(self._head(xb))
        return la, lb

# ... 166 lines not shown
```

Before: 3890.

## Fuse column sums into Gram pass for centred inputs and keep FX constants

Cells whose input is known to be zero-mean (centred, from BN-output without residual) skip the separate column-sum kernel and its reduction. The Gram kernel now accumulates the raw column sums alongside the Gram matrix in one pass, and stats1 skips the mean correction. Separately, the backward BN2 finish kernel writes per-channel BN constants into a kept FX buffer so the FX backward can reuse them instead of recomputing. This adds arena space and relies on the centred-input assumption holding for the numerical stability of uncentred Gram sums.

```diff
diff --git a/include/tfnas_hip.h b/include/tfnas_hip.h
--- a/include/tfnas_hip.h
+++ b/include/tfnas_hip.h
@@ -71,6 +71,7 @@
 #define TFNAS_CELL_ACTS 0x100
 #define TFNAS_CELL_NOEXPAND 0x200
 #define TFNAS_CELL_FUSED 0x400
+#define TFNAS_CELL_CENTRED 0x800
 #define TFNAS_ROUTE_FX_OFF 0x1
 #define TFNAS_ROUTE_FOLD_OFF 0x2
 #define TFNAS_ROUTE_DWWG_OFF 0x4
@@ -83,7 +84,8 @@
 #define TFNAS_ROUTE_SE_MASK 0x300
 #define TFNAS_ROUTE_WGRAD_INLINE 0x400
 #define TFNAS_ROUTE_GRAM2 0x800
-#define TFNAS_ROUTE_ALL 0xfff
+#define TFNAS_ROUTE_FXH_OFF 0x2000
+#define TFNAS_ROUTE_ALL 0x2fff
 #define TFNAS_ROUTE_TAKEN_VALID 0x1
 #define TFNAS_ROUTE_TAKEN_FX 0x2
 
@@ -123,6 +125,7 @@
 int tfnas_efree_supported(const TfnasCellDesc *d);
 int tfnas_cell_route(const TfnasCellDesc *d);
 int tfnas_fx_supported(const TfnasCellDesc *d);
+uint64_t tfnas_fx_keep_floats(const TfnasCellDesc *d);
 
 int tfnas_mixedop_fwd(const TfnasCellDesc *d, const float *x, const float *wmix,
                       float *E, float *D, float *Pr, float *fsmall, double *stats, float *part,
@@ -228,6 +231,7 @@
 int tfnas_path_destroy(void *ctx);
 int tfnas_path_set_side_stream(void *ctx, void *stream);
 int tfnas_path_plan(void *ctx, const TfnasPathDesc *pd, TfnasPathWs *ws);
+int tfnas_path_centred_cells(const TfnasPathDesc *pd, uint32_t *mask);
 int tfnas_path_set_wgrad_accum(void *ctx, uint32_t cell_mask);
 
 int tfnas_paths_fwd(int npath, void *const *ctx, const float *const *x0, const float *const *wmix,
diff --git a/tf-nas_amd/csrc/capi.hip b/tf-nas_amd/csrc/capi.hip
--- a/tf-nas_amd/csrc/capi.hip
+++ b/tf-nas_amd/csrc/capi.hip
@@ -157,7 +157,7 @@
         if (!(d->gemm_mode & TFNAS_GEMM_EXPLICIT) || (gm != 0 && gm != 1 && gm != 3 && gm != 6)) return TFNAS_EINVAL;
     }
     if (d->flags & ~(TFNAS_CELL_LAZY_JOIN | TFNAS_CELL_ACCUM_WGRAD | TFNAS_CELL_K7 | TFNAS_CELL_ACTS | TFNAS_CELL_NOEXPAND |
-                     TFNAS_CELL_FUSED))
+                     TFNAS_CELL_FUSED | TFNAS_CELL_CENTRED))
         return TFNAS_EINVAL;
     TRY(check_kind(d));
     if (!(d->flags & TFNAS_CELL_K7)) {
@@ -259,6 +259,7 @@
 
 extern "C" int tfnas_efree_supported(const TfnasCellDesc* dp) { return (dp && efree_supported(*dp)) ? 1 : 0; }
 extern "C" int tfnas_fx_supported(const TfnasCellDesc* dp) { return (dp && fx_supported(*dp)) ? 1 : 0; }
+extern "C" uint64_t tfnas_fx_keep_floats(const TfnasCellDesc* dp) { return dp ? (uint64_t)fx_keep_floats(*dp) : 0; }
 static int route_taken(const TfnasCellDesc& d, bool affine) {
     return TFNAS_ROUTE_TAKEN_VALID | ((!affine && fx_supported(d)) ? TFNAS_ROUTE_TAKEN_FX : 0);
 }
@@ -291,7 +292,7 @@
     else TRY(launch_expand_stats_gram(d, b.x, stats1, b.part, s));
     if (sync) TRY(stats_sync(d, stats1, 2 * (size_t)d.M, s));
     if (bn) TRY(bn_fwd_fix(d0, bn, 0, stats1, s));
-    if (fx) TRY(launch_fx_fwd(d, b.x, stats1, b.E, b.D, stats2, b.part, s));
+    if (fx) TRY(launch_fx_fwd(d, b.x, stats1, b.E, b.D, stats2, b.part, s, b.fx_keep));
     else TRY(launch_dw_fwd(d, b.E, b.x, stats1, b.D, stats2, b.part, s));
     return 0;
 }
@@ -416,7 +417,9 @@
         else TRY(launch_se_bwd_reduce(d, b.dZ, b.D, stats2, dgate, s));
     }
     TRY(launch_se_fc_bwd(d, dgate, gate, hpre, dhpre, dpooled, b.dEh, (size_t)ws.dEh, s));
-    if (fused2) TRY(launch_bn2_finish(d, part, gate, dpooled, red2, s));
+    const bool fx_kept = (taken & TFNAS_ROUTE_TAKEN_FX) && b.fx_keep;
+    if (fx_kept && !fused2) return TFNAS_EINVAL;
+    if (fused2) TRY(launch_bn2_finish(d, part, gate, dpooled, red2, s, stats2, fx_keep_cst2(d, fx_kept ? b.fx_keep : nullptr)));
     else TRY(launch_bn2_bwd(d, b.dZ, b.D, stats2, gate, dpooled, red2, part, s));
     TRY(stats_sync(d, red2, 2 * (size_t)d.M, s));
     if (bn) TRY(bn_bwd_fix(d0, bn, 1, red2, s));
@@ -453,7 +456,8 @@
 int CellBwd::tail_mbconv() {
     if (taken & TFNAS_ROUTE_TAKEN_FX) {
         int nsl = 0;
-        TRY(launch_fx_bwd(d, b.x, b.E, stats1, stats2, red2, b.dZ, b.D, gate, dpooled, b.dEh, (size_t)ws.dEh, red1, cb1, part, &nsl, s));
+        TRY(launch_fx_bwd(d, b.x, b.E, stats1, stats2, red2, b.dZ, b.D, gate, dpooled, b.dEh, (size_t)ws.dEh, red1, cb1, part, &nsl, s,
+                          b.fx_keep));
         if (b.dx) TRY(expand_dx(d, nullptr, b.x, cb1, part, dout_res, b.wmix, b.dx, b.dEh, s, b.add_src, b.add_scale, nsl));
         return 0;
     }
diff --git a/tf-nas_amd/csrc/cell_impl.h b/tf-nas_amd/csrc/cell_impl.h
--- a/tf-nas_amd/csrc/cell_impl.h
+++ b/tf-nas_amd/csrc/cell_impl.h
@@ -19,6 +19,7 @@
     float* out;
     const TfnasBnAffine* bn = nullptr;
     const float* drop_scale = nullptr;
+    float* fx_keep = nullptr;
 };
 
 struct CellBwdBufs {
@@ -35,6 +36,7 @@
     const float* drop_scale = nullptr;
     float* dout_s = nullptr;
     float *part_w1 = nullptr, *part_w2 = nullptr;
+    float* fx_keep = nullptr;
 };
 
 struct CellSide {
diff --git a/tf-nas_amd/csrc/efree_kernels.hip b/tf-nas_amd/csrc/efree_kernels.hip
--- a/tf-nas_amd/csrc/efree_kernels.hip
+++ b/tf-nas_amd/csrc/efree_kernels.hip
@@ -35,14 +35,17 @@
 __global__ __launch_bounds__(256) void k_x_gram(const float* __restrict__ x, int P, int ic, int rps,
                                                 const double* __restrict__ xsum, float* __restrict__ part) {
     __shared__ float red[4][CT * CT][4][64 + 1];
+    __shared__ float csum[4][CT * 16];
     const int tid = threadIdx.x, lane = tid & 63, wave = tid >> 6, n = lane & 15, q = lane >> 4;
     const int r0 = blockIdx.x * rps, r1 = min(P, r0 + rps);
-    float mu[CT];
+    const bool raw = xsum == nullptr;
+    float mu[CT], cs[CT];
     bool chok[CT];
 #pragma unroll
     for (int t = 0; t < CT; ++t) {
         chok[t] = 16 * t + n < ic;
-        mu[t] = chok[t] ? (float)(xsum[16 * t + n] / (double)P) : 0.f;
+        mu[t] = (!raw && chok[t]) ? (float)(xsum[16 * t + n] / (double)P) : 0.f;
+        cs[t] = 0.f;
     }
     f32x4 acc[CT][CT];
 #pragma unroll
@@ -65,6 +68,10 @@
 #pragma unroll
                 for (int j = 0; j < CT; ++j)
                     acc[i][j] = __builtin_amdgcn_mfma_f32_16x16x4f32(a[u][i], a[u][j], acc[i][j], 0, 0, 0);
+#pragma unroll
+        for (int u = 0; u < 4; ++u)
+#pragma unroll
+            for (int t = 0; t < CT; ++t) cs[t] += a[u][t];
     }
 #pragma unroll
     for (int i = 0; i < CT; ++i)
@@ -72,17 +79,25 @@
         for (int j = 0; j < CT; ++j)
 #pragma unroll
             for (int r = 0; r < 4; ++r) red[wave][i * CT + j][r][lane] = acc[i][j][r];
+#pragma unroll
+    for (int t = 0; t < CT; ++t) {
+        float v = cs[t];
+        v += __shfl_xor(v, 16, 64);
+        v += __shfl_xor(v, 32, 64);
+        if (q == 0) csum[wave][16 * t + n] = v;
+    }
     __syncthreads();
+    float* __restrict__ out = part + (size_t)blockIdx.x * (ic * ic + (raw ? ic : 0));
     for (int e = tid; e < ic * ic; e += 256) {
         const int gi = e / ic, gj = e - gi * ic;
         const int i = gi >> 4, ri = gi & 15, j = gj >> 4, l = (ri >> 2) * 16 + (gj & 15), r = ri & 3;
-        part[(size_t)blockIdx.x * ic * ic + e] =
-            (red[0][i * CT + j][r][l] + red[1][i * CT + j][r][l]) + (red[2][i * CT + j][r][l] + red[3][i * CT + j][r][l]);
+        out[e] = (red[0][i * CT + j][r][l] + red[1][i * CT + j][r][l]) + (red[2][i * CT + j][r][l] + red[3][i * CT + j][r][l]);
     }
+    if (raw && tid < ic) out[ic * ic + tid] = (csum[0][tid] + csum[1][tid]) + (csum[2][tid] + csum[3][tid]);
 }
 
 __global__ __launch_bounds__(256) void k_stats1_gram(TfnasCellDesc d, const double* __restrict__ xsum,
-                                                     const double* __restrict__ C, double* __restrict__ stats1) {
+                                                     const double* __restrict__ C, double* __restrict__ stats1, int raw) {
     __shared__ double Cs[40 * 40 + 40];
     const int ic = d.ic;
     for (int i = threadIdx.x; i < ic * ic + ic; i += 256) Cs[i] = i < ic * ic ? C[i] : xsum[i - ic * ic];
@@ -113,7 +128,7 @@
             q += (double)w[c] * (t0 + t1);
             s += (double)w[c] * Cs[ic * ic + c];
         }
-        q += s * s / P;
+        if (!raw) q += s * s / P;
     }
     stats1[2 * (size_t)col + 0] = s;
     stats1[2 * (size_t)col + 1] = q;
@@ -143,25 +158,32 @@
     if (rps < 256) rps = 256;
     rps = (rps + 63) & ~63;
     const int nb = cdiv(P, rps);
-    double* xsum = reinterpret_cast<double*>(part + TFNAS_PART_FLOATS) - (ne + ic + 2);
-    xsum = reinterpret_cast<double*>((uintptr_t)xsum & ~(uintptr_t)15);
-    double* C = xsum + ic;
-    if ((size_t)nb * ne + 2 * (size_t)(ne + ic + 4) > TFNAS_PART_FLOATS) return TFNAS_ERANGE;
+    const bool one = gram_one_pass(d);
+    const int row = one ? ne + ic : ne;
+    double* top = reinterpret_cast<double*>(part + TFNAS_PART_FLOATS) - (ne + ic + 2);
+    top = reinterpret_cast<double*>((uintptr_t)top & ~(uintptr_t)15);
+    double* xsum = one ? top + ne : top;
+    double* C = one ? top : top + ic;
+    if ((size_t)nb * row + 2 * (size_t)(ne + ic + 4) > TFNAS_PART_FLOATS) return TFNAS_ERANGE;
+    int rc = 0;
+    if (!one) {
+        {
+            ProfScope _prof(TK_EXPAND_FWD, s);
+            hipLaunchKernelGGL(k_x_colsum, dim3(nb), dim3(256), 0, s, x, P, ic, rps, part);
+        }
+        rc = launch_reduce_rows(part, nb, ic, (size_t)ic, xsum, nullptr, s);
+        if (rc) return rc;
+    }
     {
         ProfScope _prof(TK_EXPAND_FWD, s);
-        hipLaunchKernelGGL(k_x_colsum, dim3(nb), dim3(256), 0, s, x, P, ic, rps, part);
+        const double* mean_of = one ? nullptr : xsum;
+        if (ic <= 16) hipLaunchKernelGGL(k_x_gram<1>, dim3(nb), dim3(256), 0, s, x, P, ic, rps, mean_of, part);
+        else if (ic <= 32) hipLaunchKernelGGL(k_x_gram<2>, dim3(nb), dim3(256), 0, s, x, P, ic, rps, mean_of, part);
+        else hipLaunchKernelGGL(k_x_gram<3>, dim3(nb), dim3(256), 0, s, x, P, ic, rps, mean_of, part);
     }
-    int rc = launch_reduce_rows(part, nb, ic, (size_t)ic, xsum, nullptr, s);
-    if (rc) return rc;
-    {
-        ProfScope _prof(TK_EXPAND_FWD, s);
-        if (ic <= 16) hipLaunchKernelGGL(k_x_gram<1>, dim3(nb), dim3(256), 0, s, x, P, ic, rps, xsum, part);
-        else if (ic <= 32) hipLaunchKernelGGL(k_x_gram<2>, dim3(nb), dim3(256), 0, s, x, P, ic, rps, xsum, part);
-        else hipLaunchKernelGGL(k_x_gram<3>, dim3(nb), dim3(256), 0, s, x, P, ic, rps, xsum, part);
-    }
-    rc = launch_reduce_rows(part, nb, ne, (size_t)ne, C, nullptr, s);
+    rc = launch_reduce_rows(part, nb, row, (size_t)row, C, nullptr, s);
     if (rc) return rc;
     ProfScope _prof(TK_SMALL, s);
-    hipLaunchKernelGGL(k_stats1_gram, dim3(cdiv(d.M, 256)), dim3(256), 0, s, d, xsum, C, stats1);
+    hipLaunchKernelGGL(k_stats1_gram, dim3(cdiv(d.M, 256)), dim3(256), 0, s, d, xsum, C, stats1, one ? 1 : 0);
     return (int)hipGetLastError();
 }
diff --git a/tf-nas_amd/csrc/fx_kernels.hip b/tf-nas_amd/csrc/fx_kernels.hip
--- a/tf-nas_amd/csrc/fx_kernels.hip
+++ b/tf-nas_amd/csrc/fx_kernels.hip
@@ -129,7 +129,7 @@
     }
     if (pl.XB) {
         f32x4* c2 = reinterpret_cast<f32x4*>(b + pl.PB + pl.WB);
-        if (tid < 8) {
+        if (tid < 8 && stats2) {
             f32x4 t = zero4();
             const int ch = cy + tid;
             if (c0 + ch < mc) {
@@ -1088,12 +1088,14 @@
     constexpr int NT = (CT + 3) / 4;
     const int tid = threadIdx.x, lane = tid & 63, wave = tid >> 6, n = lane & 15, q = lane >> 4, jy = blockIdx.y;
     const int r0 = blockIdx.x * rps, r1 = min(P, r0 + rps);
-    float mui[NT], muj[NT];
+    const bool raw = xsum == nullptr;
+    float mui[NT], muj[NT], cs[NT];
 #pragma unroll
     for (int t = 0; t < NT; ++t) {
         const int it = wave + 4 * t, jt = jy + 4 * t;
-        mui[t] = it < CT ? (float)(xsum[16 * it + n] / (double)P) : 0.f;
-        muj[t] = jt < CT ? (float)(xsum[16 * jt + n] / (double)P) : 0.f;
+        mui[t] = (!raw && it < CT) ? (float)(xsum[16 * it + n] / (double)P) : 0.f;
+        muj[t] = (!raw && jt < CT) ? (float)(xsum[16 * jt + n] / (double)P) : 0.f;
+        cs[t] = 0.f;
     }
     f32x4 acc[NT][NT];
 #pragma unroll
@@ -1121,8 +1123,21 @@
             for (int i = 0; i < NT; ++i)
 #pragma unroll
                 for (int j = 0; j < NT; ++j) acc[i][j] = __builtin_amdgcn_mfma_f32_16x16x4f32(a[u][i], b[u][j], acc[i][j], 0, 0, 0);
-    }
-    float* __restrict__ out = part + (size_t)blockIdx.x * ic * ic;
+#pragma unroll
+        for (int u = 0; u < RU; ++u)
+#pragma unroll
+            for (int t = 0; t < NT; ++t) cs[t] += a[u][t];
+    }
+    float* __restrict__ out = part + (size_t)blockIdx.x * (ic * ic + (raw ? ic : 0));
+    if (raw && jy == 0) {
+#pragma unroll
+        for (int t = 0; t < NT; ++t) {
+            float v = cs[t];
+            v += __shfl_xor(v, 16, 64);
+            v += __shfl_xor(v, 32, 64);
+            if (q == 0 && wave + 4 * t < CT) out[ic * ic + 16 * (wave + 4 * t) + n] = v;
+        }
+    }
 #pragma unroll
     for (int i = 0; i < NT; ++i) {
         const int it = wave + 4 * i;
@@ -1148,7 +1163,7 @@
 }
 template <int CT>
 __global__ __launch_bounds__(256) void k_fx_stats1(TfnasCellDesc d, const double* __restrict__ xsum, const double* __restrict__ C,
-                                                   double* __restrict__ stats1) {
+                                                   double* __restrict__ stats1, int raw) {
     constexpr int NT = (CT + 3) / 4;
     __shared__ double red[2][4][16];
     const int tid = threadIdx.x, lane = tid & 63, wave = tid >> 6, n = lane & 15, q = lane >> 4, ic = d.ic, col0 = blockIdx.x * 16;
@@ -1219,40 +1234,48 @@
         const double qf = (red[1][0][tid] + red[1][1][tid]) + (red[1][2][tid] + red[1][3][tid]);
         const double P = (double)d.N * d.H * d.W;
         stats1[2 * (size_t)(col0 + tid) + 0] = sm;
-        stats1[2 * (size_t)(col0 + tid) + 1] = qf + sm * sm / P;
+        stats1[2 * (size_t)(col0 + tid) + 1] = raw ? qf : qf + sm * sm / P;
     }
 }
 
 int launch_fx_stats(const TfnasCellDesc& d, const float* x, double* stats1, float* part, hipStream_t s) {
     const int P = d.N * d.H * d.W, ic = d.ic, ne = ic * ic;
+    const bool one = gram_one_pass(d);
+    const int row = one ? ne + ic : ne;
     int nb = 256;
-    while (nb > 1 && (size_t)nb * ne + 2 * (size_t)(ne + ic + 4) + 64 > TFNAS_PART_FLOATS) nb >>= 1;
+    while (nb > 1 && (size_t)nb * row + 2 * (size_t)(ne + ic + 4) + 64 > TFNAS_PART_FLOATS) nb >>= 1;
     int rps = cdiv(P, nb);
     rps = (rps + 3) & ~3;
     if (rps < 16) rps = 16;
     nb = cdiv(P, rps);
-    double* xsum = reinterpret_cast<double*>(part + TFNAS_PART_FLOATS) - (ne + ic + 2);
-    xsum = reinterpret_cast<double*>((uintptr_t)xsum & ~(uintptr_t)15);
-    double* Cm = xsum + ic;
-    int rc = launch_x_colsum(x, P, ic, rps, nb, part, s);
-    if (rc) return rc;
-    rc = launch_reduce_rows(part, nb, ic, (size_t)ic, xsum, nullptr, s);
-    if (rc) return rc;
+    double* top = reinterpret_cast<double*>(part + TFNAS_PART_FLOATS) - (ne + ic + 2);
+    top = reinterpret_cast<double*>((uintptr_t)top & ~(uintptr_t)15);
+    double* xsum = one ? top + ne : top;
+    double* Cm = one ? top : top + ic;
+    int rc = 0;
+    if (!one) {
+        rc = launch_x_colsum(x, P, ic, rps, nb, part, s);
+        if (rc) return rc;
+        rc = launch_reduce_rows(part, nb, ic, (size_t)ic, xsum, nullptr, s);
+        if (rc) return rc;
+    }
     {
         ProfScope _prof(TK_EXPAND_FWD, s);
         const int CT = ic / 16;
+        const double* mean_of = one ? nullptr : xsum;
         switch (CT) {
-#define FX_GRAM(N_) case N_: hipLaunchKernelGGL(k_fx_gram<N_>, dim3(nb, 4), dim3(256), 0, s, x, P, ic, rps, xsum, part); break;
+#define FX_GRAM(N_) case N_: hipLaunchKernelGGL(k_fx_gram<N_>, dim3(nb, 4), dim3(256), 0, s, x, P, ic, rps, mean_of, part); break;
             FX_GRAM(4) FX_GRAM(5) FX_GRAM(6) FX_GRAM(7) FX_GRAM(8) FX_GRAM(9) FX_GRAM(10) FX_GRAM(11) FX_GRAM(12)
 #undef FX_GRAM
             default: return TFNAS_EINVAL;
         }
     }
-    rc = launch_reduce_rows(part, nb, ne, (size_t)ne, Cm, nullptr, s);
+    rc = launch_reduce_rows(part, nb, row, (size_t)row, Cm, nullptr, s);
     if (rc) return rc;
     ProfScope _prof(TK_SMALL, s);
+    const int raw = one ? 1 : 0;
     switch (ic / 16) {
-#define FX_ST1(N_) case N_: hipLaunchKernelGGL(k_fx_stats1<N_>, dim3(cdiv(d.M, 16)), dim3(256), 0, s, d, xsum, Cm, stats1); break;
+#define FX_ST1(N_) case N_: hipLaunchKernelGGL(k_fx_stats1<N_>, dim3(cdiv(d.M, 16)), dim3(256), 0, s, d, xsum, Cm, stats1, raw); break;
         FX_ST1(4) FX_ST1(5) FX_ST1(6) FX_ST1(7) FX_ST1(8) FX_ST1(9) FX_ST1(10) FX_ST1(11) FX_ST1(12)
 #undef FX_ST1
         default: return TFNAS_EINVAL;
@@ -1264,12 +1287,18 @@
     return hipFuncSetAttribute(fn, hipFuncAttributeMaxDynamicSharedMemorySize, (int)shm) == hipSuccess;
 }
 
+static void fx_keep_layout(const TfnasCellDesc& d, FxPlan& pl) {
+    pl.XB = 512 + 3 * d.ic * 64;
+    pl.BLOB = (pl.PB + pl.WB + pl.XB + 255) & ~255;
+}
+
 int launch_fx_fwd(const TfnasCellDesc& d, const float* x, const double* stats1, float* E, float* D, double* stats2,
-                  float* part, hipStream_t s) {
+                  float* part, hipStream_t s, float* keep) {
     FxPlan pl;
     if (!fx_plan(d, pl, false)) return TFNAS_EINVAL;
     const size_t rows = ((size_t)pl.nig * 2 * d.M + 63) & ~(size_t)63;
-    u8* blob = reinterpret_cast<u8*>(part + rows);
+    u8* blob = reinterpret_cast<u8*>(keep ? keep : part + rows);
+    if (keep) fx_keep_layout(d, pl);
     {
         ProfScope _prof(TK_SMALL, s);
         hipLaunchKernelGGL(k_fx_pack, dim3(pl.nchunks, 4), dim3(256), 0, s, d, pl, stats1, (const double*)nullptr,
@@ -1346,17 +1375,31 @@
     return fx_bwd_layout(d, pb, (size_t)d.N * d.H * d.W * d.M, a, b);
 }
 
+size_t fx_keep_floats(const TfnasCellDesc& d) {
+    FxPlan pl;
+    if (!route_fxh(d) || !fx_supported(d) || !bn2_fused_fits(d) || !fx_plan(d, pl, true)) return 0;
+    return ((size_t)pl.nchunks * pl.BLOB + 3) / 4;
+}
+
+FxCst2 fx_keep_cst2(const TfnasCellDesc& d, float* keep) {
+    FxPlan pl;
+    if (!keep || !fx_plan(d, pl, true)) return {nullptr, 0};
+    return {reinterpret_cast<u8*>(keep) + pl.PB + pl.WB, pl.BLOB};
+}
+
 int launch_fx_bwd(const TfnasCellDesc& d, const float* x, const float* Eh, const double* stats1, const double* stats2,
                   const double* red2, const float* dZ, const float* D, const float* gate, const float* dpooled, float* scratch,
-                  size_t scratch_floats, double* red1, float* cb1, float* part, int* nsl, hipStream_t s) {
+                  size_t scratch_floats, double* red1, float* cb1, float* part, int* nsl, hipStream_t s, const float* keep) {
     FxPlan pl;
     if (!fx_plan(d, pl, true)) return TFNAS_EINVAL;
     size_t bo_s, bo_p;
     if (!fx_bwd_layout(d, pl, scratch_floats, bo_s, bo_p)) return TFNAS_ERANGE;
-    u8* blob = reinterpret_cast<u8*>(bo_s != ~(size_t)0 ? scratch + bo_s : part + bo_p);
-    {
+    const u8* blob = reinterpret_cast<const u8*>(keep);
+    if (!keep) {
+        u8* own = reinterpret_cast<u8*>(bo_s != ~(size_t)0 ? scratch + bo_s : part + bo_p);
+        blob = own;
         ProfScope _prof(TK_SMALL, s);
-        hipLaunchKernelGGL(k_fx_pack, dim3(pl.nchunks, 4), dim3(256), 0, s, d, pl, stats1, stats2, red2, blob);
+        hipLaunchKernelGGL(k_fx_pack, dim3(pl.nchunks, 4), dim3(256), 0, s, d, pl, stats1, stats2, red2, own);
     }
     const size_t shm = Eh ? fx_bwde_lds(d, pl) : fx_bwd_lds(d, pl);
     const dim3 grid(pl.nig * pl.nslices);
diff --git a/tf-nas_amd/csrc/kernels.h b/tf-nas_amd/csrc/kernels.h
--- a/tf-nas_amd/csrc/kernels.h
+++ b/tf-nas_amd/csrc/kernels.h
@@ -26,6 +26,8 @@
 static inline int route_dw(const TfnasCellDesc& d) { return (d.route & TFNAS_ROUTE_DW_MASK) >> TFNAS_ROUTE_DW_SHIFT; }
 static inline int route_se(const TfnasCellDesc& d) { return (d.route & TFNAS_ROUTE_SE_MASK) >> TFNAS_ROUTE_SE_SHIFT; }
 static inline bool route_side(const TfnasCellDesc& d) { return !(d.route & TFNAS_ROUTE_WGRAD_INLINE); }
+static inline bool route_fxh(const TfnasCellDesc& d) { return !(d.route & TFNAS_ROUTE_FXH_OFF); }
+static inline bool gram_one_pass(const TfnasCellDesc& d) { return (d.flags & TFNAS_CELL_CENTRED) && route_fxh(d); }
 static inline int wgrad_accum(const TfnasCellDesc& d) { return (d.flags & TFNAS_CELL_ACCUM_WGRAD) ? 1 : 0; }
 static constexpr bool act_tile_only(int act) { return act == TFNAS_ACT_RELU6 || act == TFNAS_ACT_HSWISH; }
 static inline bool cell_noexpand(const TfnasCellDesc& d) { return (d.flags & TFNAS_CELL_NOEXPAND) != 0; }
@@ -135,10 +137,17 @@
 bool fx_supported(const TfnasCellDesc& d);
 int launch_fx_stats(const TfnasCellDesc& d, const float* x, double* stats1, float* part, hipStream_t s);
 int launch_fx_fwd(const TfnasCellDesc& d, const float* x, const double* stats1, float* E, float* D, double* stats2,
-                  float* part, hipStream_t s);
+                  float* part, hipStream_t s, float* keep = nullptr);
 int launch_fx_bwd(const TfnasCellDesc& d, const float* x, const float* Eh, const double* stats1, const double* stats2,
                   const double* red2, const float* dZ, const float* D, const float* gate, const float* dpooled, float* scratch,
-                  size_t scratch_floats, double* red1, float* cb1, float* part, int* nsl, hipStream_t s);
+                  size_t scratch_floats, double* red1, float* cb1, float* part, int* nsl, hipStream_t s,
+                  const float* keep = nullptr);
+size_t fx_keep_floats(const TfnasCellDesc& d);
+struct FxCst2 {
+    unsigned char* base;
+    int stride;
+};
+FxCst2 fx_keep_cst2(const TfnasCellDesc& d, float* keep);
 bool dw_wgrad_row_fits(const TfnasCellDesc& d);
 DwPlan dw_plan_bwd_data(const TfnasCellDesc& d, bool efree, bool has_x);
 int launch_dw_bwd_data(const DwPlan& p, const TfnasCellDesc& d, const float* dZ, const float* gate, const float* dpooled,
@@ -178,7 +187,7 @@
                     float* pp, hipStream_t s);
 int launch_bn2_gather(const TfnasCellDesc& d, const float* rec, float* dgate, float* pp, hipStream_t s);
 int launch_bn2_finish(const TfnasCellDesc& d, const float* pp, const float* gate, const float* dpooled, double* red2,
-                      hipStream_t s);
+                      hipStream_t s, const double* stats2 = nullptr, FxCst2 c2 = {nullptr, 0});
 int launch_bn2_bwd(const TfnasCellDesc& d, const float* dZ, const float* D, const double* stats2, const float* gate,
                    const float* dpooled, double* red2, float* part, hipStream_t s);
 int launch_head_pool(const TfnasCellDesc& d, const float* E, const double* stats1, float* pooled, hipStream_t s);
diff --git a/tf-nas_amd/csrc/path.hip b/tf-nas_amd/csrc/path.hip
--- a/tf-nas_amd/csrc/path.hip
+++ b/tf-nas_amd/csrc/path.hip
@@ -11,6 +11,7 @@
 
 struct CellOff {
     uint64_t E, D, Pr, fsmall, stats, out;
+    uint64_t fx_keep;
 };
 struct StageOff {
     uint64_t sink_out, bw, dots, bound;
@@ -46,6 +47,23 @@
     int fwd_route[TFNAS_MAX_CELLS] = {};
 };
 
+uint32_t centred_cells(const TfnasPathDesc& pd) {
+    uint32_t mask = 0;
+    bool in_c = false;
+    int i = 0;
+    for (int st = 0; st < pd.nstage; ++st) {
+        const TfnasStage& sg = pd.stage[st];
+        bool sink_c = sg.start_res != 0 || in_c;
+        for (int j = 0; j < sg.ncell; ++j, ++i) {
+            if (in_c) mask |= 1u << i;
+            in_c = !pd.cell[i].has_res || in_c;
+            sink_c = sink_c && in_c;
+        }
+        in_c = sink_c;
+    }
+    return mask;
+}
+
 int plan_path(PathCtx& c, const TfnasPathDesc& in, TfnasPathWs* out) {
     if (in.ncell < 1 || in.ncell > TFNAS_MAX_CELLS || in.nstage < 1 || in.nstage > TFNAS_MAX_STAGES) return TFNAS_ERANGE;
     c.planned = false;
@@ -65,6 +83,7 @@
     }
     if (nc != pd.ncell) return TFNAS_EINVAL;
     if (pd.reserved0 != 0) return TFNAS_EINVAL;
+    const uint32_t centred = centred_cells(pd);
     for (int i = 0; i < pd.ncell; ++i) {
         TfnasCellDesc& d = pd.cell[i];
         if (d.mode != TFNAS_MODE_CELL) return TFNAS_EINVAL;
@@ -77,6 +96,7 @@
             d.H = p.Ho;
             d.W = p.Wo;
         }
+        if ((centred >> i) & 1) d.flags |= TFNAS_CELL_CENTRED;
         TRY(tfnas_cell_plan(&d));
         TRY(tfnas_cell_ws(&d, &c.cws[i]));
         const bool efree = (pd.efree_mask_lo >> i) & 1;
@@ -108,6 +128,9 @@
         o.fsmall = off; off += up(w.fsmall);
         o.stats = off; off += up(2 * w.stats);
         o.out = off; off += up(w.out);
+        const uint64_t keep = fx_keep_floats(pd.cell[i]);
+        o.fx_keep = ~(uint64_t)0;
+        if (keep) { o.fx_keep = off; off += up(keep); }
     }
     for (int st = 0; st < pd.nstage; ++st) {
         const TfnasStage& sg = pd.stage[st];
@@ -179,6 +202,7 @@
     b.stats = reinterpret_cast<double*>(arena + o.stats);
     b.part = arena + c.set[0].part;
     b.out = arena + o.out;
+    b.fx_keep = o.fx_keep == ~(uint64_t)0 ? nullptr : arena + o.fx_keep;
     return cell_fwd_impl(pd.cell[i], c.cws[i], b, s, &c.fwd_route[i]);
 }
 
@@ -261,6 +285,20 @@
     if (e == hipSuccess) e = hipStreamWaitEvent(s, c->join, 0);
     if (e != hipSuccess) (void)hipStreamSynchronize(c->side);
     return (int)e;
+}
+
+extern "C" int tfnas_path_centred_cells(const TfnasPathDesc* pd, uint32_t* mask) {
+    if (!pd || !mask) return TFNAS_ENULL;
+    if (pd->ncell < 1 || pd->ncell > TFNAS_MAX_CELLS || pd->nstage < 1 || pd->nstage > TFNAS_MAX_STAGES) return TFNAS_ERANGE;
+    int nc = 0;
+    for (int st = 0; st < pd->nstage; ++st) {
+        const TfnasStage& sg = pd->stage[st];
+        if (sg.ncell < 1 || sg.ncell > TFNAS_MAX_SINK || (sg.start_res != 0 && sg.start_res != 1)) return TFNAS_EINVAL;
+        nc += sg.ncell;
+    }
+    if (nc != pd->ncell) return TFNAS_EINVAL;
+    *mask = centred_cells(*pd);
+    return 0;
 }
 
 extern "C" int tfnas_path_plan(void* ctx, const TfnasPathDesc* pd, TfnasPathWs* ws) {
@@ -388,6 +426,7 @@
     b.part_w = r.arena + ss.part_w;
     b.dxp = r.arena + c.dxp;
     b.dwmix = (r.dwmix && pd.soft) ? r.dwmix + (size_t)i * TFNAS_MAX_GROUPS : nullptr;
+    b.fx_keep = o.fx_keep == ~(uint64_t)0 ? nullptr : r.arena + o.fx_keep;
     if (j > 0) b.dx = r.arena + c.ring[i % NRING];
     else if (st > 0) b.dx = r.arena + c.so[st - 1].bound;
     else b.dx = pd.need_dx0 ? r.dx0 : nullptr;
diff --git a/tf-nas_amd/csrc/pointwise_kernels.hip b/tf-nas_amd/csrc/pointwise_kernels.hip
--- a/tf-nas_amd/csrc/pointwise_kernels.hip
+++ b/tf-nas_amd/csrc/pointwise_kernels.hip
@@ -302,7 +302,7 @@
 
 __global__ __launch_bounds__(256) void k_bn2_finish(TfnasCellDesc d, const float* __restrict__ pp,
                                                     const float* __restrict__ gate, const float* __restrict__ dpooled,
-                                                    double* __restrict__ red2) {
+                                                    double* __restrict__ red2, const double* __restrict__ stats2, FxCst2 c2) {
     __shared__ double sh[2][16][65];
     int g, c0;
     if (!chunk_locate(d, blockIdx.x, 64, false, g, c0)) return;
@@ -339,14 +339,30 @@
     __syncthreads();
     if (tid < 128) {
         const int which = tid >> 6, cl = tid & 63;
+        double t = 0.0;
         if (c0 + cl < mc) {
-            double t = 0.0;
 #pragma unroll
             for (int r = 0; r < 16; ++r) t += sh[which][r][cl];
             red2[2 * (size_t)(off + c0 + cl) + which] = t;
         } else if (c0 + cl < mcp) {
             red2[2 * (size_t)(off + c0 + cl) + which] = 0.0;
         }
+        if (c2.base) sh[which][0][cl] = t;
+    }
+    if (!c2.base) return;
+    __syncthreads();
+    if (tid < 64 && c0 + tid < ((mcp + 31) & ~31)) {
+        const int ch = c0 + tid;
+        f32x4 t = zero4();
+        if (ch < mc) {
+            const double inv = 1.0 / ((double)N * d.Ho * d.Wo);
+            const float2 c = bn_consts(stats2 + 2 * (size_t)(off + ch), inv, d.eps);
+            t.x = c.x;
+            t.y = c.y;
+            t.z = (float)(sh[0][0][tid] * inv);
+            t.w = (float)(sh[1][0][tid] * inv);
+        }
+        reinterpret_cast<f32x4*>(c2.base + (size_t)((off + ch) >> 5) * c2.stride)[ch & 31] = t;
     }
 }
 
@@ -781,9 +797,10 @@
 }
 
 int launch_bn2_finish(const TfnasCellDesc& d, const float* pp, const float* gate, const float* dpooled, double* red2,
-                      hipStream_t s) {
+                      hipStream_t s, const double* stats2, FxCst2 c2) {
     ProfScope _prof(TK_BN2_BWD, s);
-    hipLaunchKernelGGL(k_bn2_finish, dim3(chunk_count(d, 64, false)), dim3(256), 0, s, d, pp, gate, dpooled, red2);
+    if (c2.base && !stats2) return TFNAS_ENULL;
+    hipLaunchKernelGGL(k_bn2_finish, dim3(chunk_count(d, 64, false)), dim3(256), 0, s, d, pp, gate, dpooled, red2, stats2, c2);
     return (int)hipGetLastError();
 }
 
diff --git a/tf-nas_amd/tfnas_amd/_lib.py b/tf-nas_amd/tfnas_amd/_lib.py
--- a/tf-nas_amd/tfnas_amd/_lib.py
+++ b/tf-nas_amd/tfnas_amd/_lib.py
@@ -26,6 +26,8 @@
 ROUTE_DW = {'auto': 0, 'direct': 1 << 6, 'lds': 2 << 6, 'tiled': 3 << 6}
 ROUTE_SE = {'wave': 0, 'fused': 1 << 8, 'gemm': 2 << 8}
 ROUTE_WGRAD_INLINE, ROUTE_GRAM2 = 0x400, 0x800
+ROUTE_FXH_OFF = 0x2000
+CELL_CENTRED = 0x800
 ROUTE_TAKEN_VALID, ROUTE_TAKEN_FX = 1, 2
 GEMM_MODES = {'f32': 0, 'bf16': 1, 'x2': 3, 'x3': 6}
 
@@ -149,6 +151,8 @@
     'tfnas_efree_supported': (C.c_int, [C.POINTER(TfnasCellDesc)]),
     'tfnas_fx_supported': (C.c_int, [C.POINTER(TfnasCellDesc)]),
     'tfnas_cell_route': (C.c_int, [C.POINTER(TfnasCellDesc)]),
+    'tfnas_fx_keep_floats': (C.c_uint64, [C.POINTER(TfnasCellDesc)]),
+    'tfnas_path_centred_cells': (C.c_int, [C.POINTER(TfnasPathDesc), C.POINTER(C.c_uint32)]),
     'tfnas_arch_project': (C.c_int, [C.c_int, C.POINTER(_P), C.POINTER(C.c_int32), _P]),
     'tfnas_arch_sample': (C.c_int, [C.c_int, C.POINTER(_P), _P, _P, C.c_float, C.c_int, _P, _P]),
     'tfnas_sink_fwd': (C.c_int, [C.c_int, _P, C.POINTER(_P), _P, C.c_uint64, _P, _P, _P, _P]),
diff --git a/tf-nas_amd/tfnas_amd/functions.py b/tf-nas_amd/tfnas_amd/functions.py
--- a/tf-nas_amd/tfnas_amd/functions.py
+++ b/tf-nas_amd/tfnas_amd/functions.py
@@ -16,7 +16,8 @@
     env = os.environ if env is None else env
     r = 0
     for var, bit in (('TFNAS_FX', _lib.ROUTE_FX_OFF), ('TFNAS_FOLD', _lib.ROUTE_FOLD_OFF), ('TFNAS_DWWG', _lib.ROUTE_DWWG_OFF),
-                     ('TFNAS_DWWG2', _lib.ROUTE_DWWG2_OFF), ('TFNAS_WGRAD_STREAM', _lib.ROUTE_WGRAD_INLINE)):
+                     ('TFNAS_DWWG2', _lib.ROUTE_DWWG2_OFF), ('TFNAS_WGRAD_STREAM', _lib.ROUTE_WGRAD_INLINE),
+                     ('TFNAS_FXH', _lib.ROUTE_FXH_OFF)):
         if env.get(var, '1')[:1] == '0':
             r |= bit
     xg = env.get('TFNAS_XG', 'auto')
@@ -27,10 +28,11 @@
     return r
 
 
-def route_bits(fx=True, fold=True, dwwg=True, dwwg2=True, xg='auto', dw='auto', se='wave', wgrad_stream=True, gram=1):
+def route_bits(fx=True, fold=True, dwwg=True, dwwg2=True, xg='auto', dw='auto', se='wave', wgrad_stream=True, gram=1, fxh=True):
     return route_from_env({'TFNAS_FX': '1' if fx else '0', 'TFNAS_FOLD': '1' if fold else '0', 'TFNAS_DWWG': '1' if dwwg else '0',
                            'TFNAS_DWWG2': '1' if dwwg2 else '0', 'TFNAS_XG': xg, 'TFNAS_DW': dw, 'TFNAS_SE': se,
-                           'TFNAS_WGRAD_STREAM': '1' if wgrad_stream else '0', 'TFNAS_GRAM': str(gram)})
+                           'TFNAS_WGRAD_STREAM': '1' if wgrad_stream else '0', 'TFNAS_GRAM': str(gram),
+                           'TFNAS_FXH': '1' if fxh else '0'})
 
 
 ENV_ROUTE = route_from_env()
@@ -129,8 +131,9 @@
     def __deepcopy__(self, memo):
         return None
 
-    def __init__(self, ic, oc, stride, act, blocks, mode=_lib.MODE_CELL, modes=None):
+    def __init__(self, ic, oc, stride, act, blocks, mode=_lib.MODE_CELL, modes=None, input_centred=False):
         self.ic, self.oc, self.stride, self.act = ic, oc, stride, act
+        self.input_centred = bool(input_centred)
         self.blocks = list(blocks)
         kinds = [getattr(b, 'kind', _lib.MBCONV) for b in self.blocks]
         if _lib.FUSED in kinds and (len(self.blocks) != 1 or mode != _lib.MODE_CELL):
@@ -174,14 +177,19 @@
             d.act, d.has_res, d.G, d.need_wgrad, d.eps = _lib.act_id(self.act), self.has_res, len(self.blocks), 0, BN_EPS
             for g, b in enumerate(self.blocks):
                 d.g[g].mc, d.g[g].k, d.g[g].se = b.mid_channels, b.kernel_size, b.se_channels
-            self.modes.apply(d, *self._kind_arg)
+            self._apply_modes(d)
             check(_lib.lib().tfnas_cell_plan(C.byref(d)), 'tfnas_cell_plan')
             ws = TfnasCellWs()
             check(_lib.lib().tfnas_cell_ws(C.byref(d), C.byref(ws)), 'tfnas_cell_ws')
             hit = (d, ws)
             self._desc_cache[key] = hit
-        self.modes.apply(hit[0], *self._kind_arg)
+        self._apply_modes(hit[0])
         return hit
+
+    def _apply_modes(self, d):
+        self.modes.apply(d, *self._kind_arg)
+        if self.input_centred:
+            d.flags |= _lib.CELL_CENTRED
 
     def bind(self, d, params, grads=None):
         for (g, f), p in zip(self._w_slots, params):
diff --git a/tf-nas_amd/tfnas_amd/model_search.py b/tf-nas_amd/tfnas_amd/model_search.py
--- a/tf-nas_amd/tfnas_amd/model_search.py
+++ b/tf-nas_amd/tfnas_amd/model_search.py
@@ -80,7 +80,7 @@
             self._plans, p = {}, None
         if p is None:
             p = CellPlan(self.in_channels, self.out_channels, self.stride, self.act_func,
-                         [self.m_ops[i] for i in idxs])
+                         [self.m_ops[i] for i in idxs], input_centred=getattr(self, 'input_centred', False))
             self._plans[key] = p
         return p
 
@@ -273,7 +273,21 @@
     def cells(self):
         if self._cells is None:
             self._cells = [blk for st in self.stages() for blk in st.blocks()]
+            self._mark_centred_inputs()
         return self._cells
+
+    def _mark_centred_inputs(self):
+        import ctypes as C
+        pd = _lib.TfnasPathDesc()
+        pd.ncell, pd.nstage = len(self._cells), len(self._stage_names)
+        for k, st in enumerate(self.stages()):
+            pd.stage[k].ncell, pd.stage[k].start_res = st.nblocks, st.start_res
+        for i, c in enumerate(self._cells):
+            pd.cell[i].has_res = int(c.in_channels == c.out_channels and c.stride == 1)
+        mask = C.c_uint32(0)
+        _lib.check(_lib.lib().tfnas_path_centred_cells(C.byref(pd), C.byref(mask)), 'tfnas_path_centred_cells')
+        for i, c in enumerate(self._cells):
+            c.input_centred = bool((mask.value >> i) & 1)
 
     def arch_weights(self, size, dev, exp_noise=None):
         cells = self.cells()
```

Measured after the change: 3886. Within noise of the previous version (-0.1%).
